# lipku/LiveTalking

Measured on AMD Instinct MI355X. Metric: inferfps, higher is better.
Workload: dtype f16; 1 GPU; wav2lip256, 1 session(s)/GPU, 16-frame batch, fp16 activations / fp32 accumulate, through LipReal.inference_batch; sessions_per_gpu=1, batch=16, parallelism=session-sharded x1 (no collective)

## Files before the change

include/ltk.h:

```cpp
#ifndef LTK_H
#define LTK_H

#include <stddef.h>
#include <stdint.h>

#ifdef __cplusplus
extern "C" {
#endif

#define LTK_OK 0
#define LTK_E_INVALID (-1)
#define LTK_E_HIP (-2)
#define LTK_E_STATE (-3)
#define LTK_E_NOMEM (-4)

typedef struct ltk_engine ltk_engine;

typedef struct ltk_named_tensor {
    const char* name;
    const float* data;
    int ndim;
    const int64_t* shape;
} ltk_named_tensor;

typedef struct ltk_w2l_req {
    int avatar;
    int index;
    int batch;
    const void* d_mel;
    void* d_pred;
} ltk_w2l_req;

const char* ltk_last_error(void);
const char* ltk_version(void);

int ltk_engine_create(int device, ltk_engine** out);
void ltk_engine_destroy(ltk_engine* e);
int ltk_engine_sync(ltk_engine* e);

int ltk_wav2lip_load(ltk_engine* e, const ltk_named_tensor* sd, int n, int max_frames);

int ltk_avatar_register(ltk_engine* e, const uint8_t* face_bank, const uint8_t* full_bank,
                        const int32_t* coords, int n, int H, int W, int* avatar_id);
int ltk_avatar_release(ltk_engine* e, int avatar_id);

int ltk_mel_step(ltk_engine* e, const float* pcm, int n_samples, const int32_t* win_start,
                 int n_win, void* d_out, void* stream);

int ltk_wav2lip_infer(ltk_engine* e, const ltk_w2l_req* reqs, int nreq, void* stream);

int ltk_paste_back(ltk_engine* e, int avatar_id, int idx, const void* d_pred, void* out,
                   int out_is_device, void* stream);

int ltk_paste_back_batch(ltk_engine* e, int avatar_id, const int32_t* idx, const void* d_pred, int n, void* out, void* stream);


int ltk_musetalk_load(ltk_engine* e, const ltk_named_tensor* unet_sd, int n_unet, const ltk_named_tensor* vae_sd,
                      int n_vae, int max_frames);

int ltk_musetalk_avatar_register(ltk_engine* e, const float* latents, const uint8_t* full_bank, const int32_t* face_boxes,
                                 const int32_t* crop_boxes, const uint8_t* masks, const int64_t* mask_offsets, int n,
                                 int H, int W, int* avatar_id);

int ltk_musetalk_set_fp8(ltk_engine* e, int enable, float act_scale);
int ltk_musetalk_info(ltk_engine* e, double* macs_per_frame, double* macs_fp8_per_frame);

typedef struct ltk_mt_req {
    int avatar;
    int index;
    int batch;
    const void* d_feat;
    void* d_pred;
} ltk_mt_req;

int ltk_musetalk_infer(ltk_engine* e, const ltk_mt_req* reqs, int nreq, void* stream);

int ltk_paste_blend(ltk_engine* e, int avatar_id, int idx, const void* d_pred, void* out, int out_is_device, void* stream);


int ltk_ultralight_avatar_register(ltk_engine* e, const ltk_named_tensor* sd, int n_tensors, const uint8_t* face_bank,
                                   const uint8_t* full_bank, const int32_t* coords, int n, int H, int W, int max_frames, int* avatar_id);

typedef struct ltk_ul_req {
    int avatar;
    int index;
    int batch;
    const void* d_feat;
    void* d_pred;
} ltk_ul_req;

int ltk_ultralight_infer(ltk_engine* e, const ltk_ul_req* reqs, int nreq, void* stream);

int ltk_ultralight_paste_back(ltk_engine* e, int avatar_id, int idx, const void* d_pred, void* out, int out_is_device, void* stream);

int ltk_ultralight_paste_back_batch(ltk_engine* e, int avatar_id, const int32_t* idx, const void* d_pred, int n, void* out, void* stream);

typedef struct ltk_egress ltk_egress;
int ltk_egress_open(ltk_engine* e, int H, int W, ltk_egress** out);
int ltk_egress_close(ltk_engine* e, ltk_egress* s);
int ltk_egress_watermark(ltk_engine* e, ltk_egress* s, const uint8_t* mask, int x, int y, int w, int h, int b, int g, int r);

#define LTK_FMT_BGR24 0
#define LTK_FMT_I420 1
#define LTK_SRC_WAV2LIP 0
#define LTK_SRC_MUSETALK 1
#define LTK_SRC_HOST 2
#define LTK_SRC_ULTRALIGHT 3
typedef struct ltk_egress_req {
    int source;
    int avatar, idx;
    const void* d_pred;
    const uint8_t* h_frame;
    int speaking;
    double alpha;
    int keep;
    int format;
    int chroma;
} ltk_egress_req;
int ltk_egress_frame(ltk_engine* e, ltk_egress* s, const ltk_egress_req* req, uint8_t* h_out, void* stream);

int ltk_egress_batch(ltk_engine* e, ltk_egress* s, int source, int avatar, const int32_t* idx, const void* d_pred, int n, int format,
                     int chroma, uint8_t* h_out, void* stream);

int ltk_whisper_load(ltk_engine* e, const ltk_named_tensor* encoder_sd, int n);

int ltk_whisper_step(ltk_engine* e, const float* pcm, int n_samples, int batch, int first_row, int row_step, int rows,
                     void* d_out, void* stream);


int ltk_hubert_load(ltk_engine* e, const ltk_named_tensor* sd, int n);

int ltk_hubert_features(ltk_engine* e, const float* pcm, long long n_samples, float* out_host, int cap_rows, int* rows);

int ltk_hubert_step(ltk_engine* e, const float* pcm, int n_samples, int batch, int first_row, int row_step, int rows, void* d_out);

int ltk_vae_encoder_load(ltk_engine* e, const ltk_named_tensor* vae_sd, int n, int max_faces);
int ltk_vae_encode_faces(ltk_engine* e, const uint8_t* faces_bgr, int nfaces, const float* noise, float* latents_out);


int ltk_whisper_debug_get(ltk_engine* e, const char* name, float* out, size_t n_floats);

int ltk_hubert_debug_get(ltk_engine* e, const char* name, float* out, size_t n_floats);
int ltk_hubert_op_count(ltk_engine* e);
int ltk_hubert_op_name(ltk_engine* e, int op, char* buf, int buf_len, int* type);
int ltk_hubert_info(ltk_engine* e, int* layers, int* programs, size_t* activation_bytes);
int ltk_hubert_stats(ltk_engine* e, const float* pcm, long long n, float* mean_var);
int ltk_hubert_layer0_host(ltk_engine* e, const float* x, int n, const float* w, const float* bias, const float* gamma, const float* beta,
                           float* out);
int ltk_hubert_ln_gelu_host(ltk_engine* e, const float* x, int T, const float* gamma, const float* beta, float* out);
int ltk_hubert_posconv_host(ltk_engine* e, const float* x, int T, const float* w, const float* bias, float* out);
int ltk_hubert_chunks_host(ltk_engine* e, const float* feat, int T, int batch, int first_row, int row_step, int rows, float* out);

int ltk_musetalk_forward_host(ltk_engine* e, const float* latents, const float* feat, int B, float* unet_out, float* image,
                              uint8_t* frames);
int ltk_musetalk_debug_get(ltk_engine* e, const char* name, int frames, float* out, size_t n_floats);
int ltk_musetalk_time(ltk_engine* e, int frames, int iters, float* ms_per_pass, double* macs_per_pass);
int ltk_musetalk_op_count(ltk_engine* e);
int ltk_musetalk_op_name(ltk_engine* e, int op, char* buf, int buf_len, int* type);
int ltk_musetalk_time_ops(ltk_engine* e, int frames, int iters, float* ms_per_op, int n_ops);


int ltk_wav2lip_forward_host(ltk_engine* e, const float* mel, const float* face6, int B, float* pred);

int ltk_ultralight_forward_host(ltk_engine* e, int avatar_id, const float* img6, const float* feat, int B, float* pred);
int ltk_ultralight_op_count(ltk_engine* e, int avatar_id);
int ltk_ultralight_op_name(ltk_engine* e, int avatar_id, int op, char* buf, int buf_len, int* type);
int ltk_ultralight_time(ltk_engine* e, int avatar_id, int frames, int iters, float* ms_per_pass, double* macs_per_pass);

int ltk_dwconv3x3_f16(ltk_engine* e, const void* d_x, int N, int H, int W, int C, const float* weight, int stride, const float* scale,
                      const float* shift, int relu, void* d_y);
int ltk_upsample2x_cat_f16(ltk_engine* e, const void* d_x, int N, int h, int w, int C_up, const void* d_skip, int Hs, int Ws, int C_skip,
                           void* d_y);

int ltk_debug_saturation(ltk_engine* e, int reset, unsigned long long* n_at_limit, unsigned long long* n_nonfinite);
int ltk_debug_capture(ltk_engine* e, int enable);
int ltk_debug_get(ltk_engine* e, const char* layer, float* out, size_t n_floats);

int ltk_debug_set_knob(const char* name, int value);

int ltk_debug_tile_table_check(char* msg, int cap);

int ltk_wav2lip_time_convs(ltk_engine* e, int frames, int iters, float* ms_per_pass, double* macs_per_pass);

int ltk_wav2lip_graph_count(ltk_engine* e);

int ltk_avatar_face_cache_bytes(ltk_engine* e, int avatar_id, size_t* bytes);

int ltk_wav2lip_prefetch_stats(ltk_engine* e, unsigned long long* hits, unsigned long long* misses, unsigned long long* issued);

int ltk_program_graph_count(ltk_engine* e);

int ltk_wav2lip_layer_count(ltk_engine* e);
int ltk_wav2lip_layer_name(ltk_engine* e, int layer, char* buf, int buf_len);
int ltk_wav2lip_set_layer_tile(ltk_engine* e, int layer, int bucket, int pxw, int nbt, int ksplit);
int ltk_wav2lip_time_layers(ltk_engine* e, int frames, int iters, float* ms_per_layer, int n_layers);

int ltk_conv2d_f16(ltk_engine* e, const void* d_x, int N, int H, int W, int Cin,
                   const float* weight, int Cout, int kh, int kw, int sh, int sw, int ph, int pw,
                   int transposed, int out_pad, const float* scale, const float* shift,
                   const void* d_res, int relu, void* d_y, int iters, float* ms_avg);

typedef struct ltk_conv_opts {
    int x_ld, x_coff, y_ld, y_coff, res_ld, res_coff;
    int act, ups;
    int force_pxw, force_nbt, force_ksplit;
    int family;
} ltk_conv_opts;
typedef struct ltk_conv_report {
    char kernel[64];
    int family, G, NBT, PXW, NC8, T, S, ksplit, items, grid, FT, UB;
} ltk_conv_report;
int ltk_conv2d_f16_ex(ltk_engine* e, const void* d_x, int N, int H, int W, int Cin,
                      const float* weight, int Cout, int kh, int kw, int sh, int sw, int ph, int pw,
                      int transposed, int out_pad, const float* scale, const float* shift,
                      const void* d_res, int relu, void* d_y, const ltk_conv_opts* opts, ltk_conv_report* rep);

int ltk_debug_conv_plan(int N, int H, int W, int Cin, int Cout, int kh, int kw, int sh, int sw, int ph, int pw,
                        int transposed, int out_pad, int has_res, int relu, const ltk_conv_opts* opts, ltk_conv_report* rep);

int ltk_debug_conv3_variants(char* buf, int cap);

int ltk_groupnorm_f16(ltk_engine* e, const void* d_x, int N, int C, int P, int groups, float eps, const float* gamma, const float* beta,
                      int silu, int impl, int out_fp8, float out_scale, void* d_y, int iters, float* ms_avg);

typedef struct ltk_norm_opts {
    int x_ld, x_coff, y_ld, y_coff;
} ltk_norm_opts;
typedef struct ltk_norm_report {
    char kernel[64];
    int impl, segs, members, grid;
} ltk_norm_report;
int ltk_groupnorm_f16_ex(ltk_engine* e, const void* d_x, int N, int C, int P, int groups, float eps, const float* gamma, const float* beta,
                         int silu, int impl, int out_fp8, float out_scale, void* d_y, const ltk_norm_opts* opts, ltk_norm_report* rep);

enum { LTK_PW_LAYERNORM = 0, LTK_PW_GEGLU = 1, LTK_PW_ACT_GELU = 2, LTK_PW_ACT_SILU = 3, LTK_PW_ADD_POS = 4, LTK_PW_NCHW_TO_CB16 = 5,
       LTK_PW_TOKENS_TO_CB16 = 6, LTK_PW_VAE_POST = 7 };
int ltk_pointwise_f16(ltk_engine* e, int op, const void* d_x, void* d_y, int N, int C, int P, float eps, const float* v0, const float* v1,
                      const ltk_norm_opts* opts);

int ltk_attention_f16(ltk_engine* e, const void* d_q, int q_cbt, int q_cb0, const void* d_k, int k_cbt, int k_cb0, const void* d_v, int v_cbt,
                      int v_cb0, void* d_o, int o_cbt, int o_cb0, int N, int heads, int d16, int Tq, int Tk, int impl);

int ltk_f32_to_e4m3(const float* in, size_t n, uint8_t* out);

int ltk_conv2d_fp8(ltk_engine* e, const void* d_x, int N, int H, int W, int Cin, const float* weight, int Cout,
                   const float* scale, const float* shift, float act_scale, const void* d_res, int act, void* d_y, int iters,
                   float* ms_avg);

int ltk_conv2d_fp8_ex(ltk_engine* e, const void* d_x, int N, int H, int W, int Cin, const float* weight, int Cout,
                      const float* scale, const float* shift, float act_scale, int quant, const void* d_res, void* d_y,
                      const ltk_conv_opts* opts, ltk_conv_report* rep);

int ltk_debug_conv_fp8_plan(int N, int H, int W, int Cin, int Cout, int kh, int kw, int sh, int sw, int ph, int pw,
                            int transposed, int out_pad, int quant, int has_res, const ltk_conv_opts* opts, ltk_conv_report* rep);

int ltk_debug_conv3_fp8_variants(char* buf, int cap);

#ifdef __cplusplus
}
#endif
#endif
```

livetalking_amd/_lib.py:

```python
from __future__ import annotations

import ctypes as C
import os

_HERE = os.path.dirname(os.path.abspath(__file__))
LIB_PATH = os.environ.get("LTK_LIB") or os.path.join(_HERE, "libltk_hip.so")


class LtkError(RuntimeError):
    def __init__(self, code: int, msg: str):
        super().__init__(f"ltk error {code}: {msg}")
        self.code = code


class NamedTensor(C.Structure):
    _fields_ = [("name", C.c_char_p), ("data", C.POINTER(C.c_float)), ("ndim", C.c_int),
                ("shape", C.POINTER(C.c_int64))]


class W2lReq(C.Structure):
    _fields_ = [("avatar", C.c_int), ("index", C.c_int), ("batch", C.c_int), ("d_mel", C.c_void_p),
                ("d_pred", C.c_void_p)]


class MtReq(C.Structure):
    _fields_ = [("avatar", C.c_int), ("index", C.c_int), ("batch", C.c_int), ("d_feat", C.c_void_p), ("d_pred", C.c_void_p)]


class UlReq(C.Structure):
    _fields_ = [("avatar", C.c_int), ("index", C.c_int), ("batch", C.c_int), ("d_feat", C.c_void_p), ("d_pred", C.c_void_p)]


class EgressReq(C.Structure):
    _fields_ = [("source", C.c_int), ("avatar", C.c_int), ("idx", C.c_int), ("d_pred", C.c_void_p), ("h_frame", C.c_void_p),
                ("speaking", C.c_int), ("alpha", C.c_double), ("keep", C.c_int), ("format", C.c_int), ("chroma", C.c_int)]


class ConvOpts(C.Structure):
    _fields_ = [(n, C.c_int) for n in ("x_ld", "x_coff", "y_ld", "y_coff", "res_ld", "res_coff", "act", "ups", "force_pxw", "force_nbt",
                                       "force_ksplit", "family")]


class ConvReport(C.Structure):
    _fields_ = [("kernel", C.c_char * 64)] + [(n, C.c_int) for n in ("family", "G", "NBT", "PXW", "NC8", "T", "S", "ksplit", "items", "grid",
                                                                     "FT", "UB")]


class NormOpts(C.Structure):
    _fields_ = [(n, C.c_int) for n in ("x_ld", "x_coff", "y_ld", "y_coff")]


class NormReport(C.Structure):
    _fields_ = [("kernel", C.c_char * 64)] + [(n, C.c_int) for n in ("impl", "segs", "members", "grid")]


SYMBOLS = {
    "ltk_last_error": (C.c_char_p, []),
    "ltk_version": (C.c_char_p, []),
    "ltk_engine_create": (C.c_int, [C.c_int, C.POINTER(C.c_void_p)]),
    "ltk_engine_destroy": (None, [C.c_void_p]),
    "ltk_engine_sync": (C.c_int, [C.c_void_p]),
    "ltk_wav2lip_load": (C.c_int, [C.c_void_p, C.POINTER(NamedTensor), C.c_int, C.c_int]),
    "ltk_avatar_register": (C.c_int, [C.c_void_p, C.c_void_p, C.c_void_p, C.c_void_p, C.c_int, C.c_int, C.c_int,
                                      C.POINTER(C.c_int)]),
    "ltk_avatar_release": (C.c_int, [C.c_void_p, C.c_int]),
    "ltk_mel_step": (C.c_int, [C.c_void_p, C.c_void_p, C.c_int, C.c_void_p, C.c_int, C.c_void_p, C.c_void_p]),
    "ltk_wav2lip_infer": (C.c_int, [C.c_void_p, C.POINTER(W2lReq), C.c_int, C.c_void_p]),
    "ltk_paste_back": (C.c_int, [C.c_void_p, C.c_int, C.c_int, C.c_void_p, C.c_void_p, C.c_int, C.c_void_p]),
    "ltk_paste_back_batch": (C.c_int, [C.c_void_p, C.c_int, C.c_void_p, C.c_void_p, C.c_int, C.c_void_p, C.c_void_p]),
    "ltk_musetalk_load": (C.c_int, [C.c_void_p, C.POINTER(NamedTensor), C.c_int, C.POINTER(NamedTensor), C.c_int, C.c_int]),
    "ltk_musetalk_set_fp8": (C.c_int, [C.c_void_p, C.c_int, C.c_float]),
    "ltk_musetalk_info": (C.c_int, [C.c_void_p, C.POINTER(C.c_double), C.POINTER(C.c_double)]),
    "ltk_musetalk_avatar_register": (C.c_int, [C.c_void_p, C.c_void_p, C.c_void_p, C.c_void_p, C.c_void_p, C.c_void_p, C.c_void_p,
                                               C.c_int, C.c_int, C.c_int, C.POINTER(C.c_int)]),
    "ltk_musetalk_infer": (C.c_int, [C.c_void_p, C.POINTER(MtReq), C.c_int, C.c_void_p]),
    "ltk_paste_blend": (C.c_int, [C.c_void_p, C.c_int, C.c_int, C.c_void_p, C.c_void_p, C.c_int, C.c_void_p]),
    "ltk_ultralight_avatar_register": (C.c_int, [C.c_void_p, C.POINTER(NamedTensor), C.c_int, C.c_void_p, C.c_void_p, C.c_void_p, C.c_int,
                                                 C.c_int, C.c_int, C.c_int, C.POINTER(C.c_int)]),
    "ltk_ultralight_infer": (C.c_int, [C.c_void_p, C.POINTER(UlReq), C.c_int, C.c_void_p]),
    "ltk_ultralight_paste_back": (C.c_int, [C.c_void_p, C.c_int, C.c_int, C.c_void_p, C.c_void_p, C.c_int, C.c_void_p]),
    "ltk_ultralight_paste_back_batch": (C.c_int, [C.c_void_p, C.c_int, C.c_void_p, C.c_void_p, C.c_int, C.c_void_p, C.c_void_p]),
    "ltk_ultralight_forward_host": (C.c_int, [C.c_void_p, C.c_int, C.c_void_p, C.c_void_p, C.c_int, C.c_void_p]),
    "ltk_ultralight_time": (C.c_int, [C.c_void_p, C.c_int, C.c_int, C.c_int, C.POINTER(C.c_float), C.POINTER(C.c_double)]),
    "ltk_dwconv3x3_f16": (C.c_int, [C.c_void_p, C.c_void_p, C.c_int, C.c_int, C.c_int, C.c_int, C.c_void_p, C.c_int, C.c_void_p,
                                    C.c_void_p, C.c_int, C.c_void_p]),
    "ltk_upsample2x_cat_f16": (C.c_int, [C.c_void_p, C.c_void_p, C.c_int, C.c_int, C.c_int, C.c_int, C.c_void_p, C.c_int, C.c_int,
                                         C.c_int, C.c_void_p]),
    "ltk_egress_open": (C.c_int, [C.c_void_p, C.c_int, C.c_int, C.POINTER(C.c_void_p)]),
    "ltk_egress_close": (C.c_int, [C.c_void_p, C.c_void_p]),
    "ltk_egress_watermark": (C.c_int, [C.c_void_p, C.c_void_p, C.c_void_p, C.c_int, C.c_int, C.c_int, C.c_int, C.c_int, C.c_int, C.c_int]),
    "ltk_egress_frame": (C.c_int, [C.c_void_p, C.c_void_p, C.POINTER(EgressReq), C.c_void_p, C.c_void_p]),
    "ltk_egress_batch": (C.c_int, [C.c_void_p, C.c_void_p, C.c_int, C.c_int, C.c_void_p, C.c_void_p, C.c_int, C.c_int, C.c_int,
                                   C.c_void_p, C.c_void_p]),
    "ltk_musetalk_forward_host": (C.c_int, [C.c_void_p, C.c_void_p, C.c_void_p, C.c_int, C.c_void_p, C.c_void_p, C.c_void_p]),
    "ltk_musetalk_debug_get": (C.c_int, [C.c_void_p, C.c_char_p, C.c_int, C.c_void_p, C.c_size_t]),
    "ltk_musetalk_time": (C.c_int, [C.c_void_p, C.c_int, C.c_int, C.POINTER(C.c_float), C.POINTER(C.c_double)]),
    "ltk_whisper_load": (C.c_int, [C.c_void_p, C.POINTER(NamedTensor), C.c_int]),
    "ltk_whisper_step": (C.c_int, [C.c_void_p, C.c_void_p, C.c_int, C.c_int, C.c_int, C.c_int, C.c_int, C.c_void_p, C.c_void_p]),
    "ltk_whisper_debug_get": (C.c_int, [C.c_void_p, C.c_char_p, C.c_void_p, C.c_size_t]),
    "ltk_hubert_load": (C.c_int, [C.c_void_p, C.POINTER(NamedTensor), C.c_int]),
    "ltk_hubert_features": (C.c_int, [C.c_void_p, C.c_void_p, C.c_longlong, C.c_void_p, C.c_int, C.POINTER(C.c_int)]),
    "ltk_hubert_step": (C.c_int, [C.c_void_p, C.c_void_p, C.c_int, C.c_int, C.c_int, C.c_int, C.c_int, C.c_void_p]),
    "ltk_hubert_debug_get": (C.c_int, [C.c_void_p, C.c_char_p, C.c_void_p, C.c_size_t]),
    "ltk_ultralight_op_count": (C.c_int, [C.c_void_p, C.c_int]),
    "ltk_ultralight_op_name": (C.c_int, [C.c_void_p, C.c_int, C.c_int, C.c_char_p, C.c_int, C.POINTER(C.c_int)]),
    "ltk_hubert_op_count": (C.c_int, [C.c_void_p]),
    "ltk_hubert_op_name": (C.c_int, [C.c_void_p, C.c_int, C.c_char_p, C.c_int, C.POINTER(C.c_int)]),
    "ltk_hubert_info": (C.c_int, [C.c_void_p, C.POINTER(C.c_int), C.POINTER(C.c_int), C.POINTER(C.c_size_t)]),
    "ltk_hubert_stats": (C.c_int, [C.c_void_p, C.c_void_p, C.c_longlong, C.c_void_p]),
    "ltk_hubert_layer0_host": (C.c_int, [C.c_void_p, C.c_void_p, C.c_int, C.c_void_p, C.c_void_p, C.c_void_p, C.c_void_p, C.c_void_p]),
    "ltk_hubert_ln_gelu_host": (C.c_int, [C.c_void_p, C.c_void_p, C.c_int, C.c_void_p, C.c_void_p, C.c_void_p]),
    "ltk_hubert_posconv_host": (C.c_int, [C.c_void_p, C.c_void_p, C.c_int, C.c_void_p, C.c_void_p, C.c_void_p]),
    "ltk_hubert_chunks_host": (C.c_int, [C.c_void_p, C.c_void_p, C.c_int, C.c_int, C.c_int, C.c_int, C.c_int, C.c_void_p]),
    "ltk_vae_encoder_load": (C.c_int, [C.c_void_p, C.POINTER(NamedTensor), C.c_int, C.c_int]),
    "ltk_vae_encode_faces": (C.c_int, [C.c_void_p, C.c_void_p, C.c_int, C.c_void_p, C.c_void_p]),
    "ltk_wav2lip_forward_host": (C.c_int, [C.c_void_p, C.c_void_p, C.c_void_p, C.c_int, C.c_void_p]),
    "ltk_debug_capture": (C.c_int, [C.c_void_p, C.c_int]),
    "ltk_debug_saturation": (C.c_int, [C.c_void_p, C.c_int, C.POINTER(C.c_ulonglong), C.POINTER(C.c_ulonglong)]),
    "ltk_debug_set_knob": (C.c_int, [C.c_char_p, C.c_int]),
    "ltk_debug_tile_table_check": (C.c_int, [C.c_char_p, C.c_int]),
    "ltk_debug_get": (C.c_int, [C.c_void_p, C.c_char_p, C.c_void_p, C.c_size_t]),
    "ltk_wav2lip_time_convs": (C.c_int, [C.c_void_p, C.c_int, C.c_int, C.POINTER(C.c_float), C.POINTER(C.c_double)]),
    "ltk_wav2lip_graph_count": (C.c_int, [C.c_void_p]),
    "ltk_program_graph_count": (C.c_int, [C.c_void_p]),
    "ltk_wav2lip_prefetch_stats": (C.c_int, [C.c_void_p, C.POINTER(C.c_ulonglong), C.POINTER(C.c_ulonglong), C.POINTER(C.c_ulonglong)]),
    "ltk_avatar_face_cache_bytes": (C.c_int, [C.c_void_p, C.c_int, C.POINTER(C.c_size_t)]),
    "ltk_musetalk_op_count": (C.c_int, [C.c_void_p]),
    "ltk_musetalk_op_name": (C.c_int, [C.c_void_p, C.c_int, C.c_char_p, C.c_int, C.POINTER(C.c_int)]),
    "ltk_musetalk_time_ops": (C.c_int, [C.c_void_p, C.c_int, C.c_int, C.POINTER(C.c_float), C.c_int]),
    "ltk_wav2lip_layer_count": (C.c_int, [C.c_void_p]),
    "ltk_wav2lip_layer_name": (C.c_int, [C.c_void_p, C.c_int, C.c_char_p, C.c_int]),
    "ltk_wav2lip_set_layer_tile": (C.c_int, [C.c_void_p, C.c_int, C.c_int, C.c_int, C.c_int, C.c_int]),
    "ltk_wav2lip_time_layers": (C.c_int, [C.c_void_p, C.c_int, C.c_int, C.POINTER(C.c_float), C.c_int]),
    "ltk_conv2d_f16": (C.c_int, [C.c_void_p, C.c_void_p, C.c_int, C.c_int, C.c_int, C.c_int, C.c_void_p, C.c_int,
                                 C.c_int, C.c_int, C.c_int, C.c_int, C.c_int, C.c_int, C.c_int, C.c_int,
                                 C.c_void_p, C.c_void_p, C.c_void_p, C.c_int, C.c_void_p, C.c_int,
                                 C.POINTER(C.c_float)]),
    "ltk_conv2d_f16_ex": (C.c_int, [C.c_void_p, C.c_void_p, C.c_int, C.c_int, C.c_int, C.c_int, C.c_void_p, C.c_int,
                                    C.c_int, C.c_int, C.c_int, C.c_int, C.c_int, C.c_int, C.c_int, C.c_int,
                                    C.c_void_p, C.c_void_p, C.c_void_p, C.c_int, C.c_void_p, C.POINTER(ConvOpts), C.POINTER(ConvReport)]),
    "ltk_debug_conv_plan": (C.c_int, [C.c_int] * 15 + [C.POINTER(ConvOpts), C.POINTER(ConvReport)]),
    "ltk_debug_conv3_variants": (C.c_int, [C.c_char_p, C.c_int]),
    "ltk_groupnorm_f16": (C.c_int, [C.c_void_p, C.c_void_p, C.c_int, C.c_int, C.c_int, C.c_int, C.c_float, C.c_void_p, C.c_void_p, C.c_int, C.c_int,
                                    C.c_int, C.c_float, C.c_void_p, C.c_int, C.POINTER(C.c_float)]),
    "ltk_groupnorm_f16_ex": (C.c_int, [C.c_void_p, C.c_void_p, C.c_int, C.c_int, C.c_int, C.c_int, C.c_float, C.c_void_p, C.c_void_p, C.c_int, C.c_int,
                                       C.c_int, C.c_float, C.c_void_p, C.POINTER(NormOpts), C.POINTER(NormReport)]),
    "ltk_pointwise_f16": (C.c_int, [C.c_void_p, C.c_int, C.c_void_p, C.c_void_p, C.c_int, C.c_int, C.c_int, C.c_float, C.c_void_p, C.c_void_p,
                                    C.POINTER(NormOpts)]),
    "ltk_attention_f16": (C.c_int, [C.c_void_p] + [C.c_void_p, C.c_int, C.c_int] * 4 + [C.c_int] * 6),
    "ltk_f32_to_e4m3": (C.c_int, [C.c_void_p, C.c_size_t, C.c_void_p]),
    "ltk_conv2d_fp8": (C.c_int, [C.c_void_p, C.c_void_p, C.c_int, C.c_int, C.c_int, C.c_int, C.c_void_p, C.c_int, C.c_void_p,
                                 C.c_void_p, C.c_float, C.c_void_p, C.c_int, C.c_void_p, C.c_int, C.POINTER(C.c_float)]),
    "ltk_conv2d_fp8_ex": (C.c_int, [C.c_void_p, C.c_void_p, C.c_int, C.c_int, C.c_int, C.c_int, C.c_void_p, C.c_int, C.c_void_p,
                                    C.c_void_p, C.c_float, C.c_int, C.c_void_p, C.c_void_p, C.POINTER(ConvOpts), C.POINTER(ConvReport)]),
    "ltk_debug_conv_fp8_plan": (C.c_int, [C.c_int] * 15 + [C.POINTER(ConvOpts), C.POINTER(ConvReport)]),
    "ltk_debug_conv3_fp8_variants": (C.c_int, [C.c_char_p, C.c_int]),
}

_lib = None


def load() -> C.CDLL:
    global _lib
    if _lib is not None:
        return _lib
    if not os.path.exists(LIB_PATH):
        raise RuntimeError(
            f"{LIB_PATH} is missing: build it with `python -c 'import __graft_entry__ as g; g.build()'` "
            "(or `make -C livetalking_amd/csrc`). livetalking_amd has no CPU fallback.")
    try:
        import torch
    except ImportError:
        pass
    lib = C.CDLL(LIB_PATH)
    other_build = bool(os.environ.get("LTK_LIB"))
    for name, (res, args) in SYMBOLS.items():
        if other_build and not hasattr(lib, name):
            continue
        fn = getattr(lib, name)
        fn.restype = res
        fn.argtypes = args
    _lib = lib
    return lib


def check(rc: int) -> None:
    if rc != 0:
        msg = load().ltk_last_error()
        raise LtkError(rc, msg.decode("utf-8", "replace") if msg else "")
```

livetalking_amd/avatars/wav2lip_avatar.py:

```python
from __future__ import annotations

import glob
import os
import pickle
import threading
import weakref

import numpy as np

from ..egress import SRC_WAV2LIP, DeviceEgressMixin, FrameGroup
from ..engine import Engine
from ..hostshim import BaseAvatar, mirror_index, register
from ..scheduler import get_scheduler
from ..sharding import EnginePool, visible_devices
from .audio_features.mel import MelASR

_PASTE_BATCH = os.environ.get("LTK_PASTE_BATCH", "1") != "0"


class Wav2LipModel:

    def __init__(self, engine_or_pool):
        if isinstance(engine_or_pool, EnginePool):
            self.pool = engine_or_pool
        else:
            self.pool = EnginePool([getattr(engine_or_pool, "device", 0)], lambda d: engine_or_pool)
        self.engines = self.pool.engines
        self._avatars = {}
        self._lock = threading.Lock()

    @property
    def engine(self) -> Engine:
        return self.engines[0]

    def place(self, session) -> int:
        slot = self.pool.place(id(session))
        weakref.finalize(session, self.pool.release, id(session))
        return slot

    def avatar_id(self, avatar, slot: int = 0) -> int:
        frame_list, face_list, coord_list = avatar
        key = (id(face_list), slot)
        with self._lock:
            aid = self._avatars.get(key)
            if aid is None:
                aid = self.engines[slot].register_avatar(face_list, frame_list, coord_list)
                self._avatars[key] = aid
            return aid

    def eval(self):
        return self


def _state_dict_from_checkpoint(path):
    import torch
    checkpoint = torch.load(path, map_location="cpu")
    s = checkpoint["state_dict"]
    return {k.replace("module.", ""): v for k, v in s.items()}


def load_model(path, state_dict=None, max_frames=None, device=None):
    if state_dict is None:
        state_dict = _state_dict_from_checkpoint(path)
    if max_frames is None:
        max_frames = int(os.environ.get("LTK_MAX_FRAMES", "256"))

    def factory(dev):
        eng = Engine(dev)
        eng.load_wav2lip(state_dict, max_frames=max_frames)
        return eng

    devices = visible_devices() if device is None else [int(device)]
    cap = int(os.environ.get("LTK_SESSIONS_PER_GPU", "0")) or (1 << 30)
    return Wav2LipModel(EnginePool(devices, factory, capacity_per_gpu=cap))


def read_imgs(img_list):
    import cv2
    return [cv2.imread(p) for p in img_list]


def load_avatar(avatar_id):
    avatar_path = f"./data/avatars/{avatar_id}"
    bank_path = os.path.join(avatar_path, "bank.ltkbank")
    if os.path.exists(bank_path):
        from ..bank import load_bank
        return load_bank(bank_path).as_avatar()
    with open(f"{avatar_path}/coords.pkl", "rb") as f:
        coord_list_cycle = pickle.load(f)

    def numbered(d):
        files = glob.glob(os.path.join(d, "*.[jpJP][pnPN]*[gG]"))
        return sorted(files, key=lambda x: int(os.path.splitext(os.path.basename(x))[0]))

    frame_list_cycle = read_imgs(numbered(f"{avatar_path}/full_imgs"))
    face_list_cycle = read_imgs(numbered(f"{avatar_path}/face_imgs"))
    return frame_list_cycle, face_list_cycle, coord_list_cycle


def warm_up(batch_size, model, modelres=256):
    mel = np.ones((batch_size, 80, 16), dtype=np.float32)
    img = np.ones((batch_size, 6, modelres, modelres), dtype=np.float32)
    for eng in model.engines:
        n = min(batch_size, eng.max_frames)
        eng.wav2lip_forward_host(mel[:n], img[:n])


@register("avatar", "wav2lip")
class LipReal(DeviceEgressMixin, BaseAvatar):
    _egress_source = SRC_WAV2LIP

    def __init__(self, opt, model, avatar):
        super().__init__(opt)
        self.model = model
        self.frame_list_cycle, self.face_list_cycle, self.coord_list_cycle = avatar
        self._slot = model.place(self)
        self.engine = model.engines[self._slot]
        self._aid = model.avatar_id(avatar, self._slot)
        h, w = self.frame_list_cycle[0].shape[:2]
        self._frame_hw = (int(h), int(w))
        self._sched = get_scheduler(self.engine)
        self.asr = MelASR(opt, self, engine=self.engine)
        self.asr.warm_up()

    def _mel_to_device(self, audiofeat_batch):
        import torch
        if isinstance(audiofeat_batch, torch.Tensor):
            return audiofeat_batch
        arr = np.ascontiguousarray(np.asarray(audiofeat_batch), dtype=np.float32)
        return torch.from_numpy(arr).to(self.engine.torch_device)

    def inference_batch(self, index, audiofeat_batch):
        import torch
        mel = self._mel_to_device(audiofeat_batch)
        B = self.batch_size
        if mel.shape[0] != B:
            raise ValueError(f"expected {B} mel windows, got {mel.shape[0]}")
        pred = torch.empty((B, 256, 256, 3), dtype=torch.uint8, device=mel.device)
        self._sched.infer(self._aid, int(index), B, mel.data_ptr(), pred.data_ptr())
        self._last_mel = mel
        items = list(pred.unbind(0))
        if _PASTE_BATCH and hasattr(self.engine, "paste_back_batch"):
            FrameGroup.attach(items, pred, span=(len(self.frame_list_cycle), int(index), B))
        return items

    def paste_back_frame(self, pred_frame, idx: int):
        import torch
        if not isinstance(pred_frame, torch.Tensor):
            pred_frame = torch.from_numpy(np.ascontiguousarray(pred_frame).astype(np.uint8)).to(
                self.engine.torch_device)
        h, w = self._frame_hw
        grp = getattr(pred_frame, "_ltk_group", None)
        if grp is not None and grp.idx[pred_frame._ltk_i] == int(idx):
            with grp.lock:
                if grp.host is None:
                    host = torch.empty((len(grp.idx), h, w, 3), dtype=torch.uint8, pin_memory=True)
                    self.engine.paste_back_batch(self._aid, grp.idx, grp.pred.data_ptr(), host.data_ptr())
                    grp.host = host.numpy()
            return grp.host[pred_frame._ltk_i]
        out = np.empty((h, w, 3), dtype=np.uint8)
        self.engine.paste_back(self._aid, int(idx), pred_frame.data_ptr(), out)
        return out
```

livetalking_amd/csrc/egress.hip:

```cpp
#include "engine_internal.h"

struct ltk_egress {
    int H = 0, W = 0;
    std::mutex mu;
    uint8_t* d_cache[2] = {nullptr, nullptr};
    bool have[2] = {false, false};
    uint8_t* d_frame = nullptr;
    uint8_t* d_out = nullptr;
    uint8_t* d_wm = nullptr;
    int wm_x = 0, wm_y = 0, wm_w = 0, wm_h = 0, wm_b = 0, wm_g = 0, wm_r = 0;
};

extern "C" {

int ltk_egress_open(ltk_engine* e, int H, int W, ltk_egress** out) {
    if (!e || !out || H <= 0 || W <= 0) return fail(LTK_E_INVALID, "bad arguments");
    CHK(enter_device(e->device));
    ltk_egress* s = new ltk_egress();
    s->H = H; s->W = W;
    const size_t bytes = (size_t)H * W * 3;
    if (hipMalloc((void**)&s->d_cache[0], bytes) != hipSuccess || hipMalloc((void**)&s->d_cache[1], bytes) != hipSuccess ||
        hipMalloc((void**)&s->d_frame, bytes) != hipSuccess || hipMalloc((void**)&s->d_out, bytes) != hipSuccess) {
        (void)hipFree(s->d_cache[0]); (void)hipFree(s->d_cache[1]); (void)hipFree(s->d_frame); (void)hipFree(s->d_out);
        delete s;
        return fail(LTK_E_NOMEM, "egress session buffers");
    }
    *out = s;
    return LTK_OK;
}

int ltk_egress_close(ltk_engine* e, ltk_egress* s) {
    if (!e || !s) return fail(LTK_E_INVALID, "bad arguments");
    CHK(enter_device(e->device));
    {
        std::lock_guard<std::mutex> g(s->mu);
        (void)hipFree(s->d_cache[0]); (void)hipFree(s->d_cache[1]); (void)hipFree(s->d_frame); (void)hipFree(s->d_out); (void)hipFree(s->d_wm);
    }
    delete s;
    return LTK_OK;
}

int ltk_egress_watermark(ltk_engine* e, ltk_egress* s, const uint8_t* mask, int x, int y, int w, int h, int b, int g, int r) {
    if (!e || !s) return fail(LTK_E_INVALID, "bad arguments");
    CHK(enter_device(e->device));
    std::lock_guard<std::mutex> gd(s->mu);
    (void)hipFree(s->d_wm);
    s->d_wm = nullptr;
    s->wm_w = s->wm_h = 0;
    if (!mask) return LTK_OK;
    if (w <= 0 || h <= 0) return fail(LTK_E_INVALID, "empty watermark rectangle");
    CHK(hipMalloc((void**)&s->d_wm, (size_t)w * h));
    CHK(hipMemcpy(s->d_wm, mask, (size_t)w * h, hipMemcpyHostToDevice));
    s->wm_x = x; s->wm_y = y; s->wm_w = w; s->wm_h = h; s->wm_b = b; s->wm_g = g; s->wm_r = r;
    return LTK_OK;
}

int ltk_egress_frame(ltk_engine* e, ltk_egress* s, const ltk_egress_req* q, uint8_t* h_out, void* stream) {
    if (!e || !s || !q || !h_out) return fail(LTK_E_INVALID, "bad arguments");
    const int H = s->H, W = s->W;
    const size_t bytes = (size_t)H * W * 3;
    if (q->format != LTK_FMT_BGR24 && q->format != LTK_FMT_I420) return fail(LTK_E_INVALID, "unknown output format");
    if (q->format == LTK_FMT_I420 && ((H | W) & 1)) return fail(LTK_E_INVALID, "I420 needs even frame dimensions");
    CHK(enter_device(e->device));
    std::lock_guard<std::mutex> gs(s->mu);
    StreamLease sl(e, stream);
    const uint8_t* src = nullptr;
    std::shared_ptr<Avatar> hold_w;
    std::shared_ptr<MtAvatar> hold_m;
    std::shared_ptr<UlAvatar> hold_u;
    if (q->source == LTK_SRC_HOST) {
        if (!q->h_frame) return fail(LTK_E_INVALID, "LTK_SRC_HOST without h_frame");
        CHK(hipMemcpyAsync(s->d_frame, q->h_frame, bytes, hipMemcpyHostToDevice, sl.s));
        src = s->d_frame;
    } else if (q->source == LTK_SRC_WAV2LIP) {
        if (!(hold_w = find_avatar(e, q->avatar))) return fail(LTK_E_STATE, "unknown avatar id");
        const Avatar& a = *hold_w;
        if (q->idx < 0 || q->idx >= a.n) return fail(LTK_E_INVALID, "frame index outside the bank");
        if (a.H != H || a.W != W) return fail(LTK_E_INVALID, "avatar frame size differs from the egress session");
        const uint8_t* full = a.d_full + (size_t)q->idx * bytes;
        if (q->d_pred) {
            const int32_t* c = a.coords.data() + 4 * (size_t)q->idx;
            launch_paste(full, H, W, (const uint8_t*)q->d_pred, c[0], c[1], c[2], c[3], s->d_frame, sl.s);
            src = s->d_frame;
        } else {
            src = full;
        }
    } else if (q->source == LTK_SRC_MUSETALK) {
        if (!(hold_m = find_mt_avatar(e, q->avatar))) return fail(LTK_E_STATE, "unknown MuseTalk avatar id");
        const MtAvatar& a = *hold_m;
        if (q->idx < 0 || q->idx >= a.n) return fail(LTK_E_INVALID, "frame index outside the bank");
        if (a.H != H || a.W != W) return fail(LTK_E_INVALID, "avatar frame size differs from the egress session");
        const uint8_t* full = a.d_full + (size_t)q->idx * bytes;
        const uint8_t* mask = a.d_masks + a.mask_off[q->idx];
        const int32_t* fb = a.face_box.data() + 4 * (size_t)q->idx;
        const int32_t* cb = a.crop_box.data() + 4 * (size_t)q->idx;
        if (q->d_pred) {
            launch_paste_blend(full, H, W, (const uint8_t*)q->d_pred, fb[0], fb[1], fb[2], fb[3], cb[0], cb[1], cb[2], cb[3], mask,
                               s->d_frame, sl.s);
            src = s->d_frame;
        } else {
            src = full;
        }
    } else if (q->source == LTK_SRC_ULTRALIGHT) {
        if (!(hold_u = find_ul_avatar(e, q->avatar))) return fail(LTK_E_STATE, "unknown Ultralight avatar id");
        const UlAvatar& a = *hold_u;
        if (q->idx < 0 || q->idx >= a.n) return fail(LTK_E_INVALID, "frame index outside the bank");
        if (a.H != H || a.W != W) return fail(LTK_E_INVALID, "avatar frame size differs from the egress session");
        const uint8_t* full = a.d_full + (size_t)q->idx * bytes;
        if (q->d_pred) {
            const int32_t* c = a.boxes.data() + 4 * (size_t)q->idx;
            launch_ul_paste(full, H, W, a.d_face + (size_t)q->idx * kUlFace * kUlFace * 3, (const uint8_t*)q->d_pred, c[0], c[1], c[2], c[3],
                            s->d_frame, sl.s);
            src = s->d_frame;
        } else {
            src = full;
        }
    } else {
        return fail(LTK_E_INVALID, "unknown frame source");
    }
    const int me = q->speaking ? 1 : 0, other = me ^ 1;
    const bool blend = q->alpha >= 0.0 && q->alpha < 1.0 && s->have[other];
    const float w_src = (float)q->alpha, w_prev = (float)(1.0 - q->alpha);
    launch_egress(src, blend ? s->d_cache[other] : nullptr, w_prev, w_src, q->keep ? s->d_cache[me] : nullptr, s->d_wm, s->wm_x,
                  s->wm_y, s->wm_w, s->wm_h, s->wm_b, s->wm_g, s->wm_r, s->d_out, H, W, q->format == LTK_FMT_I420, q->chroma, sl.s);
    CHK(hipGetLastError());
    if (q->keep) s->have[me] = true;
    const size_t out_bytes = q->format == LTK_FMT_I420 ? bytes / 2 : bytes;
    CHK(hipMemcpyAsync(h_out, s->d_out, out_bytes, hipMemcpyDeviceToHost, sl.s));
    CHK(hipStreamSynchronize(sl.s));
    return LTK_OK;
}

int ltk_egress_batch(ltk_engine* e, ltk_egress* s, int source, int avatar, const int32_t* idx, const void* d_pred, int n, int format,
                     int chroma, uint8_t* h_out, void* stream) {
    if (!e || !s || !idx || !d_pred || !h_out || n <= 0) return fail(LTK_E_INVALID, "bad arguments");
    const int H = s->H, W = s->W;
    const size_t bytes = (size_t)H * W * 3;
    if (format != LTK_FMT_BGR24 && format != LTK_FMT_I420) return fail(LTK_E_INVALID, "unknown output format");
    if (format == LTK_FMT_I420 && ((H | W) & 1)) return fail(LTK_E_INVALID, "I420 needs even frame dimensions");
    if (source != LTK_SRC_WAV2LIP && source != LTK_SRC_MUSETALK && source != LTK_SRC_ULTRALIGHT)
        return fail(LTK_E_INVALID, "batch egress: Wav2Lip, MuseTalk or Ultralight frames only");
    CHK(enter_device(e->device));
    std::lock_guard<std::mutex> gs(s->mu);
    std::shared_ptr<Avatar> hold_w;
    std::shared_ptr<MtAvatar> hold_m;
    std::shared_ptr<UlAvatar> hold_u;
    int bank_n, bank_h, bank_w;
    if (source == LTK_SRC_WAV2LIP) {
        if (!(hold_w = find_avatar(e, avatar))) return fail(LTK_E_STATE, "unknown avatar id");
        bank_n = hold_w->n; bank_h = hold_w->H; bank_w = hold_w->W;
    } else if (source == LTK_SRC_MUSETALK) {
        if (!(hold_m = find_mt_avatar(e, avatar))) return fail(LTK_E_STATE, "unknown MuseTalk avatar id");
        bank_n = hold_m->n; bank_h = hold_m->H; bank_w = hold_m->W;
    } else {
        if (!(hold_u = find_ul_avatar(e, avatar))) return fail(LTK_E_STATE, "unknown Ultralight avatar id");
        bank_n = hold_u->n; bank_h = hold_u->H; bank_w = hold_u->W;
    }
    if (bank_h != H || bank_w != W) return fail(LTK_E_INVALID, "avatar frame size differs from the egress session");
    for (int i = 0; i < n; ++i)
        if (idx[i] < 0 || idx[i] >= bank_n) return fail(LTK_E_INVALID, "frame index outside the bank");
    const size_t out_bytes = format == LTK_FMT_I420 ? bytes / 2 : bytes;
    StreamLease sl(e, stream);
    ScratchLease sc(e, (bytes + out_bytes) * n);
    if (!sc.s.d) return fail(LTK_E_NOMEM, "scratch allocation failed");
    uint8_t* const comp = (uint8_t*)sc.s.d;
    uint8_t* const conv = comp + bytes * n;
    if (hold_w) {
        const Avatar& a = *hold_w;
        for (int i0 = 0; i0 < n; i0 += kPasteBatch) {
            const int m = std::min(kPasteBatch, n - i0);
            PasteBatch pb;
            for (int i = 0; i < m; ++i) {
                const int32_t* c = a.coords.data() + 4 * (size_t)idx[i0 + i];
                pb.full[i] = a.d_full + (size_t)idx[i0 + i] * bytes;
                pb.y1[i] = c[0]; pb.y2[i] = c[1]; pb.x1[i] = c[2]; pb.x2[i] = c[3];
            }
            launch_paste_batch(pb, m, H, W, (const uint8_t*)d_pred + (size_t)i0 * 256 * 256 * 3, comp + bytes * i0, bytes, sl.s);
        }
    } else if (hold_u) {
        for (int i0 = 0; i0 < n; i0 += kPasteBatch) {
            const int m = std::min(kPasteBatch, n - i0);
            UlPasteBatch pb;
            ul_fill_paste_batch(*hold_u, idx + i0, m, &pb);
            launch_ul_paste_batch(pb, m, H, W, (const uint8_t*)d_pred + (size_t)i0 * kUlRes * kUlRes * 3, comp + bytes * i0, bytes, sl.s);
        }
    } else {
        const MtAvatar& a = *hold_m;
        for (int i = 0; i < n; ++i) {
            const int32_t* fb = a.face_box.data() + 4 * (size_t)idx[i];
            const int32_t* cb = a.crop_box.data() + 4 * (size_t)idx[i];
            launch_paste_blend(a.d_full + (size_t)idx[i] * bytes, H, W, (const uint8_t*)d_pred + (size_t)i * 256 * 256 * 3, fb[0], fb[1], fb[2], fb[3],
                               cb[0], cb[1], cb[2], cb[3], a.d_masks + a.mask_off[idx[i]], comp + bytes * i, sl.s);
        }
    }
    launch_egress_batch(comp, bytes, n, s->d_wm, s->wm_x, s->wm_y, s->wm_w, s->wm_h, s->wm_b, s->wm_g, s->wm_r, conv, out_bytes, H, W,
                        format == LTK_FMT_I420, chroma, sl.s);
    hipError_t pe = hipGetLastError();
    if (pe == hipSuccess) pe = hipMemcpyAsync(h_out, conv, out_bytes * n, hipMemcpyDeviceToHost, sl.s);
    const hipError_t se = hipStreamSynchronize(sl.s);
    if (pe != hipSuccess || se != hipSuccess) return fail(LTK_E_HIP, std::string("egress_batch: ") + hipGetErrorString(pe != hipSuccess ? pe : se));
    return LTK_OK;
}

}
```

livetalking_amd/csrc/engine.hip:

```cpp
#include "engine_internal.h"

thread_local std::string ltk::g_err;

namespace {

double hz_to_mel(double f) {
    const double f_sp = 200.0 / 3, min_log_hz = 1000.0, min_log_mel = min_log_hz / f_sp, logstep = log(6.4) / 27.0;
    return f >= min_log_hz ? min_log_mel + log(f / min_log_hz) / logstep : f / f_sp;
}
double mel_to_hz(double m) {
    const double f_sp = 200.0 / 3, min_log_hz = 1000.0, min_log_mel = min_log_hz / f_sp, logstep = log(6.4) / 27.0;
    return m >= min_log_mel ? min_log_hz * exp(logstep * (m - min_log_mel)) : f_sp * m;
}
}

void ltk::build_mel_basis(std::vector<float>* basis, std::vector<int32_t>* lohi, int n_bins, double f_lo, double f_hi) {
    const int n_mels = 80;
    const double sr = 16000.0;
    std::vector<double> mel_f(n_mels + 2);
    const double m0 = hz_to_mel(f_lo), m1 = hz_to_mel(f_hi);
    for (int i = 0; i < n_mels + 2; ++i) mel_f[i] = mel_to_hz(m0 + (m1 - m0) * i / (n_mels + 1));
    basis->assign((size_t)n_mels * n_bins, 0.f);
    lohi->assign(2 * n_mels, 0);
    for (int i = 0; i < n_mels; ++i) {
        const double enorm = 2.0 / (mel_f[i + 2] - mel_f[i]);
        int lo = n_bins, hi = 0;
        for (int k = 0; k < n_bins; ++k) {
            const double f = (sr / 2) * k / (n_bins - 1);
            const double lower = -(mel_f[i] - f) / (mel_f[i + 1] - mel_f[i]);
            const double upper = (mel_f[i + 2] - f) / (mel_f[i + 2] - mel_f[i + 1]);
            const double w = fmax(0.0, lower < upper ? lower : upper) * enorm;
            const float wf = (float)w;
            (*basis)[(size_t)i * n_bins + k] = wf;
            if (wf != 0.f) { if (k < lo) lo = k; if (k + 1 > hi) hi = k + 1; }
        }
        if (lo > hi) lo = hi = 0;
        (*lohi)[2 * i] = lo; (*lohi)[2 * i + 1] = hi;
    }
}

extern "C" {

const char* ltk_last_error(void) { return g_err.c_str(); }
const char* ltk_version(void) { return "ltk_hip 0.1 (gfx950)"; }

int ltk_engine_create(int device, ltk_engine** out) {
    if (!out) return fail(LTK_E_INVALID, "out is null");
    int ndev = 0;
    CHK(hipGetDeviceCount(&ndev));
    if (device < 0 || device >= ndev) return fail(LTK_E_INVALID, "no such HIP device");
    CHK(hipSetDevice(device));
    std::unique_ptr<ltk_engine> e(new ltk_engine());
    e->device = device;
    CHK(hipStreamCreateWithFlags(&e->compute, hipStreamNonBlocking));
    CHK(hipStreamCreateWithFlags(&e->aux, hipStreamNonBlocking));
    CHK(hipStreamCreateWithFlags(&e->aux2, hipStreamNonBlocking));
    e->graphs.side = e->aux2;
    CHK(hipEventCreateWithFlags(&e->ev_fork, hipEventDisableTiming));
    CHK(hipEventCreateWithFlags(&e->ev_join, hipEventDisableTiming));
    e->partial_cap = (size_t)128 << 20;
    e->partial_aux_cap = (size_t)16 << 20;
    e->partial_pf_cap = (size_t)64 << 20;
    CHK(hipMalloc((void**)&e->d_partial, e->partial_cap));
    CHK(hipMalloc((void**)&e->d_partial_aux, e->partial_aux_cap));
    CHK(hipMalloc((void**)&e->d_partial_pf, e->partial_pf_cap));
    CHK(hipMalloc((void**)&e->d_sat, 2 * sizeof(unsigned long long)));
    CHK(hipMemset(e->d_sat, 0, 2 * sizeof(unsigned long long)));
    std::vector<float> basis;
    std::vector<int32_t> lohi;
    build_mel_basis(&basis, &lohi);
    CHK(hipMalloc((void**)&e->d_basis, basis.size() * sizeof(float)));
    CHK(hipMemcpy(e->d_basis, basis.data(), basis.size() * sizeof(float), hipMemcpyHostToDevice));
    CHK(hipMalloc((void**)&e->d_lohi, lohi.size() * sizeof(int32_t)));
    CHK(hipMemcpy(e->d_lohi, lohi.data(), lohi.size() * sizeof(int32_t), hipMemcpyHostToDevice));
    *out = e.release();
    return LTK_OK;
}

void ltk_engine_destroy(ltk_engine* e) {
    if (!e) return;
    if (e->tm_calls)
        fprintf(stderr, "ltk: ltk_wav2lip_infer host time per call over %lu calls: prepare %.1f us, upload + pass launch %.1f us, prefetch join / serial launch %.1f us, wait for the device %.1f us\n",
                e->tm_calls, e->tm_prep / e->tm_calls, e->tm_launch / e->tm_calls, e->tm_pf / e->tm_calls, e->tm_wait / e->tm_calls);
    (void)hipSetDevice(e->device);
    (void)hipDeviceSynchronize();
    wav2lip_unload(e);
    if (e->d_basis) (void)hipFree(e->d_basis);
    if (e->d_lohi) (void)hipFree(e->d_lohi);
    e->avatars.clear();
    e->mt_avatars.clear();
    e->prog_graphs.drop();
    ul_unload(e);
    if (e->mt) mt_graph_delete(e->mt);
    if (e->whisper) mt_graph_delete(e->whisper);
    hubert_unload(e);
    if (e->vae_enc) mt_graph_delete(e->vae_enc);
    if (e->d_wbasis) (void)hipFree(e->d_wbasis);
    if (e->d_wlogspec) (void)hipFree(e->d_wlogspec);
    if (e->d_wpcm) (void)hipFree(e->d_wpcm);
    if (e->d_wgmax) (void)hipFree(e->d_wgmax);
    if (e->d_pe) (void)hipFree(e->d_pe);
    if (e->d_mt_feat) (void)hipFree(e->d_mt_feat);
    if (e->d_mt_lat) (void)hipFree(e->d_mt_lat);
    for (Scratch& s : e->scratch_free) (void)hipFree(s.d);
    for (hipStream_t s : e->stream_free) (void)hipStreamDestroy(s);
    if (e->d_partial) (void)hipFree(e->d_partial);
    if (e->d_partial_aux) (void)hipFree(e->d_partial_aux);
    if (e->d_partial_pf) (void)hipFree(e->d_partial_pf);
    if (e->d_sat) (void)hipFree(e->d_sat);
    if (e->ev_fork) (void)hipEventDestroy(e->ev_fork);
    if (e->ev_join) (void)hipEventDestroy(e->ev_join);
    if (e->aux2) (void)hipStreamDestroy(e->aux2);
    if (e->aux) (void)hipStreamDestroy(e->aux);
    if (e->compute) (void)hipStreamDestroy(e->compute);
    delete e;
}

int ltk_engine_sync(ltk_engine* e) {
    if (!e) return fail(LTK_E_INVALID, "engine is null");
    CHK(enter_device(e->device));
    CHK(hipDeviceSynchronize());
    return LTK_OK;
}

int ltk_avatar_register(ltk_engine* e, const uint8_t* face_bank, const uint8_t* full_bank,
                        const int32_t* coords, int n, int H, int W, int* avatar_id) {
    if (!e || !face_bank || !full_bank || !coords || !avatar_id || n <= 0 || H <= 0 || W <= 0)
        return fail(LTK_E_INVALID, "bad arguments");
    for (int i = 0; i < n; ++i) {
        const int32_t* c = coords + 4 * i;
        if (c[0] < 0 || c[2] < 0 || c[1] > H || c[3] > W || c[1] <= c[0] || c[3] <= c[2])
            return fail(LTK_E_INVALID, "coords box outside the frame");
    }
    CHK(enter_device(e->device));
    auto ap = std::make_shared<Avatar>();
    Avatar& a = *ap;
    a.device = e->device;
    a.n = n; a.H = H; a.W = W;
    a.coords.assign(coords, coords + 4 * (size_t)n);
    const size_t fb = (size_t)n * 256 * 256 * 3, ub = (size_t)n * H * W * 3;
    CHK(hipMalloc((void**)&a.d_face, fb));
    CHK(hipMalloc((void**)&a.d_full, ub));
    CHK(hipMemcpy(a.d_face, face_bank, fb, hipMemcpyHostToDevice));
    CHK(hipMemcpy(a.d_full, full_bank, ub, hipMemcpyHostToDevice));
    std::lock_guard<std::mutex> g(e->pool_mu);
    const int id = e->next_avatar++;
    e->avatars[id] = ap;
    *avatar_id = id;
    return LTK_OK;
}

int ltk_avatar_release(ltk_engine* e, int avatar_id) {
    if (!e) return fail(LTK_E_INVALID, "engine is null");
    {
        std::lock_guard<std::mutex> ge(e->mu);
        for (ltk_engine::PfSlot& sl : e->pfs)
            if (sl.avatar == avatar_id && (sl.valid || sl.hold)) {
                if (sl.filled && sl.ev_done) (void)hipEventSynchronize(sl.ev_done);
                sl.valid = false;
                sl.hold.reset();
            }
        ul_drop_graphs(e, avatar_id);
    }
    std::lock_guard<std::mutex> g(e->pool_mu);
    auto it = e->avatars.find(avatar_id);
    if (it != e->avatars.end()) { e->avatars.erase(it); return LTK_OK; }
    auto mt = e->mt_avatars.find(avatar_id);
    if (mt != e->mt_avatars.end()) { e->mt_avatars.erase(mt); return LTK_OK; }
    auto ul = e->ul_avatars.find(avatar_id);
    if (ul != e->ul_avatars.end()) { e->ul_avatars.erase(ul); return LTK_OK; }
    return fail(LTK_E_STATE, "unknown avatar id");
}

int ltk_mel_step(ltk_engine* e, const float* pcm, int n_samples, const int32_t* win_start, int n_win,
                 void* d_out, void* stream) {
    if (!e || !pcm || !win_start || !d_out || n_samples <= 0 || n_win <= 0 || n_win > 1024)
        return fail(LTK_E_INVALID, "bad arguments");
    const int n_cols_total = 1 + n_samples / 200;
    int cmin = 1 << 30, cmax = -1;
    for (int i = 0; i < n_win; ++i) {
        if (win_start[i] < 0 || win_start[i] + 16 > n_cols_total) return fail(LTK_E_INVALID, "mel window outside the spectrogram");
        if (win_start[i] < cmin) cmin = win_start[i];
        if (win_start[i] + 15 > cmax) cmax = win_start[i] + 15;
    }
    CHK(enter_device(e->device));
    const size_t pcm_bytes = (size_t)n_samples * sizeof(float);
    const size_t ws_off = (pcm_bytes + 255) / 256 * 256;
    ScratchLease sc(e, ws_off + (size_t)n_win * sizeof(int32_t));
    if (!sc.s.d) return fail(LTK_E_NOMEM, "scratch allocation failed");
    StreamLease sl(e, stream);
    CHK(hipMemcpyAsync(sc.s.d, pcm, pcm_bytes, hipMemcpyHostToDevice, sl.s));
    CHK(hipMemcpyAsync((char*)sc.s.d + ws_off, win_start, (size_t)n_win * sizeof(int32_t), hipMemcpyHostToDevice, sl.s));
    launch_mel((const float*)sc.s.d, n_samples, (const int32_t*)((char*)sc.s.d + ws_off), n_win, cmin, cmax - cmin + 1,
               e->d_basis, e->d_lohi, (float*)d_out, sl.s);
    CHK(hipGetLastError());
    CHK(hipStreamSynchronize(sl.s));
    return LTK_OK;
}

int ltk_paste_back(ltk_engine* e, int avatar_id, int idx, const void* d_pred, void* out, int out_is_device, void* stream) {
    if (!e || !d_pred || !out) return fail(LTK_E_INVALID, "bad arguments");
    const std::shared_ptr<Avatar> ap = find_avatar(e, avatar_id);
    if (!ap) return fail(LTK_E_STATE, "unknown avatar id");
    const Avatar& a = *ap;
    if (idx < 0 || idx >= a.n) return fail(LTK_E_INVALID, "frame index outside the bank");
    CHK(enter_device(e->device));
    const int32_t* c = a.coords.data() + 4 * (size_t)idx;
    const size_t bytes = (size_t)a.H * a.W * 3;
    StreamLease sl(e, stream);
    const uint8_t* full = a.d_full + (size_t)idx * bytes;
    if (out_is_device) {
        launch_paste(full, a.H, a.W, (const uint8_t*)d_pred, c[0], c[1], c[2], c[3], (uint8_t*)out, sl.s);
        CHK(hipGetLastError());
        CHK(hipStreamSynchronize(sl.s));
        return LTK_OK;
    }
    ScratchLease sc(e, bytes);
    if (!sc.s.d) return fail(LTK_E_NOMEM, "scratch allocation failed");
    launch_paste(full, a.H, a.W, (const uint8_t*)d_pred, c[0], c[1], c[2], c[3], (uint8_t*)sc.s.d, sl.s);
    CHK(hipGetLastError());
    CHK(hipMemcpyAsync(out, sc.s.d, bytes, hipMemcpyDeviceToHost, sl.s));
    CHK(hipStreamSynchronize(sl.s));
    return LTK_OK;
}

int ltk_paste_back_batch(ltk_engine* e, int avatar_id, const int32_t* idx, const void* d_pred, int n, void* out, void* stream) {
    if (!e || !idx || !d_pred || !out || n <= 0) return fail(LTK_E_INVALID, "bad arguments");
    const std::shared_ptr<Avatar> ap = find_avatar(e, avatar_id);
    if (!ap) return fail(LTK_E_STATE, "unknown avatar id");
    const Avatar& a = *ap;
    for (int i = 0; i < n; ++i)
        if (idx[i] < 0 || idx[i] >= a.n) return fail(LTK_E_INVALID, "frame index outside the bank");
    CHK(enter_device(e->device));
    const size_t bytes = (size_t)a.H * a.W * 3;
    StreamLease sl(e, stream);
    ScratchLease sc(e, bytes * n);
    if (!sc.s.d) return fail(LTK_E_NOMEM, "scratch allocation failed");
    for (int i0 = 0; i0 < n; i0 += kPasteBatch) {
        const int m = std::min(kPasteBatch, n - i0);
        PasteBatch pb;
        for (int i = 0; i < m; ++i) {
            const int32_t* c = a.coords.data() + 4 * (size_t)idx[i0 + i];
            pb.full[i] = a.d_full + (size_t)idx[i0 + i] * bytes;
            pb.y1[i] = c[0]; pb.y2[i] = c[1]; pb.x1[i] = c[2]; pb.x2[i] = c[3];
        }
        launch_paste_batch(pb, m, a.H, a.W, (const uint8_t*)d_pred + (size_t)i0 * 256 * 256 * 3, (uint8_t*)sc.s.d + (size_t)i0 * bytes, bytes, sl.s);
    }
    hipError_t pe = hipGetLastError();
    if (pe == hipSuccess) pe = hipMemcpyAsync(out, sc.s.d, bytes * n, hipMemcpyDeviceToHost, sl.s);
    const hipError_t se = hipStreamSynchronize(sl.s);
    if (pe != hipSuccess || se != hipSuccess) return fail(LTK_E_HIP, std::string("paste_back_batch: ") + hipGetErrorString(pe != hipSuccess ? pe : se));
    return LTK_OK;
}

int ltk_paste_blend(ltk_engine* e, int avatar_id, int idx, const void* d_pred, void* out, int out_is_device, void* stream) {
    if (!e || !d_pred || !out) return fail(LTK_E_INVALID, "bad arguments");
    const std::shared_ptr<MtAvatar> hold = find_mt_avatar(e, avatar_id);
    if (!hold) return fail(LTK_E_STATE, "unknown MuseTalk avatar id");
    const MtAvatar& a = *hold;
    if (idx < 0 || idx >= a.n) return fail(LTK_E_INVALID, "frame index outside the bank");
    const int H = a.H, W = a.W;
    const uint8_t* full = a.d_full + (size_t)idx * H * W * 3;
    const uint8_t* mask = a.d_masks + a.mask_off[idx];
    const int32_t* fb = a.face_box.data() + 4 * (size_t)idx;
    const int32_t* cb = a.crop_box.data() + 4 * (size_t)idx;
    CHK(enter_device(e->device));
    const size_t bytes = (size_t)H * W * 3;
    StreamLease sl(e, stream);
    if (out_is_device) {
        launch_paste_blend(full, H, W, (const uint8_t*)d_pred, fb[0], fb[1], fb[2], fb[3], cb[0], cb[1], cb[2], cb[3], mask, (uint8_t*)out, sl.s);
        CHK(hipGetLastError());
        CHK(hipStreamSynchronize(sl.s));
        return LTK_OK;
    }
    ScratchLease sc(e, bytes);
    if (!sc.s.d) return fail(LTK_E_NOMEM, "scratch allocation failed");
    launch_paste_blend(full, H, W, (const uint8_t*)d_pred, fb[0], fb[1], fb[2], fb[3], cb[0], cb[1], cb[2], cb[3], mask, (uint8_t*)sc.s.d, sl.s);
    CHK(hipGetLastError());
    CHK(hipMemcpyAsync(out, sc.s.d, bytes, hipMemcpyDeviceToHost, sl.s));
    CHK(hipStreamSynchronize(sl.s));
    return LTK_OK;
}

}
```

livetalking_amd/csrc/engine_debug.hip:

```cpp
#include "debug_util.h"

extern "C" {

int ltk_wav2lip_forward_host(ltk_engine* e, const float* mel, const float* face6, int B, float* pred) {
    if (!e || !mel || !face6 || !pred || B <= 0) return fail(LTK_E_INVALID, "bad arguments");
    if (!e->loaded) return fail(LTK_E_STATE, "ltk_wav2lip_load has not been called");
    if (B > e->max_frames) return fail(LTK_E_INVALID, "B exceeds max_frames");
    CHK(enter_device(e->device));
    const int mb = std::min(e->micro_batch, kPackMaxFrames);
    const int cap = std::min(B, mb);
    DevBuf d_mel, d_face, d_pred;
    CHK(hipMalloc(&d_mel.p, (size_t)cap * 80 * 16 * sizeof(float)));
    CHK(hipMalloc(&d_face.p, (size_t)cap * 6 * 65536 * sizeof(float)));
    CHK(hipMalloc(&d_pred.p, (size_t)cap * 3 * 65536 * sizeof(float)));
    for (int f0 = 0; f0 < B; f0 += mb) {
        const int nf = std::min(mb, B - f0);
        CHK(hipMemcpy(d_mel.p, mel + (size_t)f0 * 1280, (size_t)nf * 1280 * sizeof(float), hipMemcpyHostToDevice));
        CHK(hipMemcpy(d_face.p, face6 + (size_t)f0 * 6 * 65536, (size_t)nf * 6 * 65536 * sizeof(float), hipMemcpyHostToDevice));
        MelPtrs mp;
        for (int i = 0; i < nf; ++i) mp.p[i] = (float*)d_mel.p + (size_t)i * 1280;
        {
            std::lock_guard<std::mutex> g(e->mu);
            launch_upload_tables(nullptr, &mp, nullptr, nf, e->d_tab, e->compute);
            CHK(hipGetLastError());
            const int rc = launch_pass(e, nf, e->compute, false, (const float*)d_face.p, false, (float*)d_pred.p);
            if (rc) return rc;
            CHK(hipStreamSynchronize(e->compute));
        }
        CHK(hipMemcpy(pred + (size_t)f0 * 3 * 65536, d_pred.p, (size_t)nf * 3 * 65536 * sizeof(float), hipMemcpyDeviceToHost));
    }
    return LTK_OK;
}

int ltk_debug_saturation(ltk_engine* e, int reset, unsigned long long* n_at_limit, unsigned long long* n_nonfinite) {
    if (!e) return fail(LTK_E_INVALID, "bad arguments");
    CHK(enter_device(e->device));
    std::lock_guard<std::mutex> g(e->mu);
    CHK(hipDeviceSynchronize());
    unsigned long long h[2] = {0, 0};
    CHK(hipMemcpy(h, e->d_sat, sizeof(h), hipMemcpyDeviceToHost));
    if (n_at_limit) *n_at_limit = h[0];
    if (n_nonfinite) *n_nonfinite = h[1];
    if (reset) CHK(hipMemset(e->d_sat, 0, sizeof(h)));
    return LTK_OK;
}

int ltk_debug_capture(ltk_engine* e, int enable) {
    if (!e) return fail(LTK_E_INVALID, "engine is null");
    std::lock_guard<std::mutex> g(e->mu);
    e->capture = enable != 0;
    if (!enable) { e->taps.clear(); e->tap_shape.clear(); }
    return LTK_OK;
}

int ltk_debug_set_knob(const char* name, int value) {
    if (knob_set(name, value)) return fail(LTK_E_INVALID, std::string("unknown knob ") + (name ? name : "(null)"));
    return LTK_OK;
}

int ltk_debug_get(ltk_engine* e, const char* layer, float* out, size_t n_floats) {
    if (!e || !layer || !out) return fail(LTK_E_INVALID, "bad arguments");
    std::lock_guard<std::mutex> g(e->mu);
    auto it = e->taps.find(layer);
    if (it == e->taps.end()) return fail(LTK_E_STATE, std::string("no capture for layer ") + layer);
    if (it->second.size() != n_floats) return fail(LTK_E_INVALID, "size mismatch: captured " + std::to_string(it->second.size()));
    memcpy(out, it->second.data(), n_floats * sizeof(float));
    return LTK_OK;
}

namespace {
struct TimingIO {
    DevBuf face, mel, frames;
    int setup(ltk_engine* e, int nf) {
        CHK(hipMalloc(&face.p, 65536 * 3));
        CHK(hipMemset(face.p, 0, 65536 * 3));
        CHK(hipMalloc(&mel.p, 1280 * sizeof(float)));
        CHK(hipMemset(mel.p, 0, 1280 * sizeof(float)));
        CHK(hipMalloc(&frames.p, (size_t)nf * 65536 * 3));
        FacePtrs fp; MelPtrs mp; OutPtrs op;
        for (int i = 0; i < nf; ++i) { fp.p[i] = (const uint8_t*)face.p; mp.p[i] = (const float*)mel.p; op.p[i] = (uint8_t*)frames.p + (size_t)i * 65536 * 3; }
        launch_upload_tables(&fp, &mp, &op, nf, e->d_tab, e->compute);
        CHK(hipGetLastError());
        return 0;
    }
};
}

int ltk_wav2lip_time_convs(ltk_engine* e, int frames, int iters, float* ms_per_pass, double* macs_per_pass) {
    if (!e || frames <= 0 || iters <= 0 || !ms_per_pass) return fail(LTK_E_INVALID, "bad arguments");
    if (!e->loaded) return fail(LTK_E_STATE, "ltk_wav2lip_load has not been called");
    if (frames > e->max_frames) return fail(LTK_E_INVALID, "frames exceeds max_frames");
    CHK(enter_device(e->device));
    std::lock_guard<std::mutex> g(e->mu);
    if (e->capture) return fail(LTK_E_STATE, "disable capture before timing");
    const int mbs = std::min(e->micro_batch, kPackMaxFrames);
    TimingIO tio;
    int rc = tio.setup(e, std::min(mbs, frames));
    if (rc) return rc;
    for (ltk_engine::PfSlot& sl : e->pfs) sl.valid = false;
    const bool pipe = knob(K_PREFETCH) && e->alt_frames > 0 && frames <= std::min(e->alt_frames, mbs) && knob(K_HEAD_FUSED) && e->c7;
    if (pipe) {
        FacePtrs nx;
        for (int i = 0; i < frames; ++i) nx.p[i] = (const uint8_t*)tio.face.p;
        launch_upload_tables(&nx, nullptr, nullptr, frames, e->d_tab_next, e->aux2);
    }
    int cur = 0;
    auto pass = [&]() -> int {
        int prc = 0;
        if (pipe) {
            if (cur) CHK(hipStreamWaitEvent(e->compute, e->pfs[cur].ev_done, 0));
            prc = launch_pass(e, frames, e->compute, true, nullptr, true, nullptr, false, cur, cur != 0);
            if (cur) {
                if (hipEventRecord(e->pfs[cur].ev_read, e->compute) != hipSuccess) { if (!prc) prc = fail(LTK_E_HIP, "hipEventRecord failed"); }
                else e->pfs[cur].read = true;
            }
            const int nxt = cur == 1 ? 2 : 1;
            if (!prc) prc = launch_prefetch(e, frames, nxt);
            cur = nxt;
            return prc;
        }
        for (int f0 = 0; f0 < frames && !prc; f0 += mbs) prc = launch_pass(e, std::min(mbs, frames - f0), e->compute, true, nullptr, true, nullptr);
        return prc;
    };
    if (pipe) { rc = pass(); if (!rc) rc = pass(); if (!rc) rc = pass(); if (rc) return rc; }
    rc = pass();
    if (!rc) rc = pass();
    if (rc) return rc;
    float ms = 0.f;
    if ((rc = time_iters(e->compute, iters, pass, &ms))) return rc;
    *ms_per_pass = ms / iters;
    if (macs_per_pass) *macs_per_pass = (e->macs_per_frame - (knob(K_HEAD_FUSED) ? 0.0 : 32.0 * 3 * 65536)) * frames;
    return LTK_OK;
}

int ltk_wav2lip_prefetch_stats(ltk_engine* e, unsigned long long* hits, unsigned long long* misses, unsigned long long* issued) {
    if (!e) return fail(LTK_E_INVALID, "engine is null");
    std::lock_guard<std::mutex> g(e->mu);
    if (hits) *hits = e->pf_hits;
    if (misses) *misses = e->pf_misses;
    if (issued) *issued = e->pf_issued;
    return LTK_OK;
}

int ltk_program_graph_count(ltk_engine* e) {
    if (!e) return 0;
    std::lock_guard<std::mutex> g(e->mu);
    return e->prog_graphs.live();
}

int ltk_wav2lip_graph_count(ltk_engine* e) {
    if (!e) return 0;
    std::lock_guard<std::mutex> g(e->mu);
    return e->graphs.live();
}

int ltk_wav2lip_layer_count(ltk_engine* e) {
    if (!e || !e->loaded) return 0;
    return (int)e->layers.size();
}

int ltk_wav2lip_layer_name(ltk_engine* e, int layer, char* buf, int buf_len) {
    if (!e || !e->loaded || layer < 0 || layer >= (int)e->layers.size() || !buf || buf_len <= 0) return fail(LTK_E_INVALID, "bad arguments");
    snprintf(buf, (size_t)buf_len, "%s", e->layers[layer].name.c_str());
    return LTK_OK;
}

int ltk_wav2lip_set_layer_tile(ltk_engine* e, int layer, int bucket, int pxw, int nbt, int ksplit) {
    if (!e || !e->loaded || layer < 0 || layer >= (int)e->layers.size() || bucket < 0 || bucket > 4) return fail(LTK_E_INVALID, "bad arguments");
    std::lock_guard<std::mutex> g(e->mu);
    Layer::Tile& t = e->layers[layer].tile[bucket];
    t.pxw = (signed char)pxw; t.nbt = (signed char)nbt; t.ks = (signed char)ksplit;
    (void)hipSetDevice(e->device);
    (void)hipStreamSynchronize(e->compute);
    e->graphs.drop();
    return LTK_OK;
}

int ltk_wav2lip_time_layers(ltk_engine* e, int frames, int iters, float* ms_per_layer, int n_layers) {
    if (!e || frames <= 0 || iters <= 0 || !ms_per_layer) return fail(LTK_E_INVALID, "bad arguments");
    if (!e->loaded) return fail(LTK_E_STATE, "ltk_wav2lip_load has not been called");
    if (frames > e->micro_batch || frames > kPackMaxFrames) return fail(LTK_E_INVALID, "frames exceeds one arena pass");
    if (n_layers != (int)e->layers.size()) return fail(LTK_E_INVALID, "n_layers != ltk_wav2lip_layer_count");
    CHK(enter_device(e->device));
    std::lock_guard<std::mutex> g(e->mu);
    if (e->capture) return fail(LTK_E_STATE, "disable capture before timing");
    const bool fused = knob(K_HEAD_FUSED) != 0;
    TimingIO tio;
    int rc = tio.setup(e, frames);
    if (rc) return rc;
    const OutPtrs* d_outs = fused ? &e->d_tab->outs : nullptr;
    const FacePtrs* d_faces = e->c7 ? &e->d_tab->faces : nullptr;
    if ((rc = run_convs(e, frames, e->compute, d_outs, nullptr, d_faces))) return rc;
    return time_intervals(n_layers, iters, [&](std::vector<hipEvent_t>* evs) { return run_convs(e, frames, e->compute, d_outs, evs, d_faces); },
                          ms_per_layer);
}

namespace {
int conv2d_hook(ltk_engine* e, const void* d_x, int N, int H, int W, int Cin, const float* weight, int Cout, int kh, int kw, int sh, int sw,
                int ph, int pw, bool transposed, int out_pad, const float* scale, const float* shift, int quant, float act_scale,
                const void* d_res, int relu, int act, void* d_y, int iters, float* ms_avg) {
    if (!e || !d_x || !weight || !d_y) return fail(LTK_E_INVALID, "bad arguments");
    CHK(enter_device(e->device));
    ConvPlan plan;
    std::string err;
    int rc = conv_plan_create(&plan, weight, Cin, Cout, kh, kw, sh, sw, ph, pw, transposed, out_pad, scale, shift, &err, quant, act_scale);
    if (rc) return conv_status(rc, err);
    ConvIO io;
    io.partial = e->d_partial; io.partial_cap = e->partial_cap;
    io.x = (const f16*)d_x; io.N = N; io.H = H; io.W = W; io.x_ld = plan.Cin; io.x_coff = 0;
    io.y = (f16*)d_y; io.y_ld = Cout; io.y_coff = 0;
    io.res = (const f16*)d_res; io.res_ld = Cout; io.res_coff = 0;
    io.relu = relu; io.act = act;
    hipStream_t s = e->compute;
    std::lock_guard<std::mutex> g(e->mu);
    auto launch = [&]() -> int { const int lrc = conv_launch(plan, io, s, &err); return lrc ? conv_status(lrc, err) : 0; };
    rc = launch();
    if (!rc && iters > 0 && ms_avg) {
        float ms = 0.f;
        rc = time_iters(s, iters, launch, &ms);
        *ms_avg = ms / iters;
    }
    const hipError_t he = hipStreamSynchronize(s);
    conv_plan_destroy(&plan);
    if (rc) return rc;
    if (he != hipSuccess) return fail(LTK_E_HIP, std::string("conv kernel: ") + hipGetErrorString(he));
    return LTK_OK;
}
}

int ltk_conv2d_f16(ltk_engine* e, const void* d_x, int N, int H, int W, int Cin, const float* weight, int Cout, int kh, int kw, int sh, int sw,
                   int ph, int pw, int transposed, int out_pad, const float* scale, const float* shift, const void* d_res, int relu, void* d_y,
                   int iters, float* ms_avg) {
    return conv2d_hook(e, d_x, N, H, W, Cin, weight, Cout, kh, kw, sh, sw, ph, pw, transposed != 0, out_pad, scale, shift, 0, 1.f, d_res, relu, 0,
                       d_y, iters, ms_avg);
}

namespace {
struct ConvPlanOwner { ConvPlan p; ~ConvPlanOwner() { conv_plan_destroy(&p); } };
struct RowPlansOwner { RowGemmPlan p[4]; ~RowPlansOwner() { for (RowGemmPlan& q : p) rowgemm_plan_destroy(&q); } };
}

namespace {
struct ConvHookCall {
    int act = 0, x_ld = 0, y_ld = 0, res_ld = 0;
    int quant = 0;
    ConvIO io;
    int Ho = 0, Wo = 0;
};

void conv_report_copy(const ConvReport& cr, ltk_conv_report* rep) {
    memcpy(rep->kernel, cr.kernel, sizeof(rep->kernel));
    rep->G = cr.G; rep->NBT = cr.NBT; rep->PXW = cr.PXW; rep->NC8 = cr.NC8; rep->T = cr.T; rep->S = cr.S;
    rep->ksplit = cr.ksplit; rep->items = cr.items; rep->grid = cr.grid;
}

int conv_hook_plan(int N, int H, int W, int Cin, int Cout, int kh, int kw, int sh, int sw, int ph, int pw, int transposed, int out_pad, bool has_res,
                   int relu, int quant, const ltk_conv_opts* opts, ltk_conv_report* rep, ConvHookCall* c) {
    if (!opts || N <= 0 || H <= 0 || W <= 0 || Cin <= 0 || Cout <= 0 || quant < 0 || quant > 2) return fail(LTK_E_INVALID, "bad arguments");
    const ltk_conv_opts& o = *opts;
    if (o.family < 0 || o.family > 3 || o.act < 0 || o.act > 3 || o.ups < 0 || o.ups > 2 || (relu && o.act > 1)) return fail(LTK_E_INVALID, "bad options");
    if (quant && (o.family != 0 || o.ups != 0)) return fail(LTK_E_INVALID, "fp8 operands: the conv kernels (family 0) without an upsample");
    if (rep) { memset(rep, 0, sizeof(*rep)); rep->family = o.family; }
    c->quant = quant;
    const int act = c->act = relu ? 1 : o.act;
    const int CinP = quant ? Cin : Cin <= 8 ? 8 : (Cin + 15) / 16 * 16;
    const int x_ld = c->x_ld = o.x_ld ? o.x_ld : CinP, y_ld = c->y_ld = o.y_ld ? o.y_ld : Cout, res_ld = c->res_ld = o.res_ld ? o.res_ld : Cout;
    if (o.x_coff < 0 || o.y_coff < 0 || o.res_coff < 0 || o.x_coff + CinP > x_ld || o.y_coff + Cout > y_ld || (has_res && o.res_coff + Cout > res_ld))
        return fail(LTK_E_INVALID, "channel view outside its buffer");
    std::string err;
    if (o.family == 0) {
        ConvPlan plan;
        ConvRoute route;
        const int rc = conv_route(&plan, &route, Cin, Cout, kh, kw, sh, sw, ph, pw, transposed != 0, out_pad, quant, o.ups == 2 ? 1 : 0, conv_plan_knobs(), &err);
        if (rc) return conv_status(rc, err);
        if (quant && ((x_ld | o.x_coff) & 31)) return fail(LTK_E_INVALID, "fp8 operands: the view of x is given in multiples of 32 channels");
        const int xdiv = quant ? 2 : 1;
        if (o.ups == 2 && !plan.ups4) return fail(LTK_E_INVALID, "conv3: the four-phase upsample-conv serves 3x3 stride-1 pad-1 layers");
        static const f16 there = (f16)0.f;
        ConvReport cr;
        memset(&cr, 0, sizeof(cr));
        ConvIO& io = c->io;
        io = ConvIO();
        io.x = nullptr; io.N = N; io.H = H; io.W = W; io.x_ld = x_ld / xdiv; io.x_coff = o.x_coff / xdiv;
        io.y = nullptr; io.y_ld = y_ld; io.y_coff = o.y_coff;
        io.res = has_res ? &there : nullptr; io.res_ld = res_ld; io.res_coff = o.res_coff;
        io.relu = act == 1; io.act = act == 1 ? 0 : act;
        io.ups = o.ups ? 1 : 0;
        io.force_pxw = o.force_pxw; io.force_nbt = o.force_nbt; io.force_ksplit = o.force_ksplit;
        io.partial = const_cast<float*>(reinterpret_cast<const float*>(&there)); io.partial_cap = ~(size_t)0;
        io.report = &cr;
        const int lrc = conv_launch_dry(plan, io, &err);
        io.res = nullptr; io.partial = nullptr; io.partial_cap = 0; io.report = nullptr;
        if (lrc) return conv_status(lrc, err);
        if (rep) conv_report_copy(cr, rep);
        return LTK_OK;
    }
    if (act > 1 || o.ups || o.force_pxw || o.force_nbt || o.force_ksplit) return fail(LTK_E_INVALID, "the row kernels take no activation but ReLU, no upsample and no tile");
    if (Cin % 32 || Cout % 16) return fail(LTK_E_INVALID, "the row kernels need Cin % 32 == 0 and Cout % 16 == 0");
    if (o.family == 1) {
        if (transposed || kh != 1 || kw != 1 || H != 1 || W != 1 || has_res) return fail(LTK_E_INVALID, "rowgemm: a 1x1 conv on a one-pixel map, no residual");
        if (rep) { snprintf(rep->kernel, sizeof(rep->kernel), "rowgemm_kernel<%d>", rowgemm_ft(N)); rep->FT = rowgemm_ft(N); rep->UB = rowgemm_ub(rep->FT); rep->grid = Cout / 16; }
        return LTK_OK;
    }
    if (o.family == 2) {
// ... 633 lines not shown
```

livetalking_amd/csrc/engine_internal.h:

```cpp
#pragma once
#include <hip/hip_runtime.h>
#include <math.h>
#include <stdio.h>
#include <stdlib.h>
#include <string.h>

#include <algorithm>
#include <atomic>
#include <chrono>
#include <map>
#include <memory>
#include <mutex>
#include <string>
#include <vector>

#include "../../include/ltk.h"
#include "conv_mfma.h"
#include "dw_kernels.h"
#include "hubert_kernels.h"
#include "misc_kernels.h"
#include "musetalk.h"
#include "nn_kernels.h"
#include "state_dict.h"
#include "tune.h"

namespace ltk {

extern thread_local std::string g_err;
inline int fail(int code, const std::string& msg) { g_err = msg; return code; }
inline int conv_status(int rc, const std::string& err) { return fail(rc == -2 ? LTK_E_HIP : LTK_E_INVALID, err); }

inline hipError_t enter_device(int device) {
    (void)hipGetLastError();
    return hipSetDevice(device);
}

#define CHK(expr)                                                                        \
    do {                                                                                 \
        hipError_t _e = (expr);                                                          \
        if (_e != hipSuccess) return fail(LTK_E_HIP, std::string(#expr) + ": " + hipGetErrorString(_e)); \
    } while (0)

const int kDecCh[8] = {512, 512, 512, 512, 384, 256, 128, 64};
const int kFeatCh[8] = {16, 32, 64, 128, 256, 512, 512, 512};
const int kFeatHW[8] = {256, 128, 64, 32, 16, 8, 4, 1};
constexpr int kPrefetchMaxFrames = 32;
enum BufId { B_MEL = 0, B_AT0, B_AT1, B_X0, B_T0, B_T1, B_OUT32, B_CAT0, B_COUNT = B_CAT0 + 8 };

struct Layer {
    std::string name;
    ConvPlan plan;
    RowGemmPlan rg;
    int rg_y_ld = 0;
    bool rowconv = false;
    int rc_stride = 1, rc_stride_w = 0;
    RowGemmPlan rgT[4];
    int cin_real = 0;
    int in_buf = 0, in_ld = 0, in_coff = 0, H = 0, W = 0;
    int out_buf = 0, out_ld = 0, out_coff = 0, Ho = 0, Wo = 0;
    bool residual = false;
    bool res_folded = false;
    bool audio = false;
    int special = 0;
    ConvS2dPlan* s2d = nullptr;
    bool face_enc = false;
    double macs = 0;
    struct Tile { signed char pxw = 0, nbt = 0, ks = 0; } tile[5];
};

struct Avatar {
    uint8_t* d_face = nullptr;
    uint8_t* d_full = nullptr;
    std::vector<int32_t> coords;
    int n = 0, H = 0, W = 0;
    int device = 0;
    uint8_t* d_feat = nullptr;
    size_t feat_rec_bytes = 0;
    unsigned feat_epoch = 0;
    std::atomic<size_t> feat_bytes{0};
    Avatar() = default;
    Avatar(const Avatar&) = delete;
    Avatar& operator=(const Avatar&) = delete;
    ~Avatar() {
        (void)hipSetDevice(device);
        if (d_face) (void)hipFree(d_face);
        if (d_full) (void)hipFree(d_full);
        if (d_feat) (void)hipFree(d_feat);
    }
};

struct Scratch {
    void* d = nullptr;
    size_t cap = 0;
};

struct MtAvatar {
    float* d_latents = nullptr;
    uint8_t* d_full = nullptr;
    uint8_t* d_masks = nullptr;
    std::vector<int64_t> mask_off;
    std::vector<int32_t> face_box, crop_box;
    int n = 0, H = 0, W = 0;
    int device = 0;
    MtAvatar() = default;
    MtAvatar(const MtAvatar&) = delete;
    MtAvatar& operator=(const MtAvatar&) = delete;
    ~MtAvatar() {
        (void)hipSetDevice(device);
        if (d_latents) (void)hipFree(d_latents);
        if (d_full) (void)hipFree(d_full);
        if (d_masks) (void)hipFree(d_masks);
    }
};

struct UlProgram;
void ul_program_delete(UlProgram* p);
struct UlAvatar {
    UlProgram* prog = nullptr;
    uint8_t* d_face = nullptr;
    uint8_t* d_full = nullptr;
    std::vector<int32_t> boxes;
    int n = 0, H = 0, W = 0;
    int device = 0;
    int id = 0;
    UlAvatar() = default;
    UlAvatar(const UlAvatar&) = delete;
    UlAvatar& operator=(const UlAvatar&) = delete;
    ~UlAvatar() {
        (void)hipSetDevice(device);
        if (d_face) (void)hipFree(d_face);
        if (d_full) (void)hipFree(d_full);
        ul_program_delete(prog);
    }
};
constexpr int kUlBufs = 12;

struct Ev {
    hipEvent_t e = nullptr;
    hipError_t create() { return hipEventCreateWithFlags(&e, hipEventDisableTiming); }
    ~Ev() { if (e) (void)hipEventDestroy(e); }
};

constexpr size_t kMaxPassGraphs = 64;
struct PassGraph {
    hipGraphExec_t exec = nullptr;
    int seen = 0;
    unsigned long stamp = 0;
    hipStream_t stream = nullptr;
};

template <class Key>
struct GraphCache {
    std::map<Key, PassGraph> graphs;
    unsigned epoch = 0;
    hipStream_t side = nullptr;
    int live() const {
        int n = 0;
        for (auto& kv : graphs) n += kv.second.exec ? 1 : 0;
        return n;
    }
    void drop() {
        if (side) (void)hipStreamSynchronize(side);
        for (auto& kv : graphs)
            if (kv.second.exec) (void)hipGraphExecDestroy(kv.second.exec);
        graphs.clear();
    }
    template <class Enq>
    int run(ltk_engine* e, const Key& k, hipStream_t s, const char* what, int nf, Enq enq);
};

}

using namespace ltk;

struct ltk_engine {
    int device = 0;
    hipStream_t compute = nullptr;
    hipStream_t aux = nullptr;
    hipEvent_t ev_fork = nullptr, ev_join = nullptr;
    float* d_partial = nullptr;
    float* d_partial_aux = nullptr;
    float* d_partial_pf = nullptr;
    unsigned long long* d_sat = nullptr;
    size_t partial_cap = 0, partial_aux_cap = 0, partial_pf_cap = 0;
    std::mutex mu;
    std::mutex pool_mu;
    bool loaded = false;
    int max_frames = 0;
    int micro_batch = 0;
    std::vector<Layer> layers;
    f16* buf[B_COUNT] = {nullptr};
    struct PfSlot {
        f16* cat[B_COUNT] = {nullptr};
        bool valid = false;
        int avatar = -1, first = -1, nf = 0;
        unsigned epoch = 0;
        unsigned long stamp = 0;
        double filled_at = 0;
        hipEvent_t ev_done = nullptr;
        hipEvent_t ev_read = nullptr;
        bool filled = false, read = false;
        std::shared_ptr<Avatar> hold;
    };
    static constexpr int kPfSlots = 16;
    PfSlot pfs[kPfSlots + 1];
    f16* pf_tmp[B_COUNT] = {nullptr};
    int alt_frames = 0;
    hipStream_t aux2 = nullptr;
    unsigned long pf_clock = 0;
    DevTables* d_tab_next = nullptr;
    struct SoloSeq { int avatar = -1, next = -1, nf = 0; unsigned long stamp = 0; };
    SoloSeq solo_seq[2 * kPfSlots];
    unsigned long pf_hits = 0, pf_misses = 0, pf_issued = 0;
    std::atomic<bool> pf_fail_logged{false};
    double tm_prep = 0, tm_launch = 0, tm_pf = 0, tm_wait = 0;
    unsigned long tm_calls = 0;
    size_t buf_halfs[B_COUNT] = {0};
    float* d_head = nullptr;
    Conv7Plan* c7 = nullptr;
    Audio0Plan* a0 = nullptr;
    Audio3Plan* a3 = nullptr;
    double macs_per_frame = 0;
    DevTables* d_tab = nullptr;
    GraphCache<int> graphs;
    unsigned long graph_clock = 0;
    GraphCache<std::pair<const void*, int>> prog_graphs;
    bool capture = false;
    std::map<std::string, std::vector<float>> taps;
    std::map<std::string, std::vector<int>> tap_shape;
    std::map<int, std::shared_ptr<Avatar>> avatars;
    int next_avatar = 1;
    float* d_basis = nullptr;
    int32_t* d_lohi = nullptr;
    MtGraph* mt = nullptr;
    int mt_max_frames = 0;
    int mt_fp8 = 0;
    float mt_fp8_ascale = 8.f;
    MtGraph* vae_enc = nullptr;
    int vae_enc_faces = 0;
    MtGraph* whisper = nullptr;
    float* d_wbasis = nullptr;
    float* d_wlogspec = nullptr;
    float* d_wpcm = nullptr;
    int* d_wgmax = nullptr;
    float* d_pe = nullptr;
    float* d_mt_feat = nullptr;
    float* d_mt_lat = nullptr;
    std::map<int, std::shared_ptr<MtAvatar>> mt_avatars;
    MtGraph* hubert_w = nullptr;
    struct HubertProg { MtGraph* g = nullptr; int n_samples = 0; unsigned long stamp = 0; };
    std::vector<HubertProg> hubert_progs;
    MtGraph* hubert_last = nullptr;
    unsigned long hubert_clock = 0;
    float* d_hpcm = nullptr;
    size_t hpcm_cap = 0;
    float* d_hstats = nullptr;
    float* d_hrows = nullptr;
    size_t hrows_cap = 0;
    std::map<int, std::shared_ptr<UlAvatar>> ul_avatars;
    f16* ul_buf[kUlBufs] = {nullptr};
    int ul_frames = 0;
    DevTables* ul_tab = nullptr;
    std::vector<Scratch> scratch_free;
    std::vector<hipStream_t> stream_free;
};

namespace ltk {

struct ScratchLease {
    ltk_engine* e;
    Scratch s;
    ScratchLease(ltk_engine* e_, size_t bytes) : e(e_) {
        {
            std::lock_guard<std::mutex> g(e->pool_mu);
            for (size_t i = 0; i < e->scratch_free.size(); ++i)
                if (e->scratch_free[i].cap >= bytes) {
                    s = e->scratch_free[i];
                    e->scratch_free.erase(e->scratch_free.begin() + i);
                    break;
                }
        }
        if (!s.d) {
            size_t cap = bytes < (1u << 20) ? (1u << 20) : bytes;
            if (hipMalloc(&s.d, cap) == hipSuccess) s.cap = cap; else s.d = nullptr;
        }
    }
    ~ScratchLease() {
        if (s.d) {
            std::lock_guard<std::mutex> g(e->pool_mu);
            e->scratch_free.push_back(s);
        }
    }
};

struct StreamLease {
    ltk_engine* e;
    hipStream_t s = nullptr;
    bool owned = false;
    StreamLease(ltk_engine* e_, void* user) : e(e_) {
        if (user) { s = (hipStream_t)user; return; }
        owned = true;
        {
            std::lock_guard<std::mutex> g(e->pool_mu);
            if (!e->stream_free.empty()) { s = e->stream_free.back(); e->stream_free.pop_back(); }
        }
        if (!s) (void)hipStreamCreateWithFlags(&s, hipStreamNonBlocking);
    }
    ~StreamLease() {
        if (owned && s) {
            std::lock_guard<std::mutex> g(e->pool_mu);
            e->stream_free.push_back(s);
        }
    }
};

struct DevBuf {
    void* p = nullptr;
    ~DevBuf() { if (p) (void)hipFree(p); }
};

inline int mirror_index(int size, int index) {
    const int turn = index / size, res = index % size;
    return (turn % 2 == 0) ? res : size - res - 1;
}

template <class Key>
template <class Enq>
int GraphCache<Key>::run(ltk_engine* e, const Key& k, hipStream_t s, const char* what, int nf, Enq enq) {
    if (epoch != knob_epoch()) {
        CHK(hipStreamSynchronize(e->compute));
        drop();
        epoch = knob_epoch();
    }
    PassGraph& g = graphs[k];
    g.stamp = ++e->graph_clock;
    g.stream = s;
    if (g.exec) { CHK(hipGraphLaunch(g.exec, s)); return 0; }
    if (g.seen < 0 || g.seen++ == 0) return enq();
    if ((size_t)live() >= kMaxPassGraphs) {
        PassGraph* victim = nullptr;
        for (auto& kv : graphs)
            if (kv.second.exec && (!victim || kv.second.stamp < victim->stamp)) victim = &kv.second;
        (void)hipStreamSynchronize(e->compute);
        if (victim->stream != e->compute) (void)hipStreamSynchronize(victim->stream);
        (void)hipGraphExecDestroy(victim->exec); victim->exec = nullptr; victim->seen = 1;
    }
    hipGraph_t graph = nullptr;
    if (hipStreamBeginCapture(s, hipStreamCaptureModeRelaxed) != hipSuccess) { (void)hipGetLastError(); g.seen = -1; return enq(); }
    const int rc = enq();
    const hipError_t ce = hipStreamEndCapture(s, &graph);
    if (rc) {
        if (ce != hipSuccess) fprintf(stderr, "ltk: capture of the %d-frame %s aborted (%s)\n", nf, what, hipGetErrorString(ce));
        (void)hipGetLastError();
        if (graph) (void)hipGraphDestroy(graph);
        g.seen = -1;
        return rc;
    }
    hipGraphExec_t exec = nullptr;
    hipError_t ie = ce;
    if (ce == hipSuccess && graph) ie = hipGraphInstantiate(&exec, graph, nullptr, nullptr, 0);
    if (graph) (void)hipGraphDestroy(graph);
    if (ie != hipSuccess || !exec) {
        (void)hipGetLastError();
        g.seen = -1;
        fprintf(stderr, "ltk: hipGraph capture of the %d-frame %s failed (%s); running it as separate launches\n", nf, what, hipGetErrorString(ie));
        return enq();
    }
    g.exec = exec;
    CHK(hipGraphLaunch(exec, s));
    return 0;
}

template <class Enq>
int infer_call(ltk_engine* e, void* stream, Enq enq) {
    Ev done;
    CHK(done.create());
    int rc = 0;
    {
        std::lock_guard<std::mutex> g(e->mu);
        if (stream) {
            Ev ready;
            CHK(ready.create());
            CHK(hipEventRecord(ready.e, (hipStream_t)stream));
            CHK(hipStreamWaitEvent(e->compute, ready.e, 0));
        }
        rc = enq();
        if (!rc && hipEventRecord(done.e, e->compute) != hipSuccess) rc = fail(LTK_E_HIP, "hipEventRecord failed");
    }
    if (!rc) {
        if (stream && hipStreamWaitEvent((hipStream_t)stream, done.e, 0) != hipSuccess) rc = fail(LTK_E_HIP, "hipStreamWaitEvent failed");
        if (hipEventSynchronize(done.e) != hipSuccess) rc = fail(LTK_E_HIP, "hipEventSynchronize failed");
    } else {
        (void)hipStreamSynchronize(e->compute);
    }
    return rc;
}

inline std::shared_ptr<Avatar> find_avatar(ltk_engine* e, int id) {
    std::lock_guard<std::mutex> g(e->pool_mu);
    auto it = e->avatars.find(id);
    return it == e->avatars.end() ? nullptr : it->second;
}
inline std::shared_ptr<MtAvatar> find_mt_avatar(ltk_engine* e, int id) {
    std::lock_guard<std::mutex> g(e->pool_mu);
    auto it = e->mt_avatars.find(id);
    return it == e->mt_avatars.end() ? nullptr : it->second;
}

inline std::shared_ptr<UlAvatar> find_ul_avatar(ltk_engine* e, int id) {
    std::lock_guard<std::mutex> g(e->pool_mu);
    auto it = e->ul_avatars.find(id);
    return it == e->ul_avatars.end() ? nullptr : it->second;
}
inline void ul_fill_paste_batch(const UlAvatar& a, const int32_t* idx, int m, UlPasteBatch* pb) {
    const size_t bytes = (size_t)a.H * a.W * 3;
    for (int i = 0; i < m; ++i) {
        const int32_t* c = a.boxes.data() + 4 * (size_t)idx[i];
        pb->full[i] = a.d_full + (size_t)idx[i] * bytes;
        pb->face[i] = a.d_face + (size_t)idx[i] * kUlFace * kUlFace * 3;
        pb->x1[i] = c[0]; pb->y1[i] = c[1]; pb->x2[i] = c[2]; pb->y2[i] = c[3];
    }
}

void build_mel_basis(std::vector<float>* basis, std::vector<int32_t>* lohi, int n_bins = 401, double f_lo = 55.0, double f_hi = 7600.0);
int build_program(ltk_engine* e, const ltk_named_tensor* sd, int n);
void wav2lip_unload(ltk_engine* e);
int run_convs(ltk_engine* e, int nf, hipStream_t s, const OutPtrs* head_outs = nullptr, std::vector<hipEvent_t>* evs = nullptr,
              const FacePtrs* faces = nullptr, int part = 0, int par = 0, bool pf_enc = false);
int launch_pass(ltk_engine* e, int nf, hipStream_t s, bool bank_faces, const float* d_face6, bool have_outs, float* d_pred_f32,
                bool cached = false, int par = 0, bool have_feats = false);
int launch_prefetch(ltk_engine* e, int nf, int slot);
int run_program(ltk_engine* e, MtGraph* prog, int nf);
int ul_pass(ltk_engine* e, UlAvatar& a, int nf, bool bank, const float* d_img6, bool u8_out, float* d_pred_f32);
double ul_macs_per_frame(const UlAvatar& a);
void ul_drop_graphs(ltk_engine* e, int avatar_id);
void ul_unload(ltk_engine* e);
constexpr size_t kHubertPrograms = 3;
MtGraph* hubert_program(ltk_engine* e, int n_samples, int* rc);
void hubert_unload(ltk_engine* e);
int mt_run_locked(ltk_engine* e, const float* d_feat, const PtrList64* feat_ptrs, int nf, const OutList64* outs, float* d_image_f32);

}
```

livetalking_amd/csrc/tune.h:

```cpp
#pragma once

namespace ltk {

#define LTK_KNOBS(X) \
    X(CONV_V3, 1)               \
    X(CONV_PXW, 0)              \
    X(CONV3_NBT, 0)             \
    X(CONV3_NC8, 0)             \
    X(SPLITK, 1)                \
    X(KSPLIT, 0)                \
    X(MICROBATCH, 0)            \
    X(HEAD_FUSED, 1)            \
    X(TILE_TABLE, 1)            \
    X(ROWGEMM, 1)               \
    X(ROWCONV, 1024)            \
    X(ABLATE, 0)                \
    X(GRAPH, 1)                 \
    X(DF_FRAMES, 0)             \
    X(DF_BLOCK, 6)              \
    X(DF_MIN, 32)               \
    X(FACE_CACHE, 0)            \
    X(PREFETCH, 1)              \
    X(MT_FUSE, 7)               \
    X(MT_GN1, 1)                \
    X(SAT_CHECK, 0)             \
    X(FACE_CACHE_MAX_MB, 16384)  \
    X(LIN_FK, 1)                \
    X(ATTN_LDS, 1)              \
    X(LIN_MP, 1)                \
    X(GN_COOP, 1)               \
    X(AUDIO0, 3)                \
    X(CONV_S2D, 1)


enum Knob {
#define LTK_KNOB_ENUM(name, dflt) K_##name,
    LTK_KNOBS(LTK_KNOB_ENUM)
#undef LTK_KNOB_ENUM
    K_COUNT
};

int knob(Knob k);
unsigned knob_epoch();
int ensure_dyn_lds(const void* func, int bytes);

int knob_set(const char* name, int value);

}
```

livetalking_amd/csrc/w2l_infer.hip:

```cpp
#include "engine_internal.h"

static FeatGeom feat_geom(ltk_engine* e) {
    FeatGeom g;
    unsigned off = 0;
    for (int k = 0; k < 8; ++k) {
        const int cat = B_CAT0 + (7 - k), hw = kFeatHW[k] * kFeatHW[k];
        g.cat[k] = e->buf[cat] + (size_t)(kDecCh[7 - k] / 16) * hw * 16;
        g.cat_stride[k] = (unsigned)e->buf_halfs[cat];
        g.off[k] = off;
        off += (unsigned)((size_t)kFeatCh[k] * hw * sizeof(f16) / 16);
    }
    g.off[8] = off;
    return g;
}

static int enqueue_pass(ltk_engine* e, int nf, hipStream_t s, bool bank_faces, const float* d_face6, bool fused, bool have_outs,
                        float* d_pred_f32, bool cached = false, int par = 0, bool have_feats = false) {
    const FacePtrs* d_faces = &e->d_tab->faces;
    const OutPtrs* d_outs = &e->d_tab->outs;
    const bool pack_fused = bank_faces && e->c7;
    if (cached) launch_feat_copy(d_faces, nf, feat_geom(e), 0, s);
    else if (have_feats) {}
    else if (bank_faces) { if (!pack_fused) launch_pack_faces(d_faces, nf, e->buf[B_X0], s); }
    else launch_pack_face6_nchw(d_face6, nf, e->buf[B_X0], s);
    if (!(e->a0 && (knob(K_AUDIO0) & 1))) launch_pack_mel(&e->d_tab->mels, nf, e->buf[B_MEL], s);
    const int rc = run_convs(e, nf, s, fused ? d_outs : nullptr, nullptr, (pack_fused && !cached && !have_feats) ? d_faces : nullptr,
                             (cached || have_feats) ? 2 : 0, par);
    if (rc) return rc;
    if (!fused) {
        launch_head(e->buf[B_OUT32], 32, nf, e->d_head, e->d_head + 96, have_outs ? d_outs : nullptr, d_pred_f32, s);
        CHK(hipGetLastError());
    }
    return 0;
}

static int pass_graph_key(int nf, bool cached, bool have_feats, bool prefetch, int slot) {
    return nf | (cached ? (1 << 20) : 0) | (have_feats ? (1 << 21) : 0) | (prefetch ? (1 << 22) : 0) | (slot << 24);
}

int ltk::launch_pass(ltk_engine* e, int nf, hipStream_t s, bool bank_faces, const float* d_face6, bool have_outs, float* d_pred_f32, bool cached, int par,
                     bool have_feats) {
    const bool fused = have_outs && !d_pred_f32 && !e->capture && knob(K_HEAD_FUSED) && !knob(K_SAT_CHECK);
    const bool graphable = knob(K_GRAPH) && bank_faces && fused && e->c7 && s == e->compute;
    if (!graphable) {
        const bool product = bank_faces && fused && e->c7 && s == e->compute;
        if ((par || have_feats) && !product) return fail(LTK_E_STATE, "pipelined pass outside the product configuration");
        return enqueue_pass(e, nf, s, bank_faces, d_face6, fused, have_outs, d_pred_f32, cached && bank_faces, par, have_feats);
    }
    return e->graphs.run(e, pass_graph_key(nf, cached, have_feats, false, par), s, "pass", nf,
                         [&]() -> int { return enqueue_pass(e, nf, s, bank_faces, d_face6, fused, have_outs, d_pred_f32, cached, par, have_feats); });
}

int ltk::launch_prefetch(ltk_engine* e, int nf, int slot) {
    hipStream_t s = e->aux2;
    ltk_engine::PfSlot& sl = e->pfs[slot];
    if (sl.read) CHK(hipStreamWaitEvent(s, sl.ev_read, 0));
    auto enq = [&]() -> int { return run_convs(e, nf, s, nullptr, nullptr, &e->d_tab_next->faces, 1, slot, true); };
    const int rc = knob(K_GRAPH) ? e->graphs.run(e, pass_graph_key(nf, false, false, true, slot), s, "prefetch", nf, enq) : enq();
    CHK(hipEventRecord(sl.ev_done, s));
    sl.filled = true;
    return rc;
}

static int build_face_cache(ltk_engine* e, Avatar& a) {
    const FeatGeom g = feat_geom(e);
    const size_t rec = (size_t)g.off[8] * 16;
    if (!a.d_feat) {
        const size_t budget = (size_t)std::max(0, knob(K_FACE_CACHE_MAX_MB)) << 20;
        if (rec * a.n > budget)
            return fail(LTK_E_NOMEM, "face cache of this avatar needs " + std::to_string((rec * a.n) >> 20) + " MB, over LTK_FACE_CACHE_MAX_MB = " +
                                         std::to_string(knob(K_FACE_CACHE_MAX_MB)));
        if (hipMalloc((void**)&a.d_feat, rec * a.n) != hipSuccess) { (void)hipGetLastError(); return fail(LTK_E_NOMEM, "face-cache allocation failed"); }
        a.feat_rec_bytes = rec;
        a.feat_bytes.store(rec * a.n, std::memory_order_release);
    }
    const int chunk = std::min(std::min(16, a.n), std::min(e->micro_batch, kPackMaxFrames));
    const bool pack_fused = e->c7;
    for (int f0 = 0; f0 < a.n; f0 += chunk) {
        const int first = std::min(f0, a.n - chunk);
        FacePtrs fp;
        for (int i = 0; i < chunk; ++i) fp.p[i] = a.d_face + (size_t)(first + i) * 256 * 256 * 3;
        launch_upload_tables(&fp, nullptr, nullptr, chunk, e->d_tab, e->compute);
        if (!pack_fused) launch_pack_faces(&e->d_tab->faces, chunk, e->buf[B_X0], e->compute);
        const int rc = run_convs(e, chunk, e->compute, nullptr, nullptr, pack_fused ? &e->d_tab->faces : nullptr, 1);
        if (rc) return rc;
        for (int i = 0; i < chunk; ++i) fp.p[i] = a.d_feat + (size_t)(first + i) * rec;
        launch_upload_tables(&fp, nullptr, nullptr, chunk, e->d_tab, e->compute);
        launch_feat_copy(&e->d_tab->faces, chunk, g, 1, e->compute);
        CHK(hipGetLastError());
    }
    a.feat_epoch = knob_epoch();
    return 0;
}

extern "C" {

int ltk_avatar_face_cache_bytes(ltk_engine* e, int avatar_id, size_t* bytes) {
    if (!e || !bytes) return fail(LTK_E_INVALID, "bad arguments");
    const std::shared_ptr<Avatar> ap = find_avatar(e, avatar_id);
    if (!ap) return fail(LTK_E_STATE, "unknown avatar id");
    *bytes = ap->feat_bytes.load(std::memory_order_acquire);
    return LTK_OK;
}

int ltk_wav2lip_infer(ltk_engine* e, const ltk_w2l_req* reqs, int nreq, void* stream) {
    if (!e || !reqs || nreq <= 0) return fail(LTK_E_INVALID, "bad arguments");
    if (!e->loaded) return fail(LTK_E_STATE, "ltk_wav2lip_load has not been called");
    static const bool timing = getenv("LTK_INFER_TIMING") != nullptr;
    const auto tp0 = std::chrono::steady_clock::now();
    auto tp1 = tp0, tp2 = tp0, tp3 = tp0;
    CHK(enter_device(e->device));
    const bool want_cache = knob(K_FACE_CACHE) != 0;
    std::vector<int> fidx;
    std::vector<const uint8_t*> fptr;
    std::vector<const float*> mptr;
    std::vector<uint8_t*> optr;
    std::vector<std::shared_ptr<Avatar>> hold;
    for (int r = 0; r < nreq; ++r) {
        hold.push_back(find_avatar(e, reqs[r].avatar));
        if (!hold.back()) return fail(LTK_E_STATE, "unknown avatar id");
        if (reqs[r].batch <= 0 || reqs[r].index < 0 || !reqs[r].d_mel || !reqs[r].d_pred) return fail(LTK_E_INVALID, "bad request");
        const Avatar& a = *hold.back();
        for (int i = 0; i < reqs[r].batch; ++i) {
            const int idx = mirror_index(a.n, reqs[r].index + i);
            fptr.push_back(a.d_face + (size_t)idx * 256 * 256 * 3);
            if (want_cache) { fidx.push_back(r); fidx.push_back(idx); }
            mptr.push_back((const float*)reqs[r].d_mel + (size_t)i * 80 * 16);
            optr.push_back((uint8_t*)reqs[r].d_pred + (size_t)i * 65536 * 3);
        }
    }
    const int total = (int)fptr.size();
    if (total > e->max_frames) return fail(LTK_E_INVALID, "more frames than max_frames given to ltk_wav2lip_load");
    const int rc = infer_call(e, stream, [&]() -> int {
        int rc = 0;
        const int mbs = std::min(e->micro_batch, kPackMaxFrames);
        const bool cached = want_cache && !e->capture && knob(K_HEAD_FUSED);
        if (cached) {
            for (auto& ap : hold)
                if (!rc && (!ap->d_feat || ap->feat_epoch != knob_epoch())) rc = build_face_cache(e, *ap);
            if (!rc)
                for (int i = 0; i < total; ++i) fptr[i] = hold[fidx[2 * i]]->d_feat + (size_t)fidx[2 * i + 1] * hold[fidx[2 * i]]->feat_rec_bytes;
        } else if (!want_cache) {
            for (auto& ap : hold)
                if (ap->d_feat) {
                    CHK(hipStreamSynchronize(e->compute));
                    (void)hipFree(ap->d_feat);
                    ap->d_feat = nullptr;
                    ap->feat_bytes.store(0, std::memory_order_release);
                }
        }
        const bool solo = nreq == 1 && !cached && knob(K_PREFETCH) && e->alt_frames > 0 && total <= std::min(e->alt_frames, mbs) &&
                          !e->capture && knob(K_HEAD_FUSED) && e->c7;
        const int first = reqs[0].index;
        int slot = 0;
        if (solo)
            for (int k = 1; k <= ltk_engine::kPfSlots && !slot; ++k) {
                const ltk_engine::PfSlot& sl = e->pfs[k];
                if (sl.valid && sl.avatar == reqs[0].avatar && sl.first == first && sl.nf == total && sl.epoch == knob_epoch()) slot = k;
            }
        const bool hit = slot > 0;
        ltk_engine::SoloSeq* seq_rec = nullptr;
        if (solo)
            for (ltk_engine::SoloSeq& q : e->solo_seq)
                if (q.avatar == reqs[0].avatar && q.next == first && q.nf == total) { seq_rec = &q; break; }
        const bool prefetch = solo && (hit || seq_rec != nullptr);
        const int par = slot;
        if (solo) { if (hit) ++e->pf_hits; else ++e->pf_misses; }
        if (hit) {
            CHK(hipStreamWaitEvent(e->compute, e->pfs[slot].ev_done, 0));
            e->pfs[slot].valid = false;
            e->pfs[slot].stamp = ++e->pf_clock;
        }
        if (timing) tp1 = std::chrono::steady_clock::now();
        for (int f0 = 0; f0 < total && !rc; f0 += mbs) {
            const int nf = std::min(mbs, total - f0);
            FacePtrs fp; MelPtrs mp; OutPtrs op;
            for (int i = 0; i < nf; ++i) { fp.p[i] = fptr[f0 + i]; mp.p[i] = mptr[f0 + i]; op.p[i] = optr[f0 + i]; }
            launch_upload_tables(hit ? nullptr : &fp, &mp, &op, nf, e->d_tab, e->compute);
            if (hipGetLastError() != hipSuccess) rc = fail(LTK_E_HIP, "pointer table upload failed");
            else rc = launch_pass(e, nf, e->compute, true, nullptr, true, nullptr, cached, par, hit);
        }
        if (hit) {
            if (hipEventRecord(e->pfs[slot].ev_read, e->compute) != hipSuccess) { if (!rc) rc = fail(LTK_E_HIP, "hipEventRecord failed"); }
            else e->pfs[slot].read = true;
        }
        if (timing) tp2 = std::chrono::steady_clock::now();
        if (!rc && prefetch) {
            constexpr double kPfStale = 1.5;
            const double now = std::chrono::duration<double>(std::chrono::steady_clock::now().time_since_epoch()).count();
            int victim = 0, busy = 0;
            for (int k = 1; k <= ltk_engine::kPfSlots; ++k) {
                if (k == slot) continue;
                const ltk_engine::PfSlot& sl = e->pfs[k];
                if (sl.valid && now - sl.filled_at < kPfStale) continue;
                if (sl.read && hipEventQuery(sl.ev_read) != hipSuccess) { if (!busy || sl.stamp > e->pfs[busy].stamp) busy = k; continue; }
                if (!victim || sl.stamp > e->pfs[victim].stamp) victim = k;
            }
            (void)hipGetLastError();
            if (!victim) victim = busy;
            if (victim) {
            ltk_engine::PfSlot& sl = e->pfs[victim];
            sl.valid = false;
            FacePtrs nx;
            const Avatar& a = *hold[0];
            for (int i = 0; i < total; ++i) nx.p[i] = a.d_face + (size_t)mirror_index(a.n, first + total + i) * 256 * 256 * 3;
            sl.hold = hold[0];
            launch_upload_tables(&nx, nullptr, nullptr, total, e->d_tab_next, e->aux2);
            if (launch_prefetch(e, total, victim) == 0) {
                ++e->pf_issued;
                sl.valid = true; sl.avatar = reqs[0].avatar; sl.first = first + total; sl.nf = total; sl.epoch = knob_epoch();
                sl.stamp = ++e->pf_clock;
                sl.filled_at = now;
            } else {
                (void)hipGetLastError();
                if (!e->pf_fail_logged.exchange(true))
                    fprintf(stderr, "ltk: prefetch of %d frames could not be launched (%s); such calls run whole passes\n", total, g_err.c_str());
            }
            }
        }
        if (!rc && solo) {
            if (!seq_rec) {
                seq_rec = &e->solo_seq[0];
                for (ltk_engine::SoloSeq& q : e->solo_seq) if (q.stamp < seq_rec->stamp) seq_rec = &q;
            }
            seq_rec->avatar = reqs[0].avatar; seq_rec->next = first + total; seq_rec->nf = total; seq_rec->stamp = ++e->pf_clock;
        }
        if (timing) tp3 = std::chrono::steady_clock::now();
        return rc;
    });
    if (timing) {
        const auto tp4 = std::chrono::steady_clock::now();
        auto us = [](std::chrono::steady_clock::time_point a, std::chrono::steady_clock::time_point b) { return std::chrono::duration<double, std::micro>(b - a).count(); };
        std::lock_guard<std::mutex> g(e->pool_mu);
        e->tm_prep += us(tp0, tp1); e->tm_launch += us(tp1, tp2); e->tm_pf += us(tp2, tp3); e->tm_wait += us(tp3, tp4); ++e->tm_calls;
    }
    return rc;
}

}
```

livetalking_amd/csrc/w2l_program.hip:

```cpp
#include "engine_internal.h"

namespace {

struct LayerDef {
    const char* prefix;
    bool transposed;
    int cin, cout, k, sh, sw, pad, out_pad;
    bool residual;
};

const LayerDef kAudio[] = {
    {"audio_encoder.0", false, 1, 32, 3, 1, 1, 1, 0, false},
    {"audio_encoder.1", false, 32, 32, 3, 1, 1, 1, 0, true},
    {"audio_encoder.2", false, 32, 32, 3, 1, 1, 1, 0, true},
    {"audio_encoder.3", false, 32, 64, 3, 3, 1, 1, 0, false},
    {"audio_encoder.4", false, 64, 64, 3, 1, 1, 1, 0, true},
    {"audio_encoder.5", false, 64, 64, 3, 1, 1, 1, 0, true},
    {"audio_encoder.6", false, 64, 128, 3, 3, 3, 1, 0, false},
    {"audio_encoder.7", false, 128, 128, 3, 1, 1, 1, 0, true},
    {"audio_encoder.8", false, 128, 128, 3, 1, 1, 1, 0, true},
    {"audio_encoder.9", false, 128, 256, 3, 3, 2, 1, 0, false},
    {"audio_encoder.10", false, 256, 256, 3, 1, 1, 1, 0, true},
    {"audio_encoder.11", false, 256, 512, 3, 1, 1, 0, 0, false},
    {"audio_encoder.12", false, 512, 512, 1, 1, 1, 0, 0, false},
// ... 90 lines not shown
        if (t.pxw == 4 && d->cout > 32) complain("512-pixel tiles exist for <= 32 output channels only");
        if (t.nbt == 2 && d->cout < 64) complain("64-cout blocks need >= 64 output channels");
        if (d->k == 7) complain("the first layer runs on conv7, not conv3");
        for (size_t j = 0; j < i; ++j)
            if (!strcmp(kTileTable[j].layer, t.layer) && kTileTable[j].bucket == t.bucket) complain("duplicate entry");
    }
    return bad;
}

void apply_tile_table_impl(std::vector<Layer>& layers) {
    for (const TileEntry& t : kTileTable)
        for (Layer& L : layers)
            if (L.name == t.layer) { L.tile[t.bucket].pxw = (signed char)t.pxw; L.tile[t.bucket].nbt = (signed char)t.nbt; L.tile[t.bucket].ks = (signed char)t.ks; }
}


int build_layer_impl(ltk_engine* e, const LayerDef& d, const ltk_named_tensor* sd, int n, Layer* L, int hint_hw, int flat_ld, int map_w) {
    const std::string p = d.prefix;
    const size_t wcount = (size_t)d.cin * d.cout * d.k * d.k;
    SD dict{sd, n, ""};
    const float* w = dict.get(p + ".conv_block.0.weight", wcount);
    const float* b = dict.get(p + ".conv_block.0.bias", d.cout);
    const float* g = dict.get(p + ".conv_block.1.weight", d.cout);
    const float* beta = dict.get(p + ".conv_block.1.bias", d.cout);
    const float* mean = dict.get(p + ".conv_block.1.running_mean", d.cout);
    const float* var = dict.get(p + ".conv_block.1.running_var", d.cout);
    if (!w || !b || !g || !beta || !mean || !var)
        return fail(LTK_E_INVALID, "state_dict is missing (or has a wrong shape for) tensors of layer " + p);
    std::vector<float> sc(d.cout), sf(d.cout);
    fold_bn(g, beta, mean, var, b, kBnEps, d.cout, sc.data(), sf.data());
    std::string err;
    int rc;
    std::vector<float> wfold;
    L->res_folded = false;
    if (d.residual && !d.transposed && d.cin == d.cout && (d.k & 1) && d.sh == 1 && d.sw == 1 && d.pad == d.k / 2) {
        bool ok = true;
        for (int c = 0; c < d.cout; ++c) ok = ok && fabsf(sc[c]) >= 1e-3f;
        if (ok) {
            wfold.assign(w, w + wcount);
            const int kk = d.k * d.k, ctr = (d.k / 2) * d.k + d.k / 2;
            for (int c = 0; c < d.cout; ++c) wfold[((size_t)c * d.cin + c) * kk + ctr] += 1.0f / sc[c];
            w = wfold.data();
            L->res_folded = true;
        }
    }
    if (flat_ld > 0) {
        const int kk = d.k * d.k;
        const int cin_flat = kk * d.cin;
        std::vector<float> wf((size_t)d.cout * cin_flat, 0.f);
        for (int co = 0; co < d.cout; ++co)
            for (int ci = 0; ci < d.cin; ++ci)
                for (int t = 0; t < kk; ++t)
                    wf[(size_t)co * cin_flat + ((size_t)(ci >> 4) * kk + t) * 16 + (ci & 15)] = w[((size_t)co * d.cin + ci) * kk + t];
        rc = conv_plan_create(&L->plan, wf.data(), cin_flat, d.cout, 1, 1, 1, 1, 0, 0, false, 0, sc.data(), sf.data(), &err);
    } else {
        rc = conv_plan_create(&L->plan, w, d.cin, d.cout, d.k, d.k, d.sh, d.sw, d.pad, d.pad, d.transposed, d.out_pad,
                              sc.data(), sf.data(), &err);
    }
    if (rc) return conv_status(rc, p + ": " + err);
    const bool want_rowgemm = knob(K_ROWGEMM) && knob(K_SPLITK), want_rowconv = knob(K_ROWCONV) > 0 && knob(K_SPLITK);
    {
        std::vector<float> we, se, fe;
        int J = 0, K = 0;
        if (flat_ld > 0) {
            const int kk = d.k * d.k;
            J = d.cout; K = kk * d.cin;
            we.assign((size_t)J * K, 0.f);
            for (int co = 0; co < d.cout; ++co)
                for (int ci = 0; ci < d.cin; ++ci)
                    for (int t = 0; t < kk; ++t)
                        we[(size_t)co * K + ((size_t)(ci >> 4) * kk + t) * 16 + (ci & 15)] = w[((size_t)co * d.cin + ci) * kk + t];
            se = sc; fe = sf;
        } else if (!d.transposed && d.k == 1 && hint_hw == 1 && d.cin % 32 == 0 && d.cout % 16 == 0) {
            J = d.cout; K = d.cin;
            we.assign(w, w + (size_t)J * K);
            se = sc; fe = sf;
        } else if (d.transposed && hint_hw == 1 && d.sh == 1 && d.pad == 0 && d.out_pad == 0 && d.cin % 32 == 0 && d.cout % 16 == 0) {
            const int kk = d.k * d.k;
            J = kk * d.cout; K = d.cin;
            we.assign((size_t)J * K, 0.f); se.assign(J, 0.f); fe.assign(J, 0.f);
            for (int j = 0; j < J; ++j) {
                const int c16 = j & 15, tt = j >> 4, pos = tt % kk, co = (tt / kk) * 16 + c16;
                for (int ci = 0; ci < d.cin; ++ci) we[(size_t)j * K + ci] = w[((size_t)ci * d.cout + co) * kk + pos];
                se[j] = sc[co]; fe[j] = sf[co];
            }
        }
        if (J > 0 && !want_rowgemm) {
        } else if (J > 0) {
            rc = rowgemm_plan_create(&L->rg, we.data(), J, K, se.data(), fe.data(), &err);
            if (rc) return conv_status(rc, p + ": " + err);
            L->rg_y_ld = (d.transposed ? J : 0);
        } else if (want_rowconv && flat_ld == 0 && !d.transposed && d.k == 3 && d.pad == 1 && (d.cout % 256 == 0 || (map_w < 0 && d.cout == 128)) &&
                   ((map_w > 0 && d.sh == d.sw && (d.sh == 1 || d.sh == 2) && map_w % d.sh == 0 && map_w / d.sh <= 8 && (d.cin == 256 || d.cin == 512)) ||
                    (map_w < 0 && d.cin % 32 == 0))) {
            J = d.cout; K = 9 * d.cin;
            rowconv_weff(w, d.cin, d.cout, &we);
            rc = rowgemm_plan_create(&L->rg, we.data(), J, K, sc.data(), sf.data(), &err);
            if (rc) return conv_status(rc, p + ": " + err);
            L->rowconv = true;
            L->rc_stride = d.sh;
            L->rc_stride_w = d.sw;
        } else if (want_rowconv && map_w > 0 && map_w <= 8 && d.transposed && d.k == 3 && d.sh == 2 && d.sw == 2 && d.pad == 1 && d.out_pad == 1 &&
                   (d.cin == 256 || d.cin == 512 || d.cin == 1024) && d.cout % 256 == 0) {
            for (int gph = 0; gph < 4; ++gph) {
                J = d.cout; K = (1 + (gph >> 1)) * (1 + (gph & 1)) * d.cin;
                rowconvT_weff(w, d.cin, d.cout, gph, &we);
                rc = rowgemm_plan_create(&L->rgT[gph], we.data(), J, K, sc.data(), sf.data(), &err);
                if (rc) return conv_status(rc, p + ": " + err);
            }
        }
    }
    if (!d.transposed && d.k == 7 && d.cin == 6 && d.cout == 16 && d.sh == 1 && d.pad == 3 && !e->c7) {
        rc = conv7_plan_create(&e->c7, w, sc.data(), sf.data(), &err);
        if (rc) return fail(LTK_E_HIP, p + ": " + err);
    }
    if (!d.transposed && d.k == 3 && d.cin == 1 && d.cout == 32 && d.sh == 1 && d.sw == 1 && d.pad == 1 && !d.residual && (knob(K_AUDIO0) & 1) && !e->a0) {
        rc = audio0_plan_create(&e->a0, w, sc.data(), sf.data(), &err);
        if (rc) return fail(LTK_E_HIP, p + ": " + err);
    }
    if (!d.transposed && d.k == 3 && d.cin == 32 && d.cout == 64 && d.sh == 3 && d.sw == 1 && d.pad == 1 && !d.residual && (knob(K_AUDIO0) & 2) && !e->a3) {
        rc = audio3_plan_create(&e->a3, w, sc.data(), sf.data(), &err);
        if (rc) return fail(LTK_E_HIP, p + ": " + err);
        L->special = 3;
    }
    if (!d.transposed && d.k == 3 && d.sh == 2 && d.sw == 2 && d.pad == 1 && !d.residual && (d.cin == 16 || d.cin == 32) && d.cout % 32 == 0 &&
        knob(K_CONV_S2D) && !L->s2d) {
        rc = convs2d_plan_create(&L->s2d, w, d.cin, d.cout, sc.data(), sf.data(), &err);
        if (rc) return conv_status(rc, p + ": " + err);
    }
    L->name = p;
    L->cin_real = d.cin;
    L->residual = d.residual;
    return 0;
}


int build_layer(ltk_engine* e, const LayerDef& d, const ltk_named_tensor* sd, int n, Layer* L, int hint_hw = 0, int flat_ld = 0, int map_w = 0) {
    const int rc = build_layer_impl(e, d, sd, n, L, hint_hw, flat_ld, map_w);
    if (rc) {
        conv_plan_destroy(&L->plan); rowgemm_plan_destroy(&L->rg);
        for (RowGemmPlan& q : L->rgT) rowgemm_plan_destroy(&q);
        convs2d_plan_destroy(L->s2d); L->s2d = nullptr;
    }
    return rc;
}

void bump(size_t* cur, size_t v) { if (v > *cur) *cur = v; }

}

namespace ltk {

void wav2lip_unload(ltk_engine* e) {
    if (e->aux2) (void)hipStreamSynchronize(e->aux2);
    e->graphs.drop();
    if (e->d_tab) { (void)hipFree(e->d_tab); e->d_tab = nullptr; }
    for (Layer& L : e->layers) {
        conv_plan_destroy(&L.plan); rowgemm_plan_destroy(&L.rg);
        for (RowGemmPlan& q : L.rgT) rowgemm_plan_destroy(&q);
        convs2d_plan_destroy(L.s2d); L.s2d = nullptr;
    }
    e->layers.clear();
    for (int i = 0; i < B_COUNT; ++i) {
        if (e->buf[i]) { (void)hipFree(e->buf[i]); e->buf[i] = nullptr; }
        if (e->pf_tmp[i]) { (void)hipFree(e->pf_tmp[i]); e->pf_tmp[i] = nullptr; }
        for (ltk_engine::PfSlot& sl : e->pfs)
            if (sl.cat[i]) { (void)hipFree(sl.cat[i]); sl.cat[i] = nullptr; }
    }
    for (ltk_engine::PfSlot& sl : e->pfs) {
        if (sl.ev_done) (void)hipEventDestroy(sl.ev_done);
        if (sl.ev_read) (void)hipEventDestroy(sl.ev_read);
        sl = ltk_engine::PfSlot();
    }
    e->alt_frames = 0;
    for (ltk_engine::SoloSeq& q : e->solo_seq) q = ltk_engine::SoloSeq();
    if (e->d_tab_next) { (void)hipFree(e->d_tab_next); e->d_tab_next = nullptr; }
    if (e->d_head) { (void)hipFree(e->d_head); e->d_head = nullptr; }
    conv7_plan_destroy(e->c7);
    e->c7 = nullptr;
    audio0_plan_destroy(e->a0);
    e->a0 = nullptr;
    audio3_plan_destroy(e->a3);
    e->a3 = nullptr;
    e->loaded = false;
}

int build_program(ltk_engine* e, const ltk_named_tensor* sd, int n) {
    wav2lip_unload(e);
    size_t* bh = e->buf_halfs;
    for (int i = 0; i < B_COUNT; ++i) bh[i] = 0;
    bh[B_MEL] = 80 * 16 * 8;
    bh[B_X0] = 65536 * 8;
    bh[B_OUT32] = 65536 * 32;
    for (int k = 0; k < 8; ++k) {
        const int hw = kFeatHW[7 - k];
        bh[B_CAT0 + k] = (size_t)hw * hw * (kDecCh[k] + kFeatCh[7 - k]);
    }
    int rc;
    {
        int H = 80, W = 16, in_buf = B_MEL, in_ld = 8, pp = 0;
        for (const LayerDef& d : kAudio) {
            Layer L;
            const bool flat = !d.transposed && d.pad == 0 && d.k > 1 && d.k == H && d.k == W && d.cin % 64 == 0;
            const int oh = (H + 2 * d.pad - d.k) / d.sh + 1, ow = (W + 2 * d.pad - d.k) / d.sw + 1;
            constexpr int kAudioRowconvMaxPixels = 54;
            const bool small = !flat && d.k == 3 && d.pad == 1 && oh * ow <= kAudioRowconvMaxPixels && d.cin % 32 == 0;
            if ((rc = build_layer(e, d, sd, n, &L, H * W, flat ? in_ld : 0, small ? -1 : 0))) return rc;
            L.audio = true;
            L.in_buf = in_buf; L.in_ld = in_ld; L.in_coff = 0; L.H = H; L.W = W;
            if (flat) { L.Ho = 1; L.Wo = 1; L.H = 1; L.W = 1; L.in_ld = d.k * d.k * in_ld; }
            else
            L.plan.out_dims(H, W, &L.Ho, &L.Wo);
            L.out_buf = B_AT0 + pp; L.out_ld = d.cout; L.out_coff = 0;
            bump(&bh[L.out_buf], (size_t)L.Ho * L.Wo * d.cout);
            L.macs = (double)d.cin * d.cout * d.k * d.k * L.Ho * L.Wo;
            e->layers.push_back(L);
            in_buf = L.out_buf; in_ld = d.cout; H = L.Ho; W = L.Wo; pp ^= 1;
        }
    }
    const int audio_emb_buf = e->layers.back().out_buf;
    {
        int H = 256, W = 256, in_buf = B_X0, in_ld = 8, in_coff = 0, pp = 0;
        const int nl = (int)(sizeof(kFaceEnc) / sizeof(kFaceEnc[0]));
        for (int li = 0; li < nl; ++li) {
            const BlockLayer& bl = kFaceEnc[li];
            const bool last = (li + 1 == nl) || kFaceEnc[li + 1].block != bl.block;
            Layer L;
            const bool flat = !bl.d.transposed && bl.d.pad == 0 && bl.d.k > 1 && bl.d.k == H && bl.d.k == W && bl.d.cin % 64 == 0;
            if ((rc = build_layer(e, bl.d, sd, n, &L, H * W, flat ? in_ld : 0, H == W ? W : 0))) return rc;
            L.in_buf = in_buf; L.in_ld = in_ld; L.in_coff = in_coff; L.H = H; L.W = W;
            if (flat) {
                L.Ho = 1; L.Wo = 1;
                L.H = 1; L.W = 1;
                L.in_ld = bl.d.k * bl.d.k * in_ld; L.in_coff = bl.d.k * bl.d.k * in_coff;
            } else {
                L.plan.out_dims(H, W, &L.Ho, &L.Wo);
            }
            if (last) {
                const int k = 7 - bl.block;
                L.out_buf = B_CAT0 + k; L.out_ld = kDecCh[k] + kFeatCh[bl.block]; L.out_coff = kDecCh[k];
                if (L.Ho != kFeatHW[bl.block] || bl.d.cout != kFeatCh[bl.block]) return fail(LTK_E_INVALID, "encoder geometry mismatch");
            } else {
                L.out_buf = B_T0 + pp; L.out_ld = bl.d.cout; L.out_coff = 0; pp ^= 1;
                bump(&bh[L.out_buf], (size_t)L.Ho * L.Wo * bl.d.cout);
            }
            L.macs = (double)bl.d.cin * bl.d.cout * bl.d.k * bl.d.k * L.Ho * L.Wo;
            L.face_enc = true;
            e->layers.push_back(L);
            in_buf = L.out_buf; in_ld = L.out_ld; in_coff = L.out_coff; H = L.Ho; W = L.Wo;
        }
    }
    {
        int H = 1, W = 1, in_buf = audio_emb_buf, in_ld = 512, in_coff = 0, pp = 0;
        const int nl = (int)(sizeof(kFaceDec) / sizeof(kFaceDec[0]));
        for (int li = 0; li < nl; ++li) {
            const BlockLayer& bl = kFaceDec[li];
            const bool last = (li + 1 == nl) || kFaceDec[li + 1].block != bl.block;
            Layer L;
            if ((rc = build_layer(e, bl.d, sd, n, &L, H * W, 0, H == W ? W : 0))) return rc;
            L.in_buf = in_buf; L.in_ld = in_ld; L.in_coff = in_coff; L.H = H; L.W = W;
            L.plan.out_dims(H, W, &L.Ho, &L.Wo);
            if (last) {
                const int k = bl.block;
                L.out_buf = B_CAT0 + k; L.out_ld = kDecCh[k] + kFeatCh[7 - k]; L.out_coff = 0;
                if (L.Ho != kFeatHW[7 - k] || bl.d.cout != kDecCh[k]) return fail(LTK_E_INVALID, "decoder geometry mismatch");
            } else {
                L.out_buf = B_T0 + pp; L.out_ld = bl.d.cout; L.out_coff = 0; pp ^= 1;
                bump(&bh[L.out_buf], (size_t)L.Ho * L.Wo * bl.d.cout);
            }
            if (bl.d.transposed) L.macs = (double)bl.d.cin * bl.d.cout * bl.d.k * bl.d.k * H * W;
            else L.macs = (double)bl.d.cin * bl.d.cout * bl.d.k * bl.d.k * L.Ho * L.Wo;
            e->layers.push_back(L);
            in_buf = L.out_buf; in_ld = L.out_ld; in_coff = L.out_coff; H = L.Ho; W = L.Wo;
        }
    }
    {
        Layer L;
        if ((rc = build_layer(e, kOutConv, sd, n, &L, 65536))) return rc;
        L.in_buf = B_CAT0 + 7; L.in_ld = 80; L.in_coff = 0; L.H = 256; L.W = 256; L.Ho = 256; L.Wo = 256;
        L.out_buf = B_OUT32; L.out_ld = 32; L.out_coff = 0;
        L.macs = 80.0 * 32 * 9 * 65536;
        e->layers.push_back(L);
    }
    SD dict{sd, n, ""};
    const float* hw = dict.get("output_block.1.weight", 96);
    const float* hb = dict.get("output_block.1.bias", 3);
    if (!hw || !hb) return fail(LTK_E_INVALID, "state_dict is missing output_block.1.{weight,bias}");
    std::vector<float> h(99);
    memcpy(h.data(), hw, 96 * sizeof(float));
    memcpy(h.data() + 96, hb, 3 * sizeof(float));
    CHK(hipMalloc((void**)&e->d_head, 99 * sizeof(float)));
    CHK(hipMemcpy(e->d_head, h.data(), 99 * sizeof(float), hipMemcpyHostToDevice));
    e->macs_per_frame = 32.0 * 3 * 65536;
    for (const Layer& L : e->layers) e->macs_per_frame += L.macs;
    apply_tile_table_impl(e->layers);
    return 0;
}

int run_convs(ltk_engine* e, int nf, hipStream_t s, const OutPtrs* head_outs, std::vector<hipEvent_t>* evs, const FacePtrs* faces, int part, int par,
              bool pf_enc) {
    auto B = [&](int id) -> f16* {
        if (id >= B_CAT0) return par ? e->pfs[par].cat[id] : e->buf[id];
        if (pf_enc && (id == B_X0 || id == B_T0 || id == B_T1)) return e->pf_tmp[id];
        return e->buf[id];
    };
    std::string err;
// ... 177 lines not shown
```

livetalking_amd/engine.py:

```python
from __future__ import annotations

import ctypes as C
import threading
from typing import Dict, Optional, Sequence

import numpy as np

from . import _lib
from ._lib import LtkError, MtReq, NamedTensor, UlReq, W2lReq


def _as_f32(a) -> np.ndarray:
    if hasattr(a, "detach"):
        a = a.detach().cpu().numpy()
    return np.ascontiguousarray(a, dtype=np.float32)


def _conv_report_dict(rep: "_lib.ConvReport") -> dict:
    out = {name: getattr(rep, name) for name, _ in _lib.ConvReport._fields_}
    out["kernel"] = rep.kernel.decode()
    return out


class Engine:

    def __init__(self, device: int = 0):
        self._lib = _lib.load()
        h = C.c_void_p()
        _lib.check(self._lib.ltk_engine_create(int(device), C.byref(h)))
        self._h = h
        self.device = int(device)
        self.max_frames = 0
        self._closed = False
        self._lock = threading.Lock()
        self._egress_open = set()

    def close(self):
        if not self._closed:
            self._closed = True
            for sched in list(self.__dict__.get("_ltk_schedulers", {}).values()):
                try:
                    sched.close()
                except Exception:
                    pass
            self.__dict__.pop("_ltk_schedulers", None)
            for sess in list(self._egress_open):
                try:
                    self.egress_close(sess)
                except Exception:
                    pass
            h, self._h = self._h, None
            self._lib.ltk_engine_destroy(h)

    def __del__(self):
        try:
            self.close()
        except Exception:
            pass

    def sync(self):
        _lib.check(self._lib.ltk_engine_sync(self._h))

    @property
    def torch_device(self):
        import torch
        return torch.device("cuda", self.device)

    @staticmethod
    def _named_tensors(state_dict: Dict[str, object]):
        keep = []
        arr = (NamedTensor * len(state_dict))()
        n = 0
        for name, t in state_dict.items():
            if name.endswith("num_batches_tracked"):
                continue
            a = _as_f32(t)
            shape = (C.c_int64 * max(a.ndim, 1))(*a.shape)
            nm = name.encode()
            keep.append((a, shape, nm))
            arr[n].name = nm
            arr[n].data = a.ctypes.data_as(C.POINTER(C.c_float))
            arr[n].ndim = a.ndim
            arr[n].shape = shape
            n += 1
        return arr, n, keep

    def load_wav2lip(self, state_dict: Dict[str, object], max_frames: int = 16):
        arr, n, keep = self._named_tensors(state_dict)
        _lib.check(self._lib.ltk_wav2lip_load(self._h, arr, n, int(max_frames)))
        self.max_frames = int(max_frames)
        del keep

    def load_musetalk(self, unet_sd: Dict[str, object], vae_sd: Dict[str, object], max_frames: int = 16, fp8: bool = False,
                      fp8_act_scale: float = 0.0):
        if fp8:
            _lib.check(self._lib.ltk_musetalk_set_fp8(self._h, 1, float(fp8_act_scale)))
        ua, un, k1 = self._named_tensors(unet_sd)
        va, vn, k2 = self._named_tensors(vae_sd)
        _lib.check(self._lib.ltk_musetalk_load(self._h, ua, un, va, vn, int(max_frames)))
        self.mt_max_frames = int(max_frames)
        del k1, k2

    def register_avatar(self, face_list: Sequence[np.ndarray], frame_list: Sequence[np.ndarray],
                        coord_list: Sequence[Sequence[int]]) -> int:
        faces = getattr(face_list, "packed", None)
        fulls = getattr(frame_list, "packed", None)
        faces = np.ascontiguousarray(np.stack(face_list) if faces is None else faces, dtype=np.uint8)
        fulls = np.ascontiguousarray(np.stack(frame_list) if fulls is None else fulls, dtype=np.uint8)
        coords = np.ascontiguousarray(np.asarray(coord_list, dtype=np.int32).reshape(-1, 4))
        n = faces.shape[0]
        if faces.shape[1:] != (256, 256, 3) or fulls.shape[0] != n or coords.shape[0] != n or fulls.shape[3] != 3:
            raise ValueError("avatar bank shapes: faces (n,256,256,3), frames (n,H,W,3), coords (n,4)")
        aid = C.c_int()
        _lib.check(self._lib.ltk_avatar_register(self._h, faces.ctypes.data, fulls.ctypes.data, coords.ctypes.data,
                                                 n, fulls.shape[1], fulls.shape[2], C.byref(aid)))
        return aid.value

    def release_avatar(self, avatar_id: int):
        _lib.check(self._lib.ltk_avatar_release(self._h, int(avatar_id)))

    def mel_step(self, pcm: np.ndarray, win_start: Sequence[int], d_out_ptr: int, stream: int = 0):
        pcm = np.ascontiguousarray(pcm, dtype=np.float32)
        ws = np.ascontiguousarray(win_start, dtype=np.int32)
        _lib.check(self._lib.ltk_mel_step(self._h, pcm.ctypes.data, pcm.shape[0], ws.ctypes.data, ws.shape[0],
                                          C.c_void_p(d_out_ptr), C.c_void_p(stream)))

    def wav2lip_infer(self, reqs: Sequence[tuple], stream: int = 0):
        arr = (W2lReq * len(reqs))()
        for i, (aid, index, batch, mel_ptr, pred_ptr) in enumerate(reqs):
            arr[i].avatar = int(aid)
            arr[i].index = int(index)
            arr[i].batch = int(batch)
            arr[i].d_mel = C.c_void_p(mel_ptr)
            arr[i].d_pred = C.c_void_p(pred_ptr)
        _lib.check(self._lib.ltk_wav2lip_infer(self._h, arr, len(reqs), C.c_void_p(stream)))

    def paste_back(self, avatar_id: int, idx: int, d_pred_ptr: int, out: np.ndarray, stream: int = 0):
        _lib.check(self._lib.ltk_paste_back(self._h, int(avatar_id), int(idx), C.c_void_p(d_pred_ptr),
                                            out.ctypes.data, 0, C.c_void_p(stream)))

    def paste_back_batch(self, avatar_id: int, idx: Sequence[int], d_pred_ptr: int, out_ptr: int, stream: int = 0):
        arr = np.ascontiguousarray(np.asarray(idx, dtype=np.int32))
        _lib.check(self._lib.ltk_paste_back_batch(self._h, int(avatar_id), arr.ctypes.data, C.c_void_p(d_pred_ptr), int(arr.size),
                                                  C.c_void_p(out_ptr), C.c_void_p(stream)))

    def paste_back_device(self, avatar_id: int, idx: int, d_pred_ptr: int, d_out_ptr: int, stream: int = 0):
        _lib.check(self._lib.ltk_paste_back(self._h, int(avatar_id), int(idx), C.c_void_p(d_pred_ptr),
                                            C.c_void_p(d_out_ptr), 1, C.c_void_p(stream)))

    def register_musetalk_avatar(self, latents: Sequence[np.ndarray], frame_list: Sequence[np.ndarray], coord_list,
                                 mask_list: Sequence[np.ndarray], mask_coords_list) -> int:
        lat = np.ascontiguousarray(np.concatenate([_as_f32(x).reshape(1, 8, 32, 32) for x in latents]), dtype=np.float32)
        fulls = getattr(frame_list, "packed", None)
        fulls = np.ascontiguousarray(np.stack(frame_list) if fulls is None else fulls, dtype=np.uint8)
        fb = np.ascontiguousarray(np.asarray(coord_list, dtype=np.int32).reshape(-1, 4))
        cb = np.ascontiguousarray(np.asarray(mask_coords_list, dtype=np.int32).reshape(-1, 4))
        n = lat.shape[0]
        flat = [np.ascontiguousarray(m, dtype=np.uint8).reshape(-1) for m in mask_list]
        offs = np.zeros(n + 1, dtype=np.int64)
        offs[1:] = np.cumsum([f.size for f in flat])
        masks = np.ascontiguousarray(np.concatenate(flat))
        aid = C.c_int()
        _lib.check(self._lib.ltk_musetalk_avatar_register(self._h, lat.ctypes.data, fulls.ctypes.data, fb.ctypes.data, cb.ctypes.data,
                                                          masks.ctypes.data, offs.ctypes.data, n, fulls.shape[1], fulls.shape[2],
                                                          C.byref(aid)))
        return aid.value

    def musetalk_infer(self, reqs: Sequence[tuple], stream: int = 0):
        arr = (MtReq * len(reqs))()
        for i, (aid, index, batch, feat_ptr, pred_ptr) in enumerate(reqs):
            arr[i].avatar = int(aid); arr[i].index = int(index); arr[i].batch = int(batch)
            arr[i].d_feat = C.c_void_p(feat_ptr); arr[i].d_pred = C.c_void_p(pred_ptr)
        _lib.check(self._lib.ltk_musetalk_infer(self._h, arr, len(reqs), C.c_void_p(stream)))

    def paste_blend(self, avatar_id: int, idx: int, d_pred_ptr: int, out: np.ndarray, stream: int = 0):
        _lib.check(self._lib.ltk_paste_blend(self._h, int(avatar_id), int(idx), C.c_void_p(d_pred_ptr), out.ctypes.data, 0,
                                             C.c_void_p(stream)))

    def register_ultralight_avatar(self, state_dict: Dict[str, object], face_list: Sequence[np.ndarray], frame_list: Sequence[np.ndarray],
                                   coord_list, max_frames: int = 16) -> int:
        faces = np.ascontiguousarray(np.stack(face_list), dtype=np.uint8)
        fulls = getattr(frame_list, "packed", None)
        fulls = np.ascontiguousarray(np.stack(frame_list) if fulls is None else fulls, dtype=np.uint8)
        coords = np.ascontiguousarray(np.asarray(coord_list, dtype=np.int32).reshape(-1, 4))
        n = faces.shape[0]
        if faces.shape[1:] != (168, 168, 3) or fulls.ndim != 4 or fulls.shape[0] != n or coords.shape[0] != n or fulls.shape[3] != 3:
            raise ValueError("ultralight avatar bank shapes: faces (n,168,168,3), frames (n,H,W,3), coords (n,4)")
        arr, nt, keep = self._named_tensors(state_dict)
        aid = C.c_int()
        _lib.check(self._lib.ltk_ultralight_avatar_register(self._h, arr, nt, faces.ctypes.data, fulls.ctypes.data, coords.ctypes.data,
                                                            n, fulls.shape[1], fulls.shape[2], int(max_frames), C.byref(aid)))
        del keep
        return aid.value

    def ultralight_infer(self, reqs: Sequence[tuple], stream: int = 0):
        arr = (UlReq * len(reqs))()
        for i, (aid, index, batch, feat_ptr, pred_ptr) in enumerate(reqs):
            arr[i].avatar = int(aid); arr[i].index = int(index); arr[i].batch = int(batch)
            arr[i].d_feat = C.c_void_p(feat_ptr); arr[i].d_pred = C.c_void_p(pred_ptr)
        _lib.check(self._lib.ltk_ultralight_infer(self._h, arr, len(reqs), C.c_void_p(stream)))

    def ultralight_paste_back(self, avatar_id: int, idx: int, d_pred_ptr: int, out: np.ndarray, stream: int = 0):
        _lib.check(self._lib.ltk_ultralight_paste_back(self._h, int(avatar_id), int(idx), C.c_void_p(d_pred_ptr), out.ctypes.data, 0,
                                                       C.c_void_p(stream)))

    def ultralight_paste_back_batch(self, avatar_id: int, idx: Sequence[int], d_pred_ptr: int, out_ptr: int, stream: int = 0):
        arr = np.ascontiguousarray(np.asarray(idx, dtype=np.int32))
        _lib.check(self._lib.ltk_ultralight_paste_back_batch(self._h, int(avatar_id), arr.ctypes.data, C.c_void_p(d_pred_ptr),
                                                             int(arr.size), C.c_void_p(out_ptr), C.c_void_p(stream)))

    def ultralight_forward_host(self, avatar_id: int, img6: np.ndarray, feat: np.ndarray) -> np.ndarray:
        img6 = np.ascontiguousarray(img6, dtype=np.float32)
        B = img6.shape[0]
        feat = np.ascontiguousarray(feat, dtype=np.float32).reshape(B, 16, 32, 32)
        assert img6.shape[1:] == (6, 160, 160)
        pred = np.empty((B, 3, 160, 160), dtype=np.float32)
        _lib.check(self._lib.ltk_ultralight_forward_host(self._h, int(avatar_id), img6.ctypes.data, feat.ctypes.data, B, pred.ctypes.data))
        return pred

    def ultralight_ops(self, avatar_id: int):
        out = []
        buf = C.create_string_buffer(160)
        t = C.c_int()
        for i in range(self._lib.ltk_ultralight_op_count(self._h, int(avatar_id))):
            _lib.check(self._lib.ltk_ultralight_op_name(self._h, int(avatar_id), i, buf, 160, C.byref(t)))
            out.append((buf.value.decode(), t.value))
        return out

    def ultralight_time(self, avatar_id: int, frames: int, iters: int):
        ms = C.c_float()
        macs = C.c_double()
        _lib.check(self._lib.ltk_ultralight_time(self._h, int(avatar_id), int(frames), int(iters), C.byref(ms), C.byref(macs)))
        return ms.value, macs.value

    def dwconv3x3_f16(self, d_x_ptr: int, N, H, W, C_, weight: np.ndarray, stride: int = 1, scale=None, shift=None, relu: bool = True,
                      d_y_ptr: int = 0):
        w = np.ascontiguousarray(weight, dtype=np.float32)
        sc = np.ascontiguousarray(scale, dtype=np.float32) if scale is not None else None
        sf = np.ascontiguousarray(shift, dtype=np.float32) if shift is not None else None
        _lib.check(self._lib.ltk_dwconv3x3_f16(self._h, C.c_void_p(d_x_ptr), N, H, W, C_, w.ctypes.data, int(stride),
                                               sc.ctypes.data if sc is not None else None, sf.ctypes.data if sf is not None else None,
                                               1 if relu else 0, C.c_void_p(d_y_ptr)))

    def upsample2x_cat_f16(self, d_x_ptr: int, N, h, w, C_up, d_skip_ptr: int, Hs, Ws, C_skip, d_y_ptr: int):
        _lib.check(self._lib.ltk_upsample2x_cat_f16(self._h, C.c_void_p(d_x_ptr), N, h, w, C_up, C.c_void_p(d_skip_ptr), Hs, Ws, C_skip,
                                                    C.c_void_p(d_y_ptr)))

    def egress_open(self, H: int, W: int) -> int:
        h = C.c_void_p()
        _lib.check(self._lib.ltk_egress_open(self._h, int(H), int(W), C.byref(h)))
        with self._lock:
            self._egress_open.add(h.value)
        return h.value

    def egress_close(self, session: int) -> None:
        with self._lock:
            if not self._h or session not in self._egress_open:
                return
            self._egress_open.discard(session)
        _lib.check(self._lib.ltk_egress_close(self._h, C.c_void_p(session)))

    def egress_watermark(self, session: int, mask, x: int = 0, y: int = 0, color=(128, 128, 128)) -> None:
        if mask is None:
            _lib.check(self._lib.ltk_egress_watermark(self._h, C.c_void_p(session), None, 0, 0, 0, 0, 0, 0, 0))
            return
        mask = np.ascontiguousarray(mask, dtype=np.uint8)
        _lib.check(self._lib.ltk_egress_watermark(self._h, C.c_void_p(session), mask.ctypes.data, int(x), int(y), mask.shape[1],
                                                  mask.shape[0], int(color[0]), int(color[1]), int(color[2])))

    def egress_frame(self, session: int, out: np.ndarray, source: int, avatar_id: int = 0, idx: int = 0, d_pred_ptr: int = 0,
                     h_frame: np.ndarray = None, speaking: bool = True, alpha: float = -1.0, keep: bool = False, fmt: int = 0,
                     chroma: int = 1, stream: int = 0) -> np.ndarray:
        req = _lib.EgressReq(int(source), int(avatar_id), int(idx), C.c_void_p(d_pred_ptr or None),
                             C.c_void_p(h_frame.ctypes.data if h_frame is not None else None), int(bool(speaking)), float(alpha),
                             int(bool(keep)), int(fmt), int(chroma))
        _lib.check(self._lib.ltk_egress_frame(self._h, C.c_void_p(session), C.byref(req), out.ctypes.data, C.c_void_p(stream)))
        return out

    def egress_batch(self, session: int, source: int, avatar_id: int, idx: Sequence[int], d_pred_ptr: int, out_ptr: int, fmt: int = 0,
                     chroma: int = 1, stream: int = 0) -> None:
        arr = np.ascontiguousarray(np.asarray(idx, dtype=np.int32))
        _lib.check(self._lib.ltk_egress_batch(self._h, C.c_void_p(session), int(source), int(avatar_id), arr.ctypes.data,
                                              C.c_void_p(d_pred_ptr), int(arr.size), int(fmt), int(chroma), C.c_void_p(out_ptr),
                                              C.c_void_p(stream)))

    def musetalk_forward_host(self, latents: np.ndarray, feat: np.ndarray, want_image=True, want_frames=True):
        latents = np.ascontiguousarray(latents, dtype=np.float32).reshape(-1, 8, 32, 32)
        feat = np.ascontiguousarray(feat, dtype=np.float32).reshape(-1, 50, 384)
# ... 357 lines not shown
```

livetalking_amd/scheduler.py:

```python
from __future__ import annotations

import collections
import os
import threading
import time


class _Req:
    __slots__ = ("args", "batch", "done", "err")

    def __init__(self, args, batch):
        self.args, self.batch = args, batch
        self.done = threading.Event()
        self.err = None


class BatchingScheduler:

    def __init__(self, engine, kind: str = "wav2lip", window_ms: float = 0.0, max_frames: int = 0):
        self.engine = engine
        self.kind = kind
        self._call = engine.wav2lip_infer if kind == "wav2lip" else engine.musetalk_infer
        self.window = max(0.0, float(window_ms)) * 1e-3
        self._max_frames = int(max_frames)
        self._cv = threading.Condition()
        self._pending = collections.deque()
        self._inflight = 0
        self._inflight_frames = 0
        self._lead_frac = max(0.0, float(os.environ.get("LTK_INFLIGHT_LEAD_FRAC", "0.1")))
        self._max_inflight = max(1, int(os.environ.get("LTK_INFLIGHT", "2")))
        self._lead = max(0.0, float(os.environ.get("LTK_INFLIGHT_LEAD_US", "300"))) * 1e-6
        self._spf = None
        self._busy_until = 0.0
        self._last_done = 0.0
        self._leader_hold = False
        self._closed = False
        self._workers = []
        self._idle_exit = max(0.05, float(os.environ.get("LTK_WORKER_IDLE_S", "5")))
        self._auto_window = max(0.0, float(os.environ.get("LTK_COALESCE_AUTO_US", "200"))) * 1e-6
        self._last_multi = -1e9
        self.stats = {"calls": 0, "requests": 0, "frames": 0, "max_requests_per_call": 0, "overlapped_calls": 0}

    def _limit(self) -> int:
        if self._max_frames > 0:
            return self._max_frames
        lim = getattr(self.engine, "max_frames" if self.kind == "wav2lip" else "mt_max_frames", 0)
        return int(lim) if lim else 1 << 30

    def infer(self, aid, index, batch, in_ptr, out_ptr):
        batch = int(batch)
        with self._cv:
            solo = (self._inflight == 0 and not self._pending and self.window <= 0.0 and
                    (self._auto_window <= 0.0 or time.perf_counter() - self._last_multi >= 2.0))
            if solo:
                self._inflight += 1
                self._inflight_frames += batch
                if self._spf is not None:
                    self._busy_until = time.perf_counter() + batch * self._spf
        if solo:
            return self._run_solo((aid, index, batch, in_ptr, out_ptr), batch)
        r = _Req((aid, index, batch, in_ptr, out_ptr), batch)
        with self._cv:
            self._pending.append(r)
            leader = self._inflight == 0 and len(self._pending) == 1
            if leader:
                self._inflight += 1
                self._leader_hold = True
            else:
                self._ensure_workers()
                self._cv.notify_all()
        if leader:
            if self.window > 0.0:
                time.sleep(self.window)
            elif self._auto_window > 0.0 and time.perf_counter() - self._last_multi < 2.0:
                time.sleep(self._auto_window)
            self._run_one_batch(alone=True)
        r.done.wait()
        if r.err is not None:
            raise r.err

    def _run_solo(self, args, frames):
        t0 = time.perf_counter()
        err = None
        try:
            self._call([args])
        except Exception as ex:
            err = ex
        t1 = time.perf_counter()
        with self._cv:
            self._inflight -= 1
            st = self.stats
            st["calls"] += 1
            st["requests"] += 1
            st["frames"] += frames
            if st["max_requests_per_call"] < 1:
                st["max_requests_per_call"] = 1
            if err is None and frames > 0:
                spf = (t1 - max(t0, self._last_done)) / frames
                self._spf = spf if self._spf is None else 0.75 * self._spf + 0.25 * spf
            self._last_done = t1
            self._inflight_frames -= frames
            self._busy_until = t1 + (self._inflight_frames * self._spf if self._spf is not None else 0.0)
            if self._pending:
                self._ensure_workers()
                self._cv.notify_all()
        if err is not None:
            raise err

    def _ensure_workers(self):
        self._workers = [w for w in self._workers if w.is_alive()]
        while len(self._workers) < self._max_inflight:
            w = threading.Thread(target=self._work, name="ltk-batch", daemon=True)
            self._workers.append(w)
            w.start()

    def _take_batch(self):
        group, frames, lim = [], 0, self._limit()
        while self._pending and (not group or frames + self._pending[0].batch <= lim):
            q = self._pending.popleft()
            group.append(q)
            frames += q.batch
        return group, frames

    def _run_one_batch(self, alone: bool):
        with self._cv:
            if alone:
                self._leader_hold = False
            group, frames = self._take_batch()
            if alone and self._pending:
                self._ensure_workers()
                self._cv.notify_all()
            now = time.perf_counter()
            self._inflight_frames += frames
            if self._spf is not None:
                self._busy_until = max(now, self._busy_until) + frames * self._spf
            if not alone:
                self.stats["overlapped_calls"] += 1
        t0 = time.perf_counter()
        errs = [None] * len(group)
        if group:
            try:
                self._call([q.args for q in group])
            except Exception as ex:
                if len(group) == 1:
                    errs[0] = ex
                else:
                    for i, q in enumerate(group):
                        try:
                            self._call([q.args])
                        except Exception as ex_i:
                            errs[i] = ex_i
        t1 = time.perf_counter()
        with self._cv:
            self._inflight -= 1
            if group:
                self.stats["calls"] += 1
                self.stats["requests"] += len(group)
                self.stats["frames"] += frames
                self.stats["max_requests_per_call"] = max(self.stats["max_requests_per_call"], len(group))
                if len(group) > 1:
                    self._last_multi = t1
                if frames > 0 and all(e is None for e in errs):
                    spf = (t1 - max(t0, self._last_done)) / frames
                    self._spf = spf if self._spf is None else 0.75 * self._spf + 0.25 * spf
            self._last_done = t1
            self._inflight_frames -= frames
            self._busy_until = t1 + (self._inflight_frames * self._spf if self._spf is not None else 0.0)
            if self._pending:
                self._ensure_workers()
            self._cv.notify_all()
        for q, err in zip(group, errs):
            q.err = err
            q.done.set()

    def _work(self):
        me = threading.current_thread()
        while True:
            with self._cv:
                idle_since = time.perf_counter()
                while True:
                    if self._closed:
                        if me in self._workers:
                            self._workers.remove(me)
                        return
                    now = time.perf_counter()
                    if self._pending and not self._leader_hold:
                        if self._inflight == 0:
                            break
                        if self._inflight < self._max_inflight and self._spf is not None:
                            lead = max(self._lead, self._lead_frac * self._inflight_frames * self._spf)
                            wait_t = self._busy_until - lead - now
                            if wait_t <= 0.0:
                                break
                            self._cv.wait(timeout=wait_t)
                            continue
                        self._cv.wait()
                        idle_since = time.perf_counter()
                        continue
                    if now - idle_since >= self._idle_exit:
                        if me in self._workers:
                            self._workers.remove(me)
                        return
                    self._cv.wait(timeout=self._idle_exit)
                alone = self._inflight == 0
                self._inflight += 1
            self._run_one_batch(alone=alone)

    def close(self):
        with self._cv:
            self._closed = True
            dropped = list(self._pending)
            self._pending.clear()
            workers = list(self._workers)
            self._cv.notify_all()
        for q in dropped:
            q.err = RuntimeError("scheduler closed")
            q.done.set()
        for w in workers:
            if w is not threading.current_thread():
                w.join(timeout=5.0)
        with self._cv:
            self._workers = [w for w in self._workers if w.is_alive()]
            self._closed = False
            if self._pending:
                self._ensure_workers()
                self._cv.notify_all()


class CoalescingScheduler(BatchingScheduler):
    def __init__(self, engine, window_ms: float, kind: str = "wav2lip"):
        super().__init__(engine, kind, window_ms)


_LOCK = threading.Lock()


def get_scheduler(engine, kind: str = "wav2lip"):
    with _LOCK:
        table = engine.__dict__.setdefault("_ltk_schedulers", {})
        s = table.get(kind)
        if s is None:
            s = BatchingScheduler(engine, kind, float(os.environ.get("LTK_COALESCE_MS", "0")))
            table[kind] = s
        return s
```

Before: 13380 frames/s.

## Defer wav2lip inference completion sync and order consumers via stream events

Adds a deferred inference path in which ltk_wav2lip_infer returns without waiting for the device. Outstanding passes are tracked in a DeferWindow of events and held buffers, and any consumer of the prediction buffer (paste-back, egress, torch ops through a FrameHandle tensor subclass) first orders its stream behind the pending pass. The aim is to remove the per-call host wait so the next batch's host work and launch can overlap the previous pass. In exchange it adds event bookkeeping, a torch_function hook on every frame op, and a risk of ordering bugs, and prefetch slot choice now avoids slots still in flight.

```diff
diff --git a/include/ltk.h b/include/ltk.h
--- a/include/ltk.h
+++ b/include/ltk.h
@@ -48,6 +48,11 @@
                  int n_win, void* d_out, void* stream);
 
 int ltk_wav2lip_infer(ltk_engine* e, const ltk_w2l_req* reqs, int nreq, void* stream);
+
+#define LTK_DEFER_SYNC 2
+int ltk_wav2lip_infer_deferred(ltk_engine* e, const ltk_w2l_req* reqs, int nreq, void* stream, int flags, int* deferred);
+int ltk_wav2lip_order_stream(ltk_engine* e, const void* d_pred, size_t bytes, void* stream);
+int ltk_wav2lip_defer_stats(ltk_engine* e, unsigned long long* deferred, unsigned long long* max_outstanding, unsigned long long* outstanding);
 
 int ltk_paste_back(ltk_engine* e, int avatar_id, int idx, const void* d_pred, void* out,
                    int out_is_device, void* stream);
@@ -188,6 +193,8 @@
 
 int ltk_wav2lip_prefetch_stats(ltk_engine* e, unsigned long long* hits, unsigned long long* misses, unsigned long long* issued);
 
+int ltk_debug_solo_walk(int outstanding, int calls, int jump_at, int* slots_used);
+
 int ltk_program_graph_count(ltk_engine* e);
 
 int ltk_wav2lip_layer_count(ltk_engine* e);
diff --git a/livetalking_amd/_lib.py b/livetalking_amd/_lib.py
--- a/livetalking_amd/_lib.py
+++ b/livetalking_amd/_lib.py
@@ -54,6 +54,8 @@
     _fields_ = [("kernel", C.c_char * 64)] + [(n, C.c_int) for n in ("impl", "segs", "members", "grid")]
 
 
+DEFER_SYNC = 2
+
 SYMBOLS = {
     "ltk_last_error": (C.c_char_p, []),
     "ltk_version": (C.c_char_p, []),
@@ -66,6 +68,9 @@
     "ltk_avatar_release": (C.c_int, [C.c_void_p, C.c_int]),
     "ltk_mel_step": (C.c_int, [C.c_void_p, C.c_void_p, C.c_int, C.c_void_p, C.c_int, C.c_void_p, C.c_void_p]),
     "ltk_wav2lip_infer": (C.c_int, [C.c_void_p, C.POINTER(W2lReq), C.c_int, C.c_void_p]),
+    "ltk_wav2lip_infer_deferred": (C.c_int, [C.c_void_p, C.POINTER(W2lReq), C.c_int, C.c_void_p, C.c_int, C.POINTER(C.c_int)]),
+    "ltk_wav2lip_order_stream": (C.c_int, [C.c_void_p, C.c_void_p, C.c_size_t, C.c_void_p]),
+    "ltk_wav2lip_defer_stats": (C.c_int, [C.c_void_p, C.POINTER(C.c_ulonglong), C.POINTER(C.c_ulonglong), C.POINTER(C.c_ulonglong)]),
     "ltk_paste_back": (C.c_int, [C.c_void_p, C.c_int, C.c_int, C.c_void_p, C.c_void_p, C.c_int, C.c_void_p]),
     "ltk_paste_back_batch": (C.c_int, [C.c_void_p, C.c_int, C.c_void_p, C.c_void_p, C.c_int, C.c_void_p, C.c_void_p]),
     "ltk_musetalk_load": (C.c_int, [C.c_void_p, C.POINTER(NamedTensor), C.c_int, C.POINTER(NamedTensor), C.c_int, C.c_int]),
@@ -124,6 +129,7 @@
     "ltk_wav2lip_graph_count": (C.c_int, [C.c_void_p]),
     "ltk_program_graph_count": (C.c_int, [C.c_void_p]),
     "ltk_wav2lip_prefetch_stats": (C.c_int, [C.c_void_p, C.POINTER(C.c_ulonglong), C.POINTER(C.c_ulonglong), C.POINTER(C.c_ulonglong)]),
+    "ltk_debug_solo_walk": (C.c_int, [C.c_int, C.c_int, C.c_int, C.POINTER(C.c_int)]),
     "ltk_avatar_face_cache_bytes": (C.c_int, [C.c_void_p, C.c_int, C.POINTER(C.c_size_t)]),
     "ltk_musetalk_op_count": (C.c_int, [C.c_void_p]),
     "ltk_musetalk_op_name": (C.c_int, [C.c_void_p, C.c_int, C.c_char_p, C.c_int, C.POINTER(C.c_int)]),
diff --git a/livetalking_amd/avatars/wav2lip_avatar.py b/livetalking_amd/avatars/wav2lip_avatar.py
--- a/livetalking_amd/avatars/wav2lip_avatar.py
+++ b/livetalking_amd/avatars/wav2lip_avatar.py
@@ -104,6 +104,53 @@
     for eng in model.engines:
         n = min(batch_size, eng.max_frames)
         eng.wav2lip_forward_host(mel[:n], img[:n])
+
+
+def _frame_handle_type():
+    import torch
+
+    class FrameHandle(torch.Tensor):
+        @classmethod
+        def __torch_function__(cls, func, types, args=(), kwargs=None):
+            if getattr(func, "__name__", "") == "data_ptr":
+                return super().__torch_function__(func, types, args, kwargs or {})
+            pending = None
+            stack = list(args)
+            if kwargs:
+                stack.extend(kwargs.values())
+            while stack:
+                a = stack.pop()
+                if isinstance(a, (list, tuple)):
+                    stack.extend(a)
+                elif isinstance(a, FrameHandle):
+                    p = a.__dict__.get("_ltk_pass")
+                    if p is not None:
+                        p.order()
+                        pending = p
+            ret = super().__torch_function__(func, types, args, kwargs or {})
+            if pending is not None:
+                for r in (ret if isinstance(ret, (list, tuple)) else (ret,)):
+                    if isinstance(r, FrameHandle):
+                        r._ltk_pass = pending
+            return ret
+
+    return FrameHandle
+
+
+class _PendingPass:
+    __slots__ = ("engine", "ptr", "nbytes", "streams")
+
+    def __init__(self, engine, ptr, nbytes):
+        self.engine, self.ptr, self.nbytes, self.streams = engine, ptr, nbytes, set()
+
+    def order(self):
+        st = self.engine.current_stream()
+        if st not in self.streams:
+            self.engine.order_frames(self.ptr, self.nbytes, st)
+            self.streams.add(st)
+
+
+_FRAME_HANDLE = None
 
 
 @register("avatar", "wav2lip")
@@ -120,6 +167,9 @@
         h, w = self.frame_list_cycle[0].shape[:2]
         self._frame_hw = (int(h), int(w))
         self._sched = get_scheduler(self.engine)
+        self._held = (None, None)
+        if hasattr(self.engine, "order_frames"):
+            self.engine.defer_handles = True
         self.asr = MelASR(opt, self, engine=self.engine)
         self.asr.warm_up()
 
@@ -137,9 +187,18 @@
         if mel.shape[0] != B:
             raise ValueError(f"expected {B} mel windows, got {mel.shape[0]}")
         pred = torch.empty((B, 256, 256, 3), dtype=torch.uint8, device=mel.device)
-        self._sched.infer(self._aid, int(index), B, mel.data_ptr(), pred.data_ptr())
+        deferred = self._sched.infer(self._aid, int(index), B, mel.data_ptr(), pred.data_ptr())
         self._last_mel = mel
         items = list(pred.unbind(0))
+        if deferred:
+            self._held = (self._held[1], (mel, pred))
+            global _FRAME_HANDLE
+            if _FRAME_HANDLE is None:
+                _FRAME_HANDLE = _frame_handle_type()
+            pending = _PendingPass(self.engine, pred.data_ptr(), pred.numel())
+            items = [t.as_subclass(_FRAME_HANDLE) for t in items]
+            for t in items:
+                t._ltk_pass = pending
         if _PASTE_BATCH and hasattr(self.engine, "paste_back_batch"):
             FrameGroup.attach(items, pred, span=(len(self.frame_list_cycle), int(index), B))
         return items
diff --git a/livetalking_amd/csrc/defer_window.h b/livetalking_amd/csrc/defer_window.h
--- /dev/null
+++ b/livetalking_amd/csrc/defer_window.h
@@ -0,0 +1,204 @@
+#pragma once
+#include <stddef.h>
+
+#include <memory>
+#include <mutex>
+#include <vector>
+
+namespace ltk {
+
+struct PredRange {
+    const unsigned char* p = nullptr;
+    size_t bytes = 0;
+    bool overlaps(const void* q, size_t n) const {
+        const unsigned char* b = (const unsigned char*)q;
+        return n && bytes && b < p + bytes && p < b + n;
+    }
+};
+
+template <class Event>
+struct PendingPass {
+    Event ev{};
+    std::vector<std::shared_ptr<void>> hold;
+    std::vector<PredRange> ranges;
+    int slot = 0;
+    unsigned long seq = 0;
+};
+
+struct DeferStats {
+    unsigned long long deferred = 0;
+    unsigned long long max_outstanding = 0;
+    unsigned long long outstanding = 0;
+};
+
+template <class Event>
+class DeferWindow {
+   public:
+    using Rec = std::shared_ptr<PendingPass<Event>>;
+
+    template <class Create>
+    Rec acquire(Create create) {
+        {
+            std::lock_guard<std::mutex> g(mu_);
+            for (size_t i = 0; i < pool_.size(); ++i)
+                if (pool_[i].use_count() == 1) {
+                    Rec r = std::move(pool_[i]);
+                    pool_.erase(pool_.begin() + i);
+                    return r;
+                }
+        }
+        Rec r = std::make_shared<PendingPass<Event>>();
+        if (!create(&r->ev)) return nullptr;
+        return r;
+    }
+    void give_back(Rec r) {
+        if (!r) return;
+        clear_record(*r);
+        std::lock_guard<std::mutex> g(mu_);
+        pool_.push_back(std::move(r));
+    }
+    std::vector<Rec> push(const Rec& r) {
+        std::lock_guard<std::mutex> g(mu_);
+        std::vector<Rec> before = live_;
+        r->seq = ++issued_;
+        live_.push_back(r);
+        return before;
+    }
+    std::vector<Rec> snapshot() {
+        std::lock_guard<std::mutex> g(mu_);
+        return live_;
+    }
+    void retire(const Rec& r) {
+        std::vector<std::shared_ptr<void>> drop;
+        {
+            std::lock_guard<std::mutex> g(mu_);
+            for (size_t i = 0; i < live_.size(); ++i)
+                if (live_[i] == r) {
+                    live_.erase(live_.begin() + i);
+                    drop.swap(r->hold);
+                    r->ranges.clear();
+                    r->slot = 0;
+                    pool_.push_back(r);
+                    break;
+                }
+        }
+    }
+    void returned() {
+        std::lock_guard<std::mutex> g(mu_);
+        ++stats_.deferred;
+        if (live_.size() > stats_.max_outstanding) stats_.max_outstanding = live_.size();
+    }
+    std::vector<Rec> writers_of(const void* p, size_t bytes) {
+        std::lock_guard<std::mutex> g(mu_);
+        std::vector<Rec> out;
+        for (const Rec& r : live_)
+            for (const PredRange& q : r->ranges)
+                if (q.overlaps(p, bytes)) { out.push_back(r); break; }
+        return out;
+    }
+    bool slot_in_use(int slot) {
+        if (slot <= 0) return false;
+        std::lock_guard<std::mutex> g(mu_);
+        for (const Rec& r : live_)
+            if (r->slot == slot) return true;
+        return false;
+    }
+    unsigned long long slots_in_use() {
+        std::lock_guard<std::mutex> g(mu_);
+        unsigned long long m = 0;
+        for (const Rec& r : live_)
+            if (r->slot > 0 && r->slot < 64) m |= 1ull << r->slot;
+        return m;
+    }
+    Rec newest() {
+        std::lock_guard<std::mutex> g(mu_);
+        return live_.empty() ? nullptr : live_.back();
+    }
+    DeferStats stats() {
+        std::lock_guard<std::mutex> g(mu_);
+        DeferStats s = stats_;
+        s.outstanding = live_.size();
+        return s;
+    }
+    template <class Destroy>
+    void clear(Destroy destroy) {
+        std::vector<Rec> all;
+        {
+            std::lock_guard<std::mutex> g(mu_);
+            all.swap(live_);
+            for (Rec& r : pool_) all.push_back(std::move(r));
+            pool_.clear();
+        }
+        for (Rec& r : all) { clear_record(*r); destroy(r->ev); }
+    }
+
+   private:
+    static void clear_record(PendingPass<Event>& r) { r.hold.clear(); r.ranges.clear(); r.slot = 0; }
+    std::mutex mu_;
+    std::vector<Rec> live_;
+    std::vector<Rec> pool_;
+    unsigned long issued_ = 0;
+    DeferStats stats_;
+};
+
+struct PfSlotView {
+    bool valid = false;
+    double age = 0;
+    bool reader_running = false;
+    unsigned long stamp = 0;
+};
+
+inline int choose_prefetch_slot(const PfSlotView* s, int nslots, int cur, double stale) {
+    int victim = 0, busy = 0;
+    for (int k = 1; k <= nslots; ++k) {
+        if (k == cur) continue;
+        if (s[k].valid && s[k].age < stale) continue;
+        if (s[k].reader_running) { if (!busy || s[k].stamp > s[busy].stamp) busy = k; continue; }
+        if (!victim || s[k].stamp > s[victim].stamp) victim = k;
+    }
+    return victim ? victim : busy;
+}
+
+struct SoloWalk {
+    static constexpr int kSlots = 16;
+    PfSlotView s[kSlots + 1];
+    unsigned long clock = 0;
+    int filled_for_next = 0;
+    int calls = 0;
+    int prev_slot = 0;
+    struct Step { int slot, prefetch_into; };
+    Step call(int depth) {
+        Step st{filled_for_next, 0};
+        const bool hit = st.slot > 0;
+        if (hit) { s[st.slot].valid = false; s[st.slot].stamp = ++clock; }
+        const bool prefetch = hit || calls > 0;
+        if (prefetch) {
+            for (int k = 1; k <= kSlots; ++k) s[k].reader_running = depth > 0 && k == prev_slot && k != 0;
+            const int v = choose_prefetch_slot(s, kSlots, st.slot, 1.5);
+            if (v) { s[v].valid = true; s[v].age = 0; s[v].stamp = ++clock; }
+            st.prefetch_into = v;
+        }
+        filled_for_next = st.prefetch_into;
+        prev_slot = st.slot;
+        ++calls;
+        return st;
+    }
+    void jump() { filled_for_next = 0; calls = 0; }
+};
+
+inline int solo_walk_last_capture(int depth, int calls, int jump_at, int* slots_used) {
+    SoloWalk walk;
+    int seen_pass[SoloWalk::kSlots + 1] = {0}, seen_pf[SoloWalk::kSlots + 1] = {0};
+    int last = 0, used = 0;
+    for (int n = 0; n < calls; ++n) {
+        if (n == jump_at) walk.jump();
+        const SoloWalk::Step st = walk.call(depth);
+        if (++seen_pass[st.slot] <= 2) last = n;
+        if (st.prefetch_into && ++seen_pf[st.prefetch_into] <= 2) last = n;
+    }
+    for (int k = 1; k <= SoloWalk::kSlots; ++k) used += seen_pf[k] ? 1 : 0;
+    if (slots_used) *slots_used = used;
+    return last;
+}
+
+}
diff --git a/livetalking_amd/csrc/egress.hip b/livetalking_amd/csrc/egress.hip
--- a/livetalking_amd/csrc/egress.hip
+++ b/livetalking_amd/csrc/egress.hip
@@ -80,6 +80,7 @@
         const uint8_t* full = a.d_full + (size_t)q->idx * bytes;
         if (q->d_pred) {
             const int32_t* c = a.coords.data() + 4 * (size_t)q->idx;
+            CHK(order_behind_pending(e, sl.s, q->d_pred, (size_t)256 * 256 * 3));
             launch_paste(full, H, W, (const uint8_t*)q->d_pred, c[0], c[1], c[2], c[3], s->d_frame, sl.s);
             src = s->d_frame;
         } else {
@@ -167,6 +168,8 @@
     uint8_t* const conv = comp + bytes * n;
     if (hold_w) {
         const Avatar& a = *hold_w;
+        const hipError_t oe = order_behind_pending(e, sl.s, d_pred, (size_t)n * 256 * 256 * 3);
+        if (oe != hipSuccess) return fail(LTK_E_HIP, std::string("egress_batch: ") + hipGetErrorString(oe));
         for (int i0 = 0; i0 < n; i0 += kPasteBatch) {
             const int m = std::min(kPasteBatch, n - i0);
             PasteBatch pb;
diff --git a/livetalking_amd/csrc/engine.hip b/livetalking_amd/csrc/engine.hip
--- a/livetalking_amd/csrc/engine.hip
+++ b/livetalking_amd/csrc/engine.hip
@@ -80,10 +80,12 @@
 void ltk_engine_destroy(ltk_engine* e) {
     if (!e) return;
     if (e->tm_calls)
-        fprintf(stderr, "ltk: ltk_wav2lip_infer host time per call over %lu calls: prepare %.1f us, upload + pass launch %.1f us, prefetch join / serial launch %.1f us, wait for the device %.1f us\n",
-                e->tm_calls, e->tm_prep / e->tm_calls, e->tm_launch / e->tm_calls, e->tm_pf / e->tm_calls, e->tm_wait / e->tm_calls);
+        fprintf(stderr, "ltk: ltk_wav2lip_infer host time per call over %lu calls: prepare %.1f us, upload + pass launch %.1f us, prefetch join / serial launch %.1f us, wait for the device %.1f us, wait for the previous pass (deferred calls) %.1f us\n",
+                e->tm_calls, e->tm_prep / e->tm_calls, e->tm_launch / e->tm_calls, e->tm_pf / e->tm_calls, e->tm_wait / e->tm_calls, e->tm_prev / e->tm_calls);
     (void)hipSetDevice(e->device);
     (void)hipDeviceSynchronize();
+    (void)drain_pending(e);
+    e->defer.clear([](hipEvent_t& ev) { if (ev) (void)hipEventDestroy(ev); });
     wav2lip_unload(e);
     if (e->d_basis) (void)hipFree(e->d_basis);
     if (e->d_lohi) (void)hipFree(e->d_lohi);
@@ -119,8 +121,10 @@
 int ltk_engine_sync(ltk_engine* e) {
     if (!e) return fail(LTK_E_INVALID, "engine is null");
     CHK(enter_device(e->device));
-    CHK(hipDeviceSynchronize());
-    return LTK_OK;
+    const hipError_t se = hipDeviceSynchronize();
+    const int drc = drain_pending(e);
+    if (se != hipSuccess) return fail(LTK_E_HIP, std::string("hipDeviceSynchronize(): ") + hipGetErrorString(se));
+    return drc;
 }
 
 int ltk_avatar_register(ltk_engine* e, const uint8_t* face_bank, const uint8_t* full_bank,
@@ -152,6 +156,7 @@
 
 int ltk_avatar_release(ltk_engine* e, int avatar_id) {
     if (!e) return fail(LTK_E_INVALID, "engine is null");
+    if (e->defer.newest()) { (void)hipSetDevice(e->device); (void)drain_pending(e); }
     {
         std::lock_guard<std::mutex> ge(e->mu);
         for (ltk_engine::PfSlot& sl : e->pfs)
@@ -208,6 +213,7 @@
     const int32_t* c = a.coords.data() + 4 * (size_t)idx;
     const size_t bytes = (size_t)a.H * a.W * 3;
     StreamLease sl(e, stream);
+    CHK(order_behind_pending(e, sl.s, d_pred, (size_t)256 * 256 * 3));
     const uint8_t* full = a.d_full + (size_t)idx * bytes;
     if (out_is_device) {
         launch_paste(full, a.H, a.W, (const uint8_t*)d_pred, c[0], c[1], c[2], c[3], (uint8_t*)out, sl.s);
@@ -236,6 +242,7 @@
     StreamLease sl(e, stream);
     ScratchLease sc(e, bytes * n);
     if (!sc.s.d) return fail(LTK_E_NOMEM, "scratch allocation failed");
+    CHK(order_behind_pending(e, sl.s, d_pred, (size_t)n * 256 * 256 * 3));
     for (int i0 = 0; i0 < n; i0 += kPasteBatch) {
         const int m = std::min(kPasteBatch, n - i0);
         PasteBatch pb;
diff --git a/livetalking_amd/csrc/engine_debug.hip b/livetalking_amd/csrc/engine_debug.hip
--- a/livetalking_amd/csrc/engine_debug.hip
+++ b/livetalking_amd/csrc/engine_debug.hip
@@ -7,6 +7,7 @@
     if (!e->loaded) return fail(LTK_E_STATE, "ltk_wav2lip_load has not been called");
     if (B > e->max_frames) return fail(LTK_E_INVALID, "B exceeds max_frames");
     CHK(enter_device(e->device));
+    { const int drc = drain_pending(e); if (drc) return drc; }
     const int mb = std::min(e->micro_batch, kPackMaxFrames);
     const int cap = std::min(B, mb);
     DevBuf d_mel, d_face, d_pred;
@@ -47,6 +48,8 @@
 
 int ltk_debug_capture(ltk_engine* e, int enable) {
     if (!e) return fail(LTK_E_INVALID, "engine is null");
+    (void)hipSetDevice(e->device);
+    { const int drc = drain_pending(e); if (drc) return drc; }
     std::lock_guard<std::mutex> g(e->mu);
     e->capture = enable != 0;
     if (!enable) { e->taps.clear(); e->tap_shape.clear(); }
@@ -60,6 +63,8 @@
 
 int ltk_debug_get(ltk_engine* e, const char* layer, float* out, size_t n_floats) {
     if (!e || !layer || !out) return fail(LTK_E_INVALID, "bad arguments");
+    (void)hipSetDevice(e->device);
+    { const int drc = drain_pending(e); if (drc) return drc; }
     std::lock_guard<std::mutex> g(e->mu);
     auto it = e->taps.find(layer);
     if (it == e->taps.end()) return fail(LTK_E_STATE, std::string("no capture for layer ") + layer);
@@ -91,6 +96,7 @@
     if (!e->loaded) return fail(LTK_E_STATE, "ltk_wav2lip_load has not been called");
     if (frames > e->max_frames) return fail(LTK_E_INVALID, "frames exceeds max_frames");
     CHK(enter_device(e->device));
+    { const int drc = drain_pending(e); if (drc) return drc; }
     std::lock_guard<std::mutex> g(e->mu);
     if (e->capture) return fail(LTK_E_STATE, "disable capture before timing");
     const int mbs = std::min(e->micro_batch, kPackMaxFrames);
@@ -135,6 +141,8 @@
 
 int ltk_wav2lip_prefetch_stats(ltk_engine* e, unsigned long long* hits, unsigned long long* misses, unsigned long long* issued) {
     if (!e) return fail(LTK_E_INVALID, "engine is null");
+    (void)hipSetDevice(e->device);
+    { const int drc = drain_pending(e); if (drc) return drc; }
     std::lock_guard<std::mutex> g(e->mu);
     if (hits) *hits = e->pf_hits;
     if (misses) *misses = e->pf_misses;
@@ -142,6 +150,11 @@
     return LTK_OK;
 }
 
+int ltk_debug_solo_walk(int outstanding, int calls, int jump_at, int* slots_used) {
+    if (outstanding < 0 || outstanding > 1 || calls <= 0) return -1;
+    return solo_walk_last_capture(outstanding, calls, jump_at, slots_used);
+}
+
 int ltk_program_graph_count(ltk_engine* e) {
     if (!e) return 0;
     std::lock_guard<std::mutex> g(e->mu);
@@ -150,6 +163,8 @@
 
 int ltk_wav2lip_graph_count(ltk_engine* e) {
     if (!e) return 0;
+    (void)hipSetDevice(e->device);
+    (void)drain_pending(e);
     std::lock_guard<std::mutex> g(e->mu);
     return e->graphs.live();
 }
diff --git a/livetalking_amd/csrc/engine_internal.h b/livetalking_amd/csrc/engine_internal.h
--- a/livetalking_amd/csrc/engine_internal.h
+++ b/livetalking_amd/csrc/engine_internal.h
@@ -16,6 +16,7 @@
 
 #include "../../include/ltk.h"
 #include "conv_mfma.h"
+#include "defer_window.h"
 #include "dw_kernels.h"
 #include "hubert_kernels.h"
 #include "misc_kernels.h"
@@ -213,7 +214,9 @@
     SoloSeq solo_seq[2 * kPfSlots];
     unsigned long pf_hits = 0, pf_misses = 0, pf_issued = 0;
     std::atomic<bool> pf_fail_logged{false};
-    double tm_prep = 0, tm_launch = 0, tm_pf = 0, tm_wait = 0;
+    double tm_prep = 0, tm_launch = 0, tm_pf = 0, tm_wait = 0, tm_prev = 0;
+    DeferWindow<hipEvent_t> defer;
+    std::atomic<unsigned> defer_epoch{0};
     unsigned long tm_calls = 0;
     size_t buf_halfs[B_COUNT] = {0};
     float* d_head = nullptr;
@@ -371,28 +374,107 @@
     return 0;
 }
 
+inline int drain_pending(ltk_engine* e) {
+    const auto recs = e->defer.snapshot();
+    if (recs.empty()) return 0;
+    const hipError_t se = hipEventSynchronize(recs.back()->ev);
+    if (se != hipSuccess) (void)hipStreamSynchronize(e->compute);
+    for (const auto& r : recs) e->defer.retire(r);
+    if (se != hipSuccess)
+        return fail(LTK_E_HIP, std::string("a deferred ltk_wav2lip_infer pass issued by an EARLIER call failed on the device (reported by the call that waited for it): ") +
+                                   hipGetErrorString(se));
+    return 0;
+}
+inline hipError_t order_behind_pending(ltk_engine* e, hipStream_t s, const void* p, size_t bytes) {
+    const auto writers = e->defer.writers_of(p, bytes);
+    if (writers.empty()) return hipSuccess;
+    std::lock_guard<std::mutex> g(e->mu);
+    for (const auto& r : writers) {
+        const hipError_t we = hipStreamWaitEvent(s, r->ev, 0);
+        if (we != hipSuccess) return we;
+    }
+    return hipSuccess;
+}
+
+struct DeferCall {
+    bool want = false, ok = false;
+    int slot = 0;
+    std::vector<std::shared_ptr<void>> hold;
+    std::vector<PredRange> ranges;
+    double wait_prev_us = 0;
+    bool deferred = false;
+};
+
 template <class Enq>
-int infer_call(ltk_engine* e, void* stream, Enq enq) {
-    Ev done;
-    CHK(done.create());
+int infer_call(ltk_engine* e, void* stream, Enq enq, DeferCall* dc = nullptr) {
+    auto make_ev = [](hipEvent_t* ev) { return hipEventCreateWithFlags(ev, hipEventDisableTiming) == hipSuccess; };
+    auto rec = e->defer.acquire(make_ev);
+    if (!rec) { (void)hipGetLastError(); (void)drain_pending(e); return fail(LTK_E_HIP, "hipEventCreate failed"); }
     int rc = 0;
+    bool launched = false, stream_wait_failed = false;
+    std::vector<decltype(rec)> before;
     {
         std::lock_guard<std::mutex> g(e->mu);
         if (stream) {
             Ev ready;
-            CHK(ready.create());
-            CHK(hipEventRecord(ready.e, (hipStream_t)stream));
-            CHK(hipStreamWaitEvent(e->compute, ready.e, 0));
-        }
-        rc = enq();
-        if (!rc && hipEventRecord(done.e, e->compute) != hipSuccess) rc = fail(LTK_E_HIP, "hipEventRecord failed");
-    }
-    if (!rc) {
-        if (stream && hipStreamWaitEvent((hipStream_t)stream, done.e, 0) != hipSuccess) rc = fail(LTK_E_HIP, "hipStreamWaitEvent failed");
-        if (hipEventSynchronize(done.e) != hipSuccess) rc = fail(LTK_E_HIP, "hipEventSynchronize failed");
-    } else {
+            hipError_t he = ready.create();
+            if (he == hipSuccess) he = hipEventRecord(ready.e, (hipStream_t)stream);
+            if (he == hipSuccess) he = hipStreamWaitEvent(e->compute, ready.e, 0);
+            if (he != hipSuccess) rc = fail(LTK_E_HIP, std::string("waiting for the caller's stream: ") + hipGetErrorString(he));
+        }
+        if (!rc) {
+            launched = true;
+            rc = enq();
+            if (!rc && hipEventRecord(rec->ev, e->compute) != hipSuccess) rc = fail(LTK_E_HIP, "hipEventRecord failed");
+        }
+        if (!rc && dc && dc->want && dc->ok) {
+            rec->hold = std::move(dc->hold);
+            rec->ranges = std::move(dc->ranges);
+            rec->slot = dc->slot;
+            before = e->defer.push(rec);
+            dc->deferred = true;
+            if (stream && hipStreamWaitEvent((hipStream_t)stream, rec->ev, 0) != hipSuccess) stream_wait_failed = true;
+        } else if (!rc) {
+            before = e->defer.snapshot();
+        }
+    }
+    if (rc) {
+        const std::string msg = g_err;
+        if (launched) (void)hipStreamSynchronize(e->compute);
+        (void)drain_pending(e);
+        e->defer.give_back(rec);
+        return fail(rc, msg);
+    }
+    if (dc && dc->deferred) {
+        if (stream_wait_failed) rc = fail(LTK_E_HIP, "hipStreamWaitEvent failed");
+        if (!rc && !before.empty()) {
+            const auto t0 = std::chrono::steady_clock::now();
+            const hipError_t se = hipEventSynchronize(before.back()->ev);
+            dc->wait_prev_us = std::chrono::duration<double, std::micro>(std::chrono::steady_clock::now() - t0).count();
+            if (se != hipSuccess)
+                rc = fail(LTK_E_HIP, std::string("the deferred pass of the PREVIOUS ltk_wav2lip_infer_deferred call failed on the device (reported by this call, which "
+                                                 "waited for it; the frames of both calls are invalid): ") + hipGetErrorString(se));
+        }
+        if (rc) {
+            const std::string msg = g_err;
+            (void)hipStreamSynchronize(e->compute);
+            for (const auto& r : before) e->defer.retire(r);
+            e->defer.retire(rec);
+            dc->deferred = false;
+            return fail(rc, msg);
+        }
+        for (const auto& r : before) e->defer.retire(r);
+        e->defer.returned();
+        return 0;
+    }
+    if (stream && hipStreamWaitEvent((hipStream_t)stream, rec->ev, 0) != hipSuccess) rc = fail(LTK_E_HIP, "hipStreamWaitEvent failed");
+    if (hipEventSynchronize(rec->ev) != hipSuccess) {
+        rc = fail(LTK_E_HIP, before.empty() ? "hipEventSynchronize failed"
+                                            : "hipEventSynchronize failed (this call, or the deferred pass of an earlier call it ran behind: the frames of both are invalid)");
         (void)hipStreamSynchronize(e->compute);
     }
+    for (const auto& r : before) e->defer.retire(r);
+    e->defer.give_back(rec);
     return rc;
 }
 
diff --git a/livetalking_amd/csrc/tune.h b/livetalking_amd/csrc/tune.h
--- a/livetalking_amd/csrc/tune.h
+++ b/livetalking_amd/csrc/tune.h
@@ -30,7 +30,8 @@
     X(LIN_MP, 1)                \
     X(GN_COOP, 1)               \
     X(AUDIO0, 3)                \
-    X(CONV_S2D, 1)
+    X(CONV_S2D, 1)              \
+    X(DEFER, 1)
 
 
 enum Knob {
diff --git a/livetalking_amd/csrc/w2l_infer.hip b/livetalking_amd/csrc/w2l_infer.hip
--- a/livetalking_amd/csrc/w2l_infer.hip
+++ b/livetalking_amd/csrc/w2l_infer.hip
@@ -103,7 +103,27 @@
     return LTK_OK;
 }
 
-int ltk_wav2lip_infer(ltk_engine* e, const ltk_w2l_req* reqs, int nreq, void* stream) {
+}
+
+static int w2l_infer_checked(ltk_engine* e, const ltk_w2l_req* reqs, int nreq, void* stream, DeferCall* dc);
+static int w2l_infer(ltk_engine* e, const ltk_w2l_req* reqs, int nreq, void* stream, DeferCall* dc) {
+    if (!e) return fail(LTK_E_INVALID, "bad arguments");
+    if (e->defer_epoch.load(std::memory_order_relaxed) != knob_epoch() && e->defer.newest()) {
+        CHK(enter_device(e->device));
+        const int drc = drain_pending(e);
+        if (drc) return drc;
+    }
+    const int rc = w2l_infer_checked(e, reqs, nreq, stream, dc);
+    if (rc && e->defer.newest()) {
+        const std::string msg = g_err;
+        (void)hipSetDevice(e->device);
+        (void)drain_pending(e);
+        return fail(rc, msg);
+    }
+    return rc;
+}
+
+static int w2l_infer_checked(ltk_engine* e, const ltk_w2l_req* reqs, int nreq, void* stream, DeferCall* dc) {
     if (!e || !reqs || nreq <= 0) return fail(LTK_E_INVALID, "bad arguments");
     if (!e->loaded) return fail(LTK_E_STATE, "ltk_wav2lip_load has not been called");
     static const bool timing = getenv("LTK_INFER_TIMING") != nullptr;
@@ -151,6 +171,7 @@
         }
         const bool solo = nreq == 1 && !cached && knob(K_PREFETCH) && e->alt_frames > 0 && total <= std::min(e->alt_frames, mbs) &&
                           !e->capture && knob(K_HEAD_FUSED) && e->c7;
+        const bool defer = solo && dc && dc->want && knob(K_DEFER) != 0;
         const int first = reqs[0].index;
         int slot = 0;
         if (solo)
@@ -188,16 +209,18 @@
         if (!rc && prefetch) {
             constexpr double kPfStale = 1.5;
             const double now = std::chrono::duration<double>(std::chrono::steady_clock::now().time_since_epoch()).count();
-            int victim = 0, busy = 0;
+            PfSlotView view[ltk_engine::kPfSlots + 1];
+            const unsigned long long in_flight = e->defer.slots_in_use();
             for (int k = 1; k <= ltk_engine::kPfSlots; ++k) {
-                if (k == slot) continue;
                 const ltk_engine::PfSlot& sl = e->pfs[k];
-                if (sl.valid && now - sl.filled_at < kPfStale) continue;
-                if (sl.read && hipEventQuery(sl.ev_read) != hipSuccess) { if (!busy || sl.stamp > e->pfs[busy].stamp) busy = k; continue; }
-                if (!victim || sl.stamp > e->pfs[victim].stamp) victim = k;
+                view[k].valid = sl.valid;
+                view[k].age = now - sl.filled_at;
+                view[k].stamp = sl.stamp;
+                view[k].reader_running = k != slot && !(sl.valid && view[k].age < kPfStale) &&
+                                         (((in_flight >> k) & 1) || (sl.read && hipEventQuery(sl.ev_read) != hipSuccess));
             }
             (void)hipGetLastError();
-            if (!victim) victim = busy;
+            const int victim = choose_prefetch_slot(view, ltk_engine::kPfSlots, slot, kPfStale);
             if (victim) {
             ltk_engine::PfSlot& sl = e->pfs[victim];
             sl.valid = false;
@@ -226,15 +249,54 @@
             seq_rec->avatar = reqs[0].avatar; seq_rec->next = first + total; seq_rec->nf = total; seq_rec->stamp = ++e->pf_clock;
         }
         if (timing) tp3 = std::chrono::steady_clock::now();
+        if (!rc && defer) {
+            dc->ok = true;
+            dc->slot = slot;
+            for (auto& ap : hold) dc->hold.push_back(ap);
+            dc->ranges.push_back({(const unsigned char*)reqs[0].d_pred, (size_t)total * 65536 * 3});
+            e->defer_epoch.store(knob_epoch(), std::memory_order_relaxed);
+        }
         return rc;
-    });
+    }, dc);
     if (timing) {
         const auto tp4 = std::chrono::steady_clock::now();
         auto us = [](std::chrono::steady_clock::time_point a, std::chrono::steady_clock::time_point b) { return std::chrono::duration<double, std::micro>(b - a).count(); };
         std::lock_guard<std::mutex> g(e->pool_mu);
-        e->tm_prep += us(tp0, tp1); e->tm_launch += us(tp1, tp2); e->tm_pf += us(tp2, tp3); e->tm_wait += us(tp3, tp4); ++e->tm_calls;
+        const double prev = dc ? dc->wait_prev_us : 0.0;
+        e->tm_prep += us(tp0, tp1); e->tm_launch += us(tp1, tp2); e->tm_pf += us(tp2, tp3); e->tm_wait += us(tp3, tp4) - prev; e->tm_prev += prev; ++e->tm_calls;
     }
     return rc;
 }
 
-}
+extern "C" {
+
+int ltk_wav2lip_infer(ltk_engine* e, const ltk_w2l_req* reqs, int nreq, void* stream) { return w2l_infer(e, reqs, nreq, stream, nullptr); }
+
+int ltk_wav2lip_infer_deferred(ltk_engine* e, const ltk_w2l_req* reqs, int nreq, void* stream, int flags, int* deferred) {
+    if (deferred) *deferred = 0;
+    if (flags & ~LTK_DEFER_SYNC) return fail(LTK_E_INVALID, "unknown flags");
+    DeferCall dc;
+    dc.want = !(flags & LTK_DEFER_SYNC);
+    const int rc = w2l_infer(e, reqs, nreq, stream, &dc);
+    if (!rc && deferred) *deferred = dc.deferred ? 1 : 0;
+    return rc;
+}
+
+int ltk_wav2lip_order_stream(ltk_engine* e, const void* d_pred, size_t bytes, void* stream) {
+    if (!e || !d_pred || !bytes) return fail(LTK_E_INVALID, "bad arguments");
+    if (e->defer.writers_of(d_pred, bytes).empty()) return LTK_OK;
+    CHK(enter_device(e->device));
+    CHK(order_behind_pending(e, (hipStream_t)stream, d_pred, bytes));
+    return LTK_OK;
+}
+
+int ltk_wav2lip_defer_stats(ltk_engine* e, unsigned long long* deferred, unsigned long long* max_outstanding, unsigned long long* outstanding) {
+    if (!e) return fail(LTK_E_INVALID, "engine is null");
+    const DeferStats st = e->defer.stats();
+    if (deferred) *deferred = st.deferred;
+    if (max_outstanding) *max_outstanding = st.max_outstanding;
+    if (outstanding) *outstanding = st.outstanding;
+    return LTK_OK;
+}
+
+}
diff --git a/livetalking_amd/csrc/w2l_program.hip b/livetalking_amd/csrc/w2l_program.hip
--- a/livetalking_amd/csrc/w2l_program.hip
+++ b/livetalking_amd/csrc/w2l_program.hip
@@ -266,6 +266,7 @@
 namespace ltk {
 
 void wav2lip_unload(ltk_engine* e) {
+    (void)drain_pending(e);
     if (e->aux2) (void)hipStreamSynchronize(e->aux2);
     e->graphs.drop();
     if (e->d_tab) { (void)hipFree(e->d_tab); e->d_tab = nullptr; }
diff --git a/livetalking_amd/engine.py b/livetalking_amd/engine.py
--- a/livetalking_amd/engine.py
+++ b/livetalking_amd/engine.py
@@ -1,6 +1,7 @@
 from __future__ import annotations
 
 import ctypes as C
+import sys
 import threading
 from typing import Dict, Optional, Sequence
 
@@ -34,6 +35,7 @@
         self._closed = False
         self._lock = threading.Lock()
         self._egress_open = set()
+        self.defer_handles = False
 
     def close(self):
         if not self._closed:
@@ -133,7 +135,26 @@
             arr[i].batch = int(batch)
             arr[i].d_mel = C.c_void_p(mel_ptr)
             arr[i].d_pred = C.c_void_p(pred_ptr)
+        if len(reqs) == 1 and self.defer_handles:
+            deferred = C.c_int(0)
+            _lib.check(self._lib.ltk_wav2lip_infer_deferred(self._h, arr, 1, C.c_void_p(stream), 0, C.byref(deferred)))
+            return bool(deferred.value)
         _lib.check(self._lib.ltk_wav2lip_infer(self._h, arr, len(reqs), C.c_void_p(stream)))
+        return False
+
+    def current_stream(self) -> int:
+        torch = sys.modules.get("torch")
+        return int(torch.cuda.current_stream(self.device).cuda_stream) if torch is not None else 0
+
+    def order_frames(self, d_pred_ptr: int, nbytes: int, stream: Optional[int] = None):
+        if stream is None:
+            stream = self.current_stream()
+        _lib.check(self._lib.ltk_wav2lip_order_stream(self._h, C.c_void_p(d_pred_ptr), int(nbytes), C.c_void_p(stream)))
+
+    def defer_stats(self) -> dict:
+        d, m, o = C.c_ulonglong(0), C.c_ulonglong(0), C.c_ulonglong(0)
+        _lib.check(self._lib.ltk_wav2lip_defer_stats(self._h, C.byref(d), C.byref(m), C.byref(o)))
+        return {"deferred": int(d.value), "max_outstanding": int(m.value), "outstanding": int(o.value)}
 
     def paste_back(self, avatar_id: int, idx: int, d_pred_ptr: int, out: np.ndarray, stream: int = 0):
         _lib.check(self._lib.ltk_paste_back(self._h, int(avatar_id), int(idx), C.c_void_p(d_pred_ptr),
diff --git a/livetalking_amd/scheduler.py b/livetalking_amd/scheduler.py
--- a/livetalking_amd/scheduler.py
+++ b/livetalking_amd/scheduler.py
@@ -7,12 +7,13 @@
 
 
 class _Req:
-    __slots__ = ("args", "batch", "done", "err")
+    __slots__ = ("args", "batch", "done", "err", "deferred")
 
     def __init__(self, args, batch):
         self.args, self.batch = args, batch
         self.done = threading.Event()
         self.err = None
+        self.deferred = False
 
 
 class BatchingScheduler:
@@ -78,12 +79,14 @@
         r.done.wait()
         if r.err is not None:
             raise r.err
+        return r.deferred
 
     def _run_solo(self, args, frames):
         t0 = time.perf_counter()
         err = None
+        deferred = False
         try:
-            self._call([args])
+            deferred = self._call([args])
         except Exception as ex:
             err = ex
         t1 = time.perf_counter()
@@ -106,6 +109,7 @@
                 self._cv.notify_all()
         if err is not None:
             raise err
+        return bool(deferred)
 
     def _ensure_workers(self):
         self._workers = [w for w in self._workers if w.is_alive()]
@@ -140,14 +144,16 @@
         errs = [None] * len(group)
         if group:
             try:
-                self._call([q.args for q in group])
+                res = self._call([q.args for q in group])
+                if len(group) == 1:
+                    group[0].deferred = bool(res)
             except Exception as ex:
                 if len(group) == 1:
                     errs[0] = ex
                 else:
                     for i, q in enumerate(group):
                         try:
-                            self._call([q.args])
+                            q.deferred = bool(self._call([q.args]))
                         except Exception as ex_i:
                             errs[i] = ex_i
         t1 = time.perf_counter()
```

Measured after the change: 13610 frames/s, median of 6. 1.02x the previous value.
